# Hydr10n/DirectX-Physically-Based-Raytracer

Hardware: AMD Instinct MI355X
Metric: Mrays/s per GPU + frames/s at 1080p, Cornell Box 4spp/8bounce (higher is better)
Workload: dtype f32

## Files before the change

directx-physically-based-raytracer_amd/csrc/pt_api.hip:

```cpp
#include "pt_internal.hpp"

#include <cmath>
#include <cstdio>
#include <cstring>

using namespace pt;

static thread_local std::string g_createError;
namespace pt { std::string& create_error() { return g_createError; } }

int pt::fail(Context* c, int status, const std::string& msg)
{
    if (c) c->lastError = msg; else g_createError = msg;
    return status;
}
int pt::fail_hip(Context* c, hipError_t e, const char* what)
{
    return fail(c, e == hipErrorOutOfMemory ? PT_ERROR_OUT_OF_MEMORY : PT_ERROR_HIP, std::string(what) + ": " + hipGetErrorString(e));
}

static int poll_tlas_header(Context& c, bool wait);

extern "C" {

// ... 88 lines not shown

int pt_set_round_chains(PtContext* ctx, uint32_t chains)
{
    if (!ctx) return PT_ERROR_INVALID_ARGUMENT;
    API_ARG(&ctx->c, chains <= Context::kMaxChains, "at most 4 chains");
    ctx->c.chains = chains;
    ctx->c.graphKey.clear(); ctx->c.chainGraphKey.clear();
    return PT_OK;
}

int pt_sync(PtContext* ctx)
{
    if (!ctx) return PT_ERROR_INVALID_ARGUMENT;
    API_HIP(&ctx->c, hipSetDevice(ctx->c.device));
    API_HIP(&ctx->c, hipStreamSynchronize(ctx->c.stream));
    return poll_tlas_header(ctx->c, true);
}

int pt_heap_resize(PtContext* ctx, uint32_t descriptor_count)
{
    if (!ctx) return PT_ERROR_INVALID_ARGUMENT;
    ctx->c.heapHost.resize(descriptor_count, HeapEntry{ nullptr, 0, 0, 0 });
    ctx->c.heapDirty = true;
    return PT_OK;
}

int pt_heap_set_buffer(PtContext* ctx, uint32_t descriptor, const void* device_ptr, uint64_t bytes, uint32_t stride)
{
    if (!ctx) return PT_ERROR_INVALID_ARGUMENT;
    Context& c = ctx->c;
    API_ARG(&c, descriptor < c.heapHost.size(), "descriptor index beyond pt_heap_resize");
    API_ARG(&c, stride == 0 || stride == 2 || stride == 4 || stride == 8, "buffer stride must be 0 (raw), 2 / 4 (typed index buffer) or 8 (structured half4 motion vectors)");
    c.heapHost[descriptor] = HeapEntry{ device_ptr, bytes, stride, kKindBuffer };
    c.heapDirty = true;
    return PT_OK;
}

int pt_heap_set_texture(PtContext* ctx, uint32_t descriptor, const void* device_ptr, uint32_t width, uint32_t height, uint32_t format, uint32_t is_cube)
{
    if (!ctx) return PT_ERROR_INVALID_ARGUMENT;
    Context& c = ctx->c;
    API_ARG(&c, descriptor < c.heapHost.size(), "descriptor index beyond pt_heap_resize");
    API_ARG(&c, device_ptr && width && height, "texture pointer / size is null");
    API_ARG(&c, format <= PT_FORMAT_R32G32B32A32_FLOAT, "unsupported texture format");
    API_ARG(&c, !is_cube || width == height, "cube faces must be square");
    c.heapHost[descriptor] = HeapEntry{ device_ptr, (uint64_t)width | ((uint64_t)height << 32), format, is_cube ? kKindTextureCube : kKindTexture2D };
    c.heapDirty = true;
    return PT_OK;
}

static int upload_heap(Context& c)
{
    if (!c.srgbLutDev) {
        float lut[256];
        for (int i = 0; i < 256; i++) { double v = i / 255.0; lut[i] = (float)(v <= 0.04045 ? v / 12.92 : pow((v + 0.055) / 1.055, 2.4)); }
        DeviceBuffer<float> dev;
        API_HIP(&c, dev.reserve(256));
        API_HIP(&c, hipMemcpy(dev.data(), lut, sizeof lut, hipMemcpyHostToDevice));
        c.srgbLutDev = std::move(dev);
    }
    if (!c.heapDirty) return PT_OK;
    uint32_t n = (uint32_t)c.heapHost.size();
    c.heapHasTextures = false;
    for (const HeapEntry& e : c.heapHost) if (e.kind != kKindBuffer) c.heapHasTextures = true;
    API_HIP(&c, c.heapDev.reserve(n));
    if (n) API_HIP(&c, hipMemcpyAsync(c.heapDev.data(), c.heapHost.data(), sizeof(HeapEntry) * n, hipMemcpyHostToDevice, c.stream));
    API_HIP(&c, hipStreamSynchronize(c.stream));
    c.heapDirty = false; c.validated = false;
    return PT_OK;
}

static int check_geometries(Context& c, const PtGeometryDesc* geometries, uint32_t geometry_count)
{
    API_ARG(&c, geometries || geometry_count == 0, "geometries is NULL");
    for (uint32_t g = 0; g < geometry_count; g++) {
        API_ARG(&c, geometries[g].IndexStride == 2 || geometries[g].IndexStride == 4, "Triangle index format must be either uint16 or uint32");
        API_ARG(&c, geometries[g].IndexCount % 3 == 0, "Triangle index count must be divisible by 3");
        API_ARG(&c, geometries[g].IndexCount == 0 || (geometries[g].VertexBuffer && geometries[g].IndexBuffer), "geometry buffer is NULL");
        API_ARG(&c, geometries[g].VertexStride >= 12, "vertex stride must cover a float3 position");
    }
    return PT_OK;
}

static int check_depth(Context& c, uint32_t tlasDepth)
{
    if (2u * (tlasDepth + c.maxBlasDepth) + 4u > (uint32_t)kStackSize)
        return fail(&c, PT_ERROR_INVALID_ARGUMENT, "acceleration structure too deep for the traversal stack (top level " + std::to_string(tlasDepth)
                    + " + bottom level " + std::to_string(c.maxBlasDepth) + " levels)");
    return PT_OK;
}

static int poll_tlas_header(Context& c, bool wait)
{
    if (!c.tlasHeaderPending) return PT_OK;
    if (wait) API_HIP(&c, hipEventSynchronize(c.tlasHeaderEvent.get()));
    else if (hipEventQuery(c.tlasHeaderEvent.get()) != hipSuccess) { (void)hipGetLastError(); return PT_OK; }
    c.tlasHeaderPending = false;
    if (c.tlasHeaderHost.data()->error) { drop_tlas(c); return fail(&c, PT_ERROR_INVALID_ARGUMENT, "top-level build failed: tree deeper than the builder's level limit"); }
    int s = check_depth(c, c.tlasHeaderHost.data()->depth);
    if (s != PT_OK) drop_tlas(c);
    return s;
}

int pt_build_bottom_level(PtContext* ctx, const PtGeometryDesc* geometries, uint32_t geometry_count, uint32_t build_flags, uint64_t* out_blas_id)
{
    if (!ctx) return PT_ERROR_INVALID_ARGUMENT;
    Context& c = ctx->c;
    API_ARG(&c, out_blas_id, "out_blas_id is NULL");
    int s = check_geometries(c, geometries, geometry_count);
    if (s != PT_OK) return s;
    API_HIP(&c, hipSetDevice(c.device));
    Blas b;
    const bool updatable = (build_flags & PT_BUILD_FLAG_ALLOW_UPDATE) != 0;
    if (!updatable) std::swap(b.tree, c.buildScratch);
    hipError_t e = build_blas_device(geometries, geometry_count, updatable, c.stream, b);
    if (!updatable) std::swap(b.tree, c.buildScratch);
    if (e != hipSuccess) return fail_hip(&c, e, "bottom-level build");
    if (b.buildError || 2u * b.depth + 4u > (uint32_t)kStackSize) return fail(&c, PT_ERROR_INVALID_ARGUMENT, "bottom-level build failed: tree too deep for the traversal stack");
    b.geometryCount = geometry_count;
    uint64_t id = c.nextBlasId++;
    c.maxBlasDepth = std::max(c.maxBlasDepth, b.depth);
    c.blas[id] = std::move(b);
    *out_blas_id = id;
    return PT_OK;
}

int pt_update_bottom_level(PtContext* ctx, uint64_t blas_id, const PtGeometryDesc* geometries, uint32_t geometry_count, uint32_t build_flags)
{
    if (!ctx) return PT_ERROR_INVALID_ARGUMENT;
    Context& c = ctx->c;
    auto it = c.blas.find(blas_id);
    API_ARG(&c, it != c.blas.end(), "unknown bottom-level id");
    API_ARG(&c, c.viewers.empty(), "other contexts view this context's scene (pt_share_scene): destroy or re-point them before updating a bottom level");
    int s = check_geometries(c, geometries, geometry_count);
    if (s != PT_OK) return s;
    API_HIP(&c, hipSetDevice(c.device));
    Blas& b = it->second;
    uint32_t ntris = 0;
    for (uint32_t g = 0; g < geometry_count; g++) ntris += geometries[g].IndexCount / 3;
    if (b.updatable && ntris == b.triCount && geometry_count == b.geometryCount) {
        hipError_t e = refit_blas_device(geometries, geometry_count, c.stream, b);
        if (e != hipSuccess) return fail_hip(&c, e, "bottom-level update");
        drop_tlas(c);
        return PT_OK;
    }
    API_HIP(&c, hipStreamSynchronize(c.stream));
    Blas nb;
    const bool updatable = (build_flags & PT_BUILD_FLAG_ALLOW_UPDATE) != 0 || b.updatable;
    if (!updatable) std::swap(nb.tree, c.buildScratch);
    hipError_t e = build_blas_device(geometries, geometry_count, updatable, c.stream, nb);
    if (!updatable) std::swap(nb.tree, c.buildScratch);
    if (e != hipSuccess) return fail_hip(&c, e, "bottom-level update");
    if (nb.buildError || 2u * nb.depth + 4u > (uint32_t)kStackSize) return fail(&c, PT_ERROR_INVALID_ARGUMENT, "bottom-level update failed: tree too deep for the traversal stack");
    nb.geometryCount = geometry_count;
    c.maxBlasDepth = std::max(c.maxBlasDepth, nb.depth);
    b = std::move(nb);
    drop_tlas(c);
    return PT_OK;
}

int pt_skin_mesh(PtContext* ctx, const void* skeletal_vertices, const float* skeletal_transforms, void* vertices, void* motion_vectors, uint32_t vertex_count)
{
    if (!ctx) return PT_ERROR_INVALID_ARGUMENT;
    Context& c = ctx->c;
    API_ARG(&c, vertex_count == 0 || (skeletal_vertices && skeletal_transforms && vertices && motion_vectors), "a skinning buffer is NULL");
    API_HIP(&c, hipSetDevice(c.device));
    API_HIP(&c, launch_skin(c.stream, skeletal_vertices, skeletal_transforms, vertices, motion_vectors, vertex_count));
    return PT_OK;
}

int pt_release_bottom_level(PtContext* ctx, uint64_t blas_id)
{
    if (!ctx) return PT_ERROR_INVALID_ARGUMENT;
    Context& c = ctx->c;
    auto it = c.blas.find(blas_id);
    API_ARG(&c, it != c.blas.end(), "unknown bottom-level id");
    API_ARG(&c, c.viewers.empty(), "other contexts view this context's scene (pt_share_scene)");
    hipStreamSynchronize(c.stream);
    for (uint64_t id : c.tlasBlasIds) if (id == blas_id) { drop_tlas(c); break; }
    c.blas.erase(it);
    c.maxBlasDepth = 0;
    for (auto& kv : c.blas) c.maxBlasDepth = std::max(c.maxBlasDepth, kv.second.depth);
    return PT_OK;
}

namespace {
struct TopLevelPlan {
    struct Piece { uint64_t id; Blas* b; uint32_t nodeBase, triBase; bool referenced; };
    std::vector<Piece> pieces;
    std::vector<uint64_t> pieceIds;
    std::map<uint64_t, uint32_t> pieceOf;
    std::vector<BlasEntry> table;
    uint32_t tlasNodeExact = 0, tlasNodeCap = 0, blobNodes = 0, blobTris = 0;
    uint64_t tris = 0, objectEnd = 0, bindingHash = 1469598103934665603ull, lightHash = 1469598103934665603ull;
    size_t srcBytes = 0, nodeAt = 0, triAt = 0, idxAt = 0, instAt = 0, leafAt = 0, enterAt = 0, total = 0;
    size_t node_at(const Piece& p) const { return nodeAt + sizeof(WideNode) * (size_t)p.nodeBase; }
    size_t tri_at(const Piece& p) const { return triAt + sizeof(TriPacket) * (size_t)p.triBase; }
    size_t idx_at(const Piece& p) const { return idxAt + 16 * (size_t)p.triBase; }
    bool in_place(const Piece& p) const { return p.b->blobNodeAt == node_at(p) && p.b->blobTriAt == tri_at(p) && p.b->blobIdxAt == idx_at(p); }
};
}

static int plan_top_level(Context& c, const PtInstanceDesc* descs, uint32_t count, TopLevelPlan& P)
{
    P.tlasNodeExact = wide_node_capacity(count);
    P.tlasNodeCap = P.tlasNodeExact;
    if (count >= 64u) { P.tlasNodeCap = 128u; while (P.tlasNodeCap < P.tlasNodeExact) P.tlasNodeCap <<= 1; }
    if (c.blobDev && c.tlasNodeReserve >= P.tlasNodeExact && c.tlasNodeReserve <= 2u * P.tlasNodeCap) P.tlasNodeCap = c.tlasNodeReserve;
    P.blobNodes = P.tlasNodeCap;
    P.lightHash ^= count;
    P.srcBytes = sizeof(InstanceSource) * (size_t)count;
    std::vector<uint8_t>& up = c.tlasUploadHost;
    up.resize(P.srcBytes);
    for (uint32_t i = 0; i < count; i++) {
        auto it = c.blas.find(descs[i].AccelerationStructure);
        API_ARG(&c, it != c.blas.end(), "instance refers to an unknown bottom-level id");
        Blas& b = it->second;
        auto pb = P.pieceOf.find(descs[i].AccelerationStructure);
        if (pb == P.pieceOf.end()) {
            P.pieces.push_back(TopLevelPlan::Piece{ descs[i].AccelerationStructure, &b, P.blobNodes, P.blobTris, true });
            P.table.push_back(BlasEntry{ nullptr, nullptr, b.rootBounds.data(), b.triCount, b.nodeCount, P.blobNodes, P.blobTris, nullptr, descs[i].InstanceID & 0xFFFFFFu, b.geometryCount });
            P.blobNodes += b.nodeCount; P.blobTris += b.triCount;
            P.pieceIds.push_back(descs[i].AccelerationStructure);
            pb = P.pieceOf.emplace(descs[i].AccelerationStructure, (uint32_t)P.table.size() - 1).first;
        }
        InstanceSource src;
        memcpy(src.transform, descs[i].Transform, sizeof(float) * 12);
        src.instanceID = descs[i].InstanceID & 0xFFFFFFu; src.mask = descs[i].InstanceMask & 0xFFu; src.blasSlot = pb->second; src._pad = 0;
        memcpy(up.data() + sizeof(InstanceSource) * (size_t)i, &src, sizeof src);
        P.tris += b.triCount;
        P.objectEnd = std::max<uint64_t>(P.objectEnd, (uint64_t)src.instanceID + b.geometryCount);
        P.bindingHash = (P.bindingHash ^ src.instanceID) * 1099511628211ull; P.bindingHash = (P.bindingHash ^ descs[i].AccelerationStructure) * 1099511628211ull;
        P.lightHash = (P.lightHash ^ src.instanceID) * 1099511628211ull; P.lightHash = (P.lightHash ^ src.mask) * 1099511628211ull;
        P.lightHash = (P.lightHash ^ descs[i].AccelerationStructure) * 1099511628211ull;
    }
    for (auto& kv : c.blas)
        if (kv.second.inBlob && !P.pieceOf.count(kv.first)) {
// ... 51 lines not shown
        Blas& b = *p.b;
        uint8_t* dn = blob + P.node_at(p); uint8_t* dt = blob + P.tri_at(p); uint8_t* di = blob + P.idx_at(p);
        const uint64_t n16 = sizeof(WideNode) * (uint64_t)b.nodeCount / 16, t16 = sizeof(TriPacket) * (uint64_t)b.triCount / 16, i16 = b.triCount;
        const void *sn, *st_, *si;
        if (b.updatable) {
            jobs.push_back(BlobCopy{ b.nodes.data(), dn, n16 });
            if (b.triCount) { jobs.push_back(BlobCopy{ b.tris.data(), dt, t16 }); jobs.push_back(BlobCopy{ b.idx.data(), di, i16 }); }
            sn = b.nodes.data(); st_ = b.tris.data(); si = b.idx.data();
        } else {
            if (b.inBlob) {
                if (newBlob) {
                    preJobs.push_back(BlobCopy{ oldBlob + b.blobNodeAt, dn, n16 });
                    if (b.triCount) { preJobs.push_back(BlobCopy{ oldBlob + b.blobTriAt, dt, t16 }); preJobs.push_back(BlobCopy{ oldBlob + b.blobIdxAt, di, i16 }); }
                }
            } else {
                preJobs.push_back(BlobCopy{ b.nodes.data(), dn, n16 });
                if (b.triCount) { preJobs.push_back(BlobCopy{ b.tris.data(), dt, t16 }); preJobs.push_back(BlobCopy{ b.idx.data(), di, i16 }); }
                adopting.push_back(&b);
            }
            sn = dn; st_ = dt; si = di;
        }
        if (p.referenced) { BlasEntry& row = P.table[P.pieceOf[p.id]]; row.nodes = (const WideNode*)sn; row.tris = (const TriPacket*)st_; row.idx = (const uint4*)si; }
    }
    const size_t tableOff = (P.srcBytes + 15) / 16 * 16, tableBytes = sizeof(BlasEntry) * P.table.size();
    hipError_t e = build_tlas_prepare(c.tlas, count);
    if (e != hipSuccess) return fail_hip(&c, e, "top-level build");
    jobs.push_back(BlobCopy{ c.tlas.nodes.data(), blob + P.nodeAt, sizeof(WideNode) * (size_t)P.tlasNodeExact / 16 });
    const size_t preOff = (tableOff + tableBytes + 15) / 16 * 16, preBytes = sizeof(BlobCopy) * preJobs.size();
    const size_t jobsOff = (preOff + preBytes + 15) / 16 * 16, jobsBytes = sizeof(BlobCopy) * jobs.size();
    std::vector<uint8_t>& up = c.tlasUploadHost;
    up.resize(jobsOff + jobsBytes);
    if (tableBytes) memcpy(up.data() + tableOff, P.table.data(), tableBytes);
    if (preBytes) memcpy(up.data() + preOff, preJobs.data(), preBytes);
    memcpy(up.data() + jobsOff, jobs.data(), jobsBytes);
    if (up.size() > c.tlasUploadDev.capacity()) {
        if (!growth) API_HIP(&c, hipStreamSynchronize(c.stream));
        API_HIP(&c, c.tlasUploadDev.reserve(up.size() * 2));
    }
    {
        Context::UploadStage& sg = c.tlasStage[c.tlasStageNext];
        c.tlasStageNext ^= 1u;
        if (sg.event) API_HIP(&c, hipEventSynchronize(sg.event.get()));
        else API_HIP(&c, create_event(sg.event, hipEventDisableTiming));
        if (up.size() > sg.host.capacity()) API_HIP(&c, sg.host.reserve(up.size() * 2));
        memcpy(sg.host.data(), up.data(), up.size());
        API_HIP(&c, hipMemcpyAsync(c.tlasUploadDev.data(), sg.host.data(), up.size(), hipMemcpyHostToDevice, c.stream));
        API_HIP(&c, hipEventRecord(sg.event.get(), c.stream));
    }
    const uint8_t* upDev = c.tlasUploadDev.data();
    const InstanceSource* dSrc = (const InstanceSource*)upDev;
    const BlasEntry* dTable = (const BlasEntry*)(upDev + tableOff);
    const BlobCopy* dPre = (const BlobCopy*)(upDev + preOff);
    const BlobCopy* dJobs = (const BlobCopy*)(upDev + jobsOff);

    if (!preJobs.empty()) e = launch_blob_assembly(nullptr, c.tlas, nullptr, 0, nullptr, nullptr, dPre, (uint32_t)preJobs.size(), nullptr, c.stream);
    if (e == hipSuccess) e = launch_instance_records(dSrc, dTable, count, c.tlas.instances.data(), c.tlas.blasBounds.data(), c.tlas.tree.bounds.data(), c.stream);
    if (e == hipSuccess) e = build_tlas_device(c.tlas.instances.data(), c.tlas.blasBounds.data(), count, c.stream, c.tlas);
    if (e == hipSuccess) e = launch_blob_assembly(c.tlas.instances.data(), c.tlas, dTable, count, (InstanceT*)(blob + P.instAt), (InstanceT*)(blob + P.leafAt),
                                                 dJobs, (uint32_t)jobs.size(), (f4v*)(blob + P.enterAt), c.stream);
    if (e == hipSuccess) e = hipMemcpyAsync(c.tlasHeaderHost.data(), c.tlas.tree.header.data(), sizeof(WideHeader), hipMemcpyDeviceToHost, c.stream);
    if (e == hipSuccess) e = hipEventRecord(c.tlasHeaderEvent.get(), c.stream);
    if (!adopting.empty() || (newBlob && oldBlob)) {
        const hipError_t es = hipStreamSynchronize(c.stream);
        if (e == hipSuccess) e = es;
    }
    if (e != hipSuccess) {
        if (newCopy) (void)hipStreamSynchronize(c.stream);
        return fail_hip(&c, e, "top-level build");
    }

    if (newBlob) c.blobDev = std::move(newCopy);
    for (Blas* b : adopting) { b->nodes.reset(); b->tris.reset(); b->idx.reset(); b->inBlob = true; }
    for (const auto& p : P.pieces) if (p.b->inBlob) { p.b->blobNodeAt = P.node_at(p); p.b->blobTriAt = P.tri_at(p); p.b->blobIdxAt = P.idx_at(p); }
    c.tlasHeaderPending = true;
    c.tlasNodeReserve = P.tlasNodeCap;
    SceneRefs& r = c.scene;
    r.instances = c.tlas.instances.data(); r.instanceCount = count; r.triangleCount = P.tris;
    r.blob.base = (const f4v*)c.blobDev.data();
    r.blob.nodeOff16 = (uint32_t)(P.nodeAt / 16); r.blob.triOff16 = (uint32_t)(P.triAt / 16); r.blob.idxOff16 = (uint32_t)(P.idxAt / 16);
    r.blob.instOff16 = (uint32_t)(P.instAt / 16); r.blob.leafInstOff16 = (uint32_t)(P.leafAt / 16); r.blob.enterOff16 = (uint32_t)(P.enterAt / 16);
    r.blob.instCount = count; r.blob.nodeCount = P.blobNodes; r.blob.triCount = P.blobTris; r.blob.bytes = (uint32_t)P.total;
    r.blasTable = dTable; r.blasTableCount = (uint32_t)P.table.size(); r.instSource = dSrc; r.blasTableMaxTris = 0;
    for (const BlasEntry& te : P.table) r.blasTableMaxTris = std::max(r.blasTableMaxTris, te.triCount);
    c.tlasBlasIds = P.pieceIds;
    if (P.objectEnd != c.tlasObjectEnd || count != c.tlasValidatedCount || P.bindingHash != c.tlasBindingHash) c.validated = false;
    c.tlasObjectEnd = P.objectEnd; c.tlasValidatedCount = count; c.tlasBindingHash = P.bindingHash;
    if (P.lightHash != c.tlasLightHash) c.lightListValid = false;
    c.tlasLightHash = P.lightHash;
    c.normalsShared = c.validated && c.sharedVerdict;
    c.haveTlas = true;
    return PT_OK;
}

int pt_share_scene(PtContext* ctx, PtContext* source)
{
    if (!ctx || !source || ctx == source) return PT_ERROR_INVALID_ARGUMENT;
    Context& c = ctx->c; Context& s = source->c;
    API_ARG(&c, c.device == s.device, "both contexts must live on the same device");
    API_ARG(&c, c.viewers.empty(), "other contexts view this context's scene");
    API_ARG(&c, !s.sceneOwner, "the source views another context's scene itself: share from the owner");
    API_HIP(&c, hipSetDevice(c.device));
    API_HIP(&c, hipStreamSynchronize(s.stream));
    API_HIP(&c, hipStreamSynchronize(c.stream));
    int st = poll_tlas_header(s, true);
    if (st != PT_OK) return fail(&c, st, s.lastError);
    if (!s.haveTlas) return fail(&c, PT_ERROR_NOT_READY, "the source context has no top-level acceleration structure");
    if (c.sceneOwner) detach_from_owner(c);
    else { API_HIP(&c, materialise_adopted(c)); c.tlas = Tlas(); c.blobDev.reset(); }
    drop_tlas(c);
    c.scene = s.scene;
    c.tlasObjectEnd = s.tlasObjectEnd; c.maxBlasDepth = s.maxBlasDepth;
    c.heapHost = s.heapHost; c.heapDirty = true;
    c.objects = s.objects; c.objectCount = s.objectCount; c.instanceData = s.instanceData; c.instanceDataCount = s.instanceDataCount;
    c.sceneOwner = &s; s.viewers.push_back(&c);
    c.tlasHeaderPending = false; c.validated = false;
    c.haveTlas = true;
    return PT_OK;
}

int pt_get_accel_stats(PtContext* ctx, PtAccelStats* out)
{
    if (!ctx || !out) return PT_ERROR_INVALID_ARGUMENT;
    Context& c = ctx->c;
    API_HIP(&c, hipSetDevice(c.device));
    API_HIP(&c, hipStreamSynchronize(c.stream));
    int st = poll_tlas_header(c, true);
    if (st != PT_OK) return st;
    memset(out, 0, sizeof *out);
    out->InstanceCount = c.scene.instanceCount;
    out->BottomLevelCount = (uint32_t)c.blas.size();
    out->TriangleCount = c.scene.triangleCount;
    out->NodeSizeBytes = sizeof(WideNode); out->TriangleSizeBytes = sizeof(TriPacket);
    uint64_t nb = (uint64_t)wide_node_capacity(c.scene.instanceCount) * sizeof(WideNode), tb = 0;
    for (auto& kv : c.blas) { nb += (uint64_t)kv.second.nodeCount * sizeof(WideNode); tb += (uint64_t)kv.second.triCount * sizeof(TriPacket); out->MaxBottomLevelDepth = std::max(out->MaxBottomLevelDepth, kv.second.depth); }
    out->BlobBytes = c.sceneOwner ? 0 : c.scene.blob.bytes;
    out->SharedScene = c.sceneOwner ? 1u : 0u;
    out->NormalRecords = c.normalsShared ? 1u : 0u;
    out->RoundObjectsInLds = round_objects_in_lds(c, c.objectCount, (bool)c.shadeGeomDev);
    out->RoundRecordsInLds = round_records_in_lds(c, c.objectCount, (bool)c.shadeGeomDev);
    if (c.tlasHeaderHost && !c.tlasHeaderPending) out->TopLevelDepth = c.tlasHeaderHost.data()->depth;
    out->NodeBytes = nb; out->TriangleBytes = tb;
    for (auto& kv : c.blas) if (!kv.second.inBlob) out->OwnedBottomLevelBytes += (uint64_t)kv.second.nodeCount * sizeof(WideNode) + (uint64_t)kv.second.triCount * (sizeof(TriPacket) + 16);
    return PT_OK;
}

int pt_set_camera(PtContext* ctx, const PtCamera* camera)
{
    if (!ctx) return PT_ERROR_INVALID_ARGUMENT;
    API_ARG(&ctx->c, camera, "camera is NULL");
    ctx->c.camera = *camera; ctx->c.haveCamera = true;
    return PT_OK;
}
int pt_set_scene_data(PtContext* ctx, const PtSceneData* scene_data)
{
    if (!ctx) return PT_ERROR_INVALID_ARGUMENT;
    API_ARG(&ctx->c, scene_data, "scene_data is NULL");
    ctx->c.sceneData = *scene_data; ctx->c.haveSceneData = true;
    return PT_OK;
}
int pt_set_object_data(PtContext* ctx, const PtObjectData* device_objects, uint32_t count)
{
    if (!ctx) return PT_ERROR_INVALID_ARGUMENT;
    API_ARG(&ctx->c, device_objects || count == 0, "device_objects is NULL");
    ctx->c.objects = device_objects; ctx->c.objectCount = count;
    return PT_OK;
}
int pt_invalidate_object_data(PtContext* ctx)
{
    if (!ctx) return PT_ERROR_INVALID_ARGUMENT;
    ctx->c.validated = false; ctx->c.normalsShared = false; ctx->c.sharedVerdict = false;
    ctx->c.objectDataGen++;
    return PT_OK;
}
int pt_set_instance_data(PtContext* ctx, const PtInstanceData* device_instances, uint32_t count)
{
    if (!ctx) return PT_ERROR_INVALID_ARGUMENT;
    ctx->c.instanceData = device_instances; ctx->c.instanceDataCount = count;
    return PT_OK;
}

int pt_set_sharding(PtContext* ctx, const PtSharding* s)
{
    if (!ctx) return PT_ERROR_INVALID_ARGUMENT;
    API_ARG(&ctx->c, s && s->RankCount >= 1 && s->RankIndex < s->RankCount && s->BandHeight >= 1, "invalid sharding");
    ctx->c.sharding = *s;
    return PT_OK;
}

int pt_local_rows(const PtSharding* s, uint32_t frame_height, uint32_t* out_rows)
{
    if (!s || !out_rows || s->RankCount == 0 || s->BandHeight == 0 || s->RankIndex >= s->RankCount) return PT_ERROR_INVALID_ARGUMENT;
    uint32_t rows = 0;
    for (uint32_t b = s->RankIndex; (uint64_t)b * s->BandHeight < frame_height; b += s->RankCount) {
        uint32_t y0 = b * s->BandHeight;
        rows += (frame_height - y0 < s->BandHeight) ? frame_height - y0 : s->BandHeight;
    }
    *out_rows = rows;
    return PT_OK;
}

int pt_deinterleave_bands(PtContext* ctx, void* dst_full, const void* gathered, const uint64_t* rank_offsets_host, uint32_t rank_count,
                          uint32_t band_height, uint32_t width, uint32_t height, uint32_t pixel_bytes)
{
    if (!ctx) return PT_ERROR_INVALID_ARGUMENT;
    Context& c = ctx->c;
    API_ARG(&c, dst_full && gathered && rank_offsets_host && rank_count >= 1 && band_height >= 1, "invalid de-interleave arguments");
    API_ARG(&c, pixel_bytes % 4 == 0, "pixel size must be a multiple of 4 bytes");
    API_HIP(&c, hipSetDevice(c.device));
    API_ARG(&c, rank_count <= 64, "at most 64 ranks");
    hipError_t e = launch_deinterleave(c.stream, dst_full, gathered, rank_offsets_host, rank_count, band_height, width, height, pixel_bytes);
    if (e != hipSuccess) return fail_hip(&c, e, "de-interleave");
    return PT_OK;
}

}

static int validate_scene(Context& c)
{
    if (c.validated && c.validatedObjects == c.objects && c.validatedObjectCount == c.objectCount) return PT_OK;
    const uint32_t heapCount = (uint32_t)c.heapHost.size();
    if (c.tlasObjectEnd > c.objectCount)
        return fail(&c, PT_ERROR_INVALID_ARGUMENT, "InstanceID + geometry count of an instance reaches ObjectData[" + std::to_string(c.tlasObjectEnd - 1)
                    + "] but only " + std::to_string(c.objectCount) + " objects are bound (pt_set_object_data)");
    if (c.instanceData && c.instanceDataCount < c.scene.instanceCount)
        return fail(&c, PT_ERROR_INVALID_ARGUMENT, "InstanceData holds fewer records than the top level has instances");
    uint32_t sharedMismatch = 0;
    if (c.objectCount) {
        API_HIP(&c, c.validateDev.reserve(8));
        if (c.objectCount > c.shadeGeomDev.capacity()) {
            API_HIP(&c, hipStreamSynchronize(c.stream));
            c.shadeGeomDev.reset(); c.shadeTexDev.reset();
            API_HIP(&c, c.shadeTexDev.reserve(kTextureSlots * (size_t)c.objectCount));
            API_HIP(&c, c.shadeGeomDev.reserve(c.objectCount));
        }
        API_HIP(&c, hipMemsetAsync(c.validateDev.data(), 0, sizeof(uint32_t) * 8, c.stream));
        API_HIP(&c, launch_validate_objects(c.stream, c.objects, c.objectCount, c.heapDev.data(), heapCount, c.validateDev.data(), c.shadeGeomDev.data(), c.shadeTexDev.data()));
        if (c.scene.blasTable && c.scene.instSource)
            API_HIP(&c, launch_check_shared_geometry(c.stream, c.scene.instSource, c.scene.blasTable, c.scene.blob.instCount, c.shadeGeomDev.data(), c.validateDev.data()));
        uint32_t r[8] = { 0, 0, 0, 0, 0, 0, 0, 0 };
        API_HIP(&c, hipMemcpyAsync(r, c.validateDev.data(), sizeof r, hipMemcpyDeviceToHost, c.stream));
        API_HIP(&c, hipStreamSynchronize(c.stream));
        sharedMismatch = r[4];
        if (r[0]) {
            static const char* what[] = { "", "MeshDescriptors.Vertices", "MeshDescriptors.Indices", "MeshDescriptors.MotionVectors", "TextureMapInfo.Descriptor" };
            return fail(&c, PT_ERROR_INVALID_ARGUMENT, std::string("ObjectData[") + std::to_string(r[1]) + "]." + what[r[0] < 5 ? r[0] : 0] + " = " + std::to_string(r[2])
                        + (r[3] ? " is not the kind of descriptor that member needs" : " is beyond the descriptor heap (" + std::to_string(heapCount) + " descriptors)"));
        }
    }
    c.validated = true; c.validatedObjects = c.objects; c.validatedObjectCount = c.objectCount;
    c.sharedVerdict = c.objectCount != 0 && c.scene.blasTable != nullptr && sharedMismatch == 0;
    c.normalsShared = c.sharedVerdict;
    return PT_OK;
}

int pt::make_views(Context& c, uint32_t width, uint32_t height, SceneView& sv, FrameView& fv, bool needFrameInputs)
{
    int s = poll_tlas_header(c, true);
    if (s != PT_OK) return s;
    if (!c.haveTlas) return fail(&c, PT_ERROR_NOT_READY, "no top-level acceleration structure: call pt_build_top_level first");
    if (needFrameInputs && (!c.haveCamera || !c.haveSceneData)) return fail(&c, PT_ERROR_NOT_READY, "camera / scene data not set");
    if (!c.objects && c.scene.instanceCount) return fail(&c, PT_ERROR_NOT_READY, "object data not set");
    s = upload_heap(c);
    if (s != PT_OK) return s;
    s = validate_scene(c);
    if (s != PT_OK) return s;
    if (needFrameInputs && c.sceneData.EnvironmentLightTextureDescriptor != ~0u) {
        const uint32_t d = c.sceneData.EnvironmentLightTextureDescriptor;
        API_ARG(&c, d < c.heapHost.size(), "SceneData.EnvironmentLightTextureDescriptor is beyond the descriptor heap");
        API_ARG(&c, c.heapHost[d].kind == (c.sceneData.IsEnvironmentLightTextureCubeMap ? kKindTextureCube : kKindTexture2D),
                "SceneData.EnvironmentLightTextureDescriptor is not the kind of texture IsEnvironmentLightTextureCubeMap says");
    }
    sv.accel.instances = c.scene.instances; sv.accel.instanceCount = c.scene.instanceCount;
    sv.objects = c.objects; sv.objectCount = c.objectCount; sv.shadeGeom = c.shadeGeomDev.data(); sv.shadeTex = c.shadeTexDev.data();
    sv.instanceData = c.instanceData;
    sv.heap = c.heapDev.data(); sv.heapCount = (uint32_t)c.heapHost.size();
    sv.srgbLut = c.srgbLutDev.data();
    fv.width = width; fv.height = height;
    fv.rankIndex = c.sharding.RankIndex; fv.rankCount = c.sharding.RankCount; fv.bandHeight = c.sharding.BandHeight;
    pt_local_rows(&c.sharding, height, &fv.localRows);
    return PT_OK;
}

int pt::check_raytrace_args(Context& c, const PtTextures* tx)
{
    API_ARG(&c, c.settings.Denoiser <= PT_DENOISER_NRD_RELAX, "unknown Denoiser value");
    API_ARG(&c, !c.settings.IsDIEnabled || (tx->Diffuse && tx->Specular), "IsDIEnabled reads the direct lighting from Textures.Diffuse / Textures.Specular (pt_di_render): not bound");
    API_ARG(&c, !(c.settings.Denoiser >= PT_DENOISER_NRD_REBLUR) || (tx->Diffuse && tx->Specular), "NRD modes write Textures.Diffuse / Textures.Specular: not bound");
    API_ARG(&c, c.settings.SamplesPerPixel < 65536 && c.settings.Bounces < 32768, "SamplesPerPixel / Bounces out of range");
    API_ARG(&c, tx->Position && tx->FlatNormal && tx->GeometricNormal && tx->BaseColorMetalness && tx->NormalRoughness && tx->IOR
                 && tx->Transmission && tx->Radiance, "a G-buffer texture the path tracer reads is not bound (Raytracing::Textures)");
    return PT_OK;
}

extern "C" {

int pt_gbuffer_render(PtContext* ctx, const PtGBufferConstants* constants, const PtTextures* textures)
{
    if (!ctx) return PT_ERROR_INVALID_ARGUMENT;
    Context& c = ctx->c;
    API_ARG(&c, constants && textures, "constants / textures is NULL");
    API_HIP(&c, hipSetDevice(c.device));
    SceneView sv; FrameView fv; memset(&sv, 0, sizeof sv); memset(&fv, 0, sizeof fv);
    int s = make_views(c, constants->RenderSize[0], constants->RenderSize[1], sv, fv);
    if (s != PT_OK) return s;
    API_HIP(&c, launch_gbuffer(c, sv, fv, constants->Flags, *textures));
    return PT_OK;
}

int pt_raytrace_set_constants(PtContext* ctx, const PtGraphicsSettings* settings)
{
    if (!ctx) return PT_ERROR_INVALID_ARGUMENT;
    API_ARG(&ctx->c, settings, "settings is NULL");
    ctx->c.settings = *settings; ctx->c.haveSettings = true;
    return PT_OK;
}

int pt_raytrace_render(PtContext* ctx, const PtTextures* tx)
{
    if (!ctx) return PT_ERROR_INVALID_ARGUMENT;
    Context& c = ctx->c;
    API_ARG(&c, tx, "textures is NULL");
    if (!c.haveSettings) return fail(&c, PT_ERROR_NOT_READY, "call pt_raytrace_set_constants first");
    int s = check_raytrace_args(c, tx);
    if (s != PT_OK) return s;
    API_HIP(&c, hipSetDevice(c.device));
    SceneView sv; FrameView fv; memset(&sv, 0, sizeof sv); memset(&fv, 0, sizeof fv);
    s = make_views(c, c.settings.RenderSize[0], c.settings.RenderSize[1], sv, fv);
    if (s != PT_OK) return s;
    if (c.settings.Bounces == 0) return PT_OK;
    API_HIP(&c, launch_raytrace(c, sv, fv, *tx, false));
    return PT_OK;
}

int pt_trace_visibility(PtContext* ctx, const PtRayDesc* device_rays, uint32_t count, float* device_visibility)
// ... 168 lines not shown
```

directx-physically-based-raytracer_amd/csrc/pt_internal.hpp:

```cpp
#pragma once
#include <hip/hip_runtime.h>

#include <algorithm>
#include <map>
#include <string>
#include <type_traits>
#include <vector>

#include "../../include/ptamd.h"
#include "pt_memory.hpp"
#include "pt_trace2.hpp"
#include "pt_sharc.hpp"

namespace pt {

struct WideHeader { uint32_t nodeCount, itemCount, depth, error; };

struct TreeBuffers {
    DeviceBuffer<float4> boxLo, boxHi; DeviceBuffer<uint32_t> bounds;
    DeviceBuffer<uint64_t> keys, keysSorted; DeviceBuffer<uint32_t> index, indexSorted;
    DeviceBuffer<uint8_t> sortTemp; size_t sortTempBytes = 0;
    DeviceBuffer<uint64_t> leafKeys; DeviceBuffer<float4> leafLo, leafHi;
    DeviceBuffer<int2> children; DeviceBuffer<int> parentInternal, parentLeaf;
    DeviceBuffer<float4> nodeLo, nodeHi; DeviceBuffer<uint32_t> arrival;
    DeviceBuffer<int> binaryRootOf, slotRefs; DeviceBuffer<uint32_t> leafDst, slotOfPrim;
    DeviceBuffer<WideHeader> header; DeviceBuffer<uint8_t> collapseState;
    DeviceBuffer<uint8_t> dp;
};

inline uint32_t wide_node_capacity(uint32_t nleaves) { return nleaves + 1u; }

struct Blas {
    DeviceBuffer<WideNode> nodes;
    DeviceBuffer<TriPacket> tris;
    DeviceBuffer<uint4> idx;
    DeviceBuffer<float> rootBounds;
    uint32_t triCount = 0, leafCount = 0, nodeCount = 0, depth = 0, geometryCount = 0;
    bool buildError = false, updatable = false;
    bool inBlob = false; uint64_t blobNodeAt = 0, blobTriAt = 0, blobIdxAt = 0;
    TreeBuffers tree;
};

struct Tlas {
    DeviceBuffer<WideNode> nodes;
    DeviceBuffer<float> rootBounds;
    DeviceBuffer<InstanceRecord> instances;
    DeviceBuffer<const float*> blasBounds;
    TreeBuffers tree;
};

struct InstanceSource { float transform[12]; uint32_t instanceID, mask, blasSlot, _pad; };
struct BlasEntry { const WideNode* nodes; const TriPacket* tris; const float* rootBounds; uint32_t triCount, nodeCount, nodeBase, triBase; const uint4* idx;
                   uint32_t objectBase, geometryCount; };
struct BlobCopy { const void* src; void* dst; uint64_t n16; };

struct SceneRefs {
    const InstanceRecord* instances = nullptr; uint32_t instanceCount = 0;
    uint64_t triangleCount = 0;
    BlobView blob{};
    const BlasEntry* blasTable = nullptr; uint32_t blasTableCount = 0, blasTableMaxTris = 0;
    const InstanceSource* instSource = nullptr;
};

struct alignas(16) ShadeGeom { const uint8_t* vb; uint32_t stride, nOff, tOff, uvOff[2], _pad; };
static_assert(sizeof(ShadeGeom) == 32, "layout");

struct SceneView {
    AccelView accel;
    const PtObjectData* objects;
    const ShadeGeom* shadeGeom;
    const HeapEntry* shadeTex;
    const PtInstanceData* instanceData;
    const HeapEntry* heap;
    const float* srgbLut;
    uint32_t objectCount, heapCount;
};

struct FrameView {
    uint32_t width, height;
    uint32_t localRows;
    uint32_t rankIndex, rankCount, bandHeight;
};

struct PathQueue {
    float4* s0;
    float4* s1;
    float4* s2;
    float4* r0;
    float4* r1;
    uint4*  hit;
};

constexpr uint32_t kSubQueueShiftFused = 5, kSubQueueShiftStream = 7, kSubQueuesMax = 1u << kSubQueueShiftStream;

struct FrameConstants { PtCamera cam; PtSceneData sd; PtGraphicsSettings gs; };
struct RoundArgs;

struct DeviceCounters {
    unsigned long long primaryRays, secondaryRays, nodesVisited, trianglesTested;
    unsigned int mismatchCount, stackOverflows;
    float mismatchRay[16];
    unsigned int maxNodesPerRay, _pad2;
};

struct Context {
    int device = 0;
    hipStream_t stream = nullptr;
    std::string lastError;

    std::vector<HeapEntry> heapHost;
    DeviceBuffer<HeapEntry> heapDev; bool heapDirty = true;
    DeviceBuffer<float> srgbLutDev;
    bool heapHasTextures = false;

    std::map<uint64_t, Blas> blas; uint64_t nextBlasId = 1;
    TreeBuffers buildScratch;
    Tlas tlas; bool haveTlas = false;
    DeviceBuffer<uint8_t> blobDev;
    SceneRefs scene;
    Context* sceneOwner = nullptr;
    std::vector<Context*> viewers;
    uint32_t framesInFlight = 1;
    std::vector<uint64_t> tlasBlasIds;
    std::vector<uint8_t> tlasUploadHost; DeviceBuffer<uint8_t> tlasUploadDev;
    struct UploadStage { PinnedBuffer<uint8_t> host; Event event; };
    UploadStage tlasStage[2]; uint32_t tlasStageNext = 0;
    PinnedBuffer<WideHeader> tlasHeaderHost; Event tlasHeaderEvent; bool tlasHeaderPending = false;
    uint32_t maxBlasDepth = 0, tlasNodeReserve = 0;
    uint32_t tlasValidatedCount = ~0u, persistentGrid = 0;
    uint64_t tlasBindingHash = 0;
    uint64_t tlasObjectEnd = 0;
    DeviceBuffer<ShadeGeom> shadeGeomDev;
    DeviceBuffer<HeapEntry> shadeTexDev;
    DeviceBuffer<uint4> shadeRecA; DeviceBuffer<uint32_t> shadeRecB;
    bool normalsShared = false;
    bool sharedVerdict = false;
    bool validated = false; DeviceBuffer<uint32_t> validateDev;
    const void* validatedObjects = nullptr; uint32_t validatedObjectCount = 0;

    PtCamera camera{}; PtSceneData sceneData{}; PtGraphicsSettings settings{};
    bool haveCamera = false, haveSceneData = false, haveSettings = false;
    const PtObjectData* objects = nullptr; uint32_t objectCount = 0;
    const PtInstanceData* instanceData = nullptr; uint32_t instanceDataCount = 0;
    PtSharding sharding{0, 1, 16, 0};

    DeviceBuffer<uint4> queueArrays[2][6];
    PathQueue queue[2]{};
    DeviceBuffer<uint4> primaryRecords;
    DeviceBuffer<float2> pixelAux;
    DeviceBuffer<FrameConstants> frameConstants;
    GraphExec graphExec; std::string graphKey; bool disableGraphs = false;
    static constexpr uint32_t kMaxChains = 4;
    uint32_t chains = 0;
    Stream chainStream[kMaxChains - 1]; Event chainFork, chainJoin[kMaxChains - 1];
    GraphExec chainGraph[kMaxChains]; std::string chainGraphKey;
    DeviceBuffer<uint32_t> queueCounts;
    DeviceBuffer<RoundArgs> roundArgs; std::string roundArgsKey;
    DeviceBuffer<DeviceCounters> counters;
    uint64_t lastIterations = 0;
    uint32_t debugFlags = 0;

    void* comm = nullptr; bool commOwned = false; uint32_t commRank = 0, commWorld = 1;

    bool timing = false;
    std::vector<Event> evExtend, evShade, evRound;
    uint32_t nExtend = 0, nShade = 0, nRound = 0;

    PtDISettings diSettings{}; bool haveDISettings = false;
    uint64_t tlasLightHash = 0;
    uint32_t objectDataGen = 0;
    DeviceBuffer<uint4> lightList; uint32_t lightCount = 0;
    DeviceBuffer<uint32_t> lightInstStart;
    uint64_t lightListKey = 0; bool lightListValid = false;
    DeviceBuffer<PtTriangleLight> lightRecords; DeviceBuffer<float> lightCdf, lightBlockSums; uint32_t lightRecordCount = 0;
    PtDIResamplingSettings diReuse{}; bool diReuseOn = false;
    DeviceBuffer<PtDIReservoir> diResA, diResB;
    DeviceBuffer<int8_t> diOffsets;
    bool diHistoryValid = false; uint32_t diHistorySize[2] = {0, 0}; uint64_t diHistoryLightKey = 0; uint32_t diResCount = 0;
    PtDIVisibilitySettings diVisibility{}; bool diVisibilityOn = false;
    PtDIPairwiseSettings diPairwise{};
    PtDILightSamplingSettings diSampling{};
    DeviceBuffer<PtDIPresampledLight> diTiles, diCells;
    uint32_t diTileCount = 0, diCellCount = 0;
    uint32_t diReGIRLayout = 0;
    DeviceBuffer<float> diOnion;

    PtPostProcessSettings post{}; bool havePost = false;
    DeviceBuffer<ushort4> postLevels;
    uint32_t postDims[9][2] = {};
    size_t postOffset[9] = {};

    PtSHARCSettings sharcSettings{}; bool haveSharcSettings = false;
    uint32_t sharcCapacity = 0, sharcParity = 0;
    DeviceBuffer<unsigned long long> sharcKeys;
    DeviceBuffer<uint4> sharcVoxels[2];
    DeviceBuffer<SharcView> sharcView;
    DeviceBuffer<float> sharcRough[2];
    DeviceBuffer<PtSHARCPathScatter> sharcLogScatter;
    DeviceBuffer<PtSHARCPathVertex> sharcLog; uint32_t sharcLogPaths = 0, sharcLogBounces = 0;
};

std::string& create_error();
int fail(Context* c, int status, const std::string& msg);
int fail_hip(Context* c, hipError_t e, const char* what);
#define API_HIP(ctx, expr) do { hipError_t e_ = (expr); if (e_ != hipSuccess) return pt::fail_hip(ctx, e_, #expr); } while (0)
#define API_ARG(ctx, cond, msg) do { if (!(cond)) return pt::fail(ctx, PT_ERROR_INVALID_ARGUMENT, msg); } while (0)
int make_views(Context& c, uint32_t width, uint32_t height, SceneView& sv, FrameView& fv, bool needFrameInputs = true);
int check_raytrace_args(Context& c, const PtTextures* tx);

template <typename T>
int download_counted(Context& c, const T* src, uint32_t count, uint32_t row, T* host_dst, uint32_t capacity, uint32_t* out_count, uint32_t* out_row = nullptr)
{
    API_HIP(&c, hipSetDevice(c.device));
    API_HIP(&c, hipStreamSynchronize(c.stream));
    *out_count = count;
    if (out_row) *out_row = row;
    const size_t n = std::min((size_t)capacity, (size_t)count * row);
    if (n) API_HIP(&c, hipMemcpy(host_dst, src, sizeof(T) * n, hipMemcpyDeviceToHost));
    return PT_OK;
}

template <typename F> void with_flags(F&& f) { f(); }
template <typename F, typename... Rest> void with_flags(F&& f, bool first, Rest... rest)
{
    if (first) with_flags([&](auto... bs) { f(std::true_type{}, bs...); }, rest...);
    else with_flags([&](auto... bs) { f(std::false_type{}, bs...); }, rest...);
}

hipError_t build_blas_device(const PtGeometryDesc* geoms, uint32_t ngeoms, bool allowUpdate, hipStream_t stream, Blas& out);
hipError_t refit_blas_device(const PtGeometryDesc* geoms, uint32_t ngeoms, hipStream_t stream, Blas& b);
hipError_t build_tlas_prepare(Tlas& out, uint32_t n);
hipError_t build_tlas_device(const InstanceRecord* dInstances, const float* const* dBlasBounds, uint32_t n, hipStream_t stream, Tlas& out);
hipError_t launch_instance_records(const InstanceSource* src, const BlasEntry* table, uint32_t n, InstanceRecord* rec, const float** bounds, uint32_t* sceneBounds, hipStream_t stream);
hipError_t launch_blob_assembly(const InstanceRecord* inst, const Tlas& tlas, const BlasEntry* table, uint32_t n, InstanceT* outInst,
                                InstanceT* outLeafInst, const BlobCopy* jobs, uint32_t njobs, f4v* outEnter, hipStream_t stream);
__host__ __device__ void invert_3x4(const float m[12], float out[12]);

hipError_t launch_skin(hipStream_t stream, const void* skeletal, const float* transforms, void* vertices, void* motion, uint32_t count);

struct FramePlan {
    uint32_t rounds, segCap, grid, sqShift;
    bool streaming, fused, first;
    bool flat, lds;
    uint32_t ldsFixed, roundLds, extend2Lds;
    uint32_t objectsInLds, recordsInLds;
    bool recordsUsable;
    bool writeT, stats, di, textured, sharc;
    float2* aux;
    uint32_t nsq() const { return 1u << sqShift; }
    uint32_t cstride() const { return 3u * nsq(); }
};

hipError_t launch_shade(Context& c, const FramePlan& p, const SceneView& sv, const FrameView& fv, const PtTextures& tx, uint32_t round, uint32_t grid, hipStream_t stream,
                        uint32_t sqBase, uint32_t sqCount);
hipError_t launch_extend_stream(Context& c, const FramePlan& p, const AlphaContext& ac, uint32_t round, hipStream_t stream, uint32_t sqBase, uint32_t sqCount);

hipError_t launch_gbuffer(Context& c, const SceneView& sv, const FrameView& fv, uint32_t flags, const PtTextures& tx);
hipError_t launch_raytrace(Context& c, const SceneView& sv, const FrameView& fv, const PtTextures& tx, bool sharcQuery);
hipError_t launch_visibility(Context& c, const SceneView& sv, const void* rays, uint32_t count, void* out);
hipError_t launch_bsdf_evaluate(hipStream_t stream, const float* q, uint32_t count, float* r);
hipError_t launch_bsdf_sample(hipStream_t stream, const float* q, uint32_t count, float* r);
hipError_t launch_debug_trace(Context& c, const SceneView& sv, const float* ray8, uint32_t* devLog, uint32_t logCap);
hipError_t launch_debug_closest(Context& c, const SceneView& sv, const void* rays, uint32_t count, void* hits);
uint32_t round_objects_in_lds(const Context& c, uint32_t objectCount, bool haveShadeGeom);
uint32_t round_records_in_lds(const Context& c, uint32_t objectCount, bool haveShadeGeom);
inline bool normal_records_usable(const Context& c) { return c.normalsShared && c.scene.blasTable && c.scene.blasTableCount <= 65535u  && c.shadeRecB && c.scene.blob.triCount && c.scene.blob.triCount <= c.shadeRecB.capacity(); }
hipError_t launch_check_shared_geometry(hipStream_t stream, const InstanceSource* src, const BlasEntry* table, uint32_t n, const ShadeGeom* shadeGeom, uint32_t* out);
hipError_t launch_validate_objects(hipStream_t stream, const PtObjectData* objects, uint32_t count, const HeapEntry* heap, uint32_t heapCount, uint32_t* out, ShadeGeom* shadeGeom, HeapEntry* shadeTex);
hipError_t launch_deinterleave(hipStream_t stream, void* dst, const void* src, const uint64_t* rankOffsetsHost, uint32_t rankCount,
                               uint32_t bandHeight, uint32_t width, uint32_t height, uint32_t pixelBytes);

}

struct PtContext { pt::Context c; };
```

directx-physically-based-raytracer_amd/csrc/pt_kernels.hip:

```cpp
#include "pt_internal.hpp"

#include <cstring>

#include "pt_shade.hpp"

namespace pt {

template <bool STATS, bool TEXTURED, int MODE>
__global__ __launch_bounds__(256) void k_gbuffer(SceneView sv, FrameView fv, PtCamera cam, PtSceneData sd, uint32_t flags, PtTextures tx,
                                                 BlobView bv, DeviceCounters* counters)
{
    const uint32_t wv = threadIdx.x >> 6, ln = threadIdx.x & 63u;
    const uint32_t x = blockIdx.x * 16 + (wv & 1u) * 8u + (ln & 7u), ly = blockIdx.y * 16 + (wv >> 1) * 8u + (ln >> 3);
    const bool valid = x < fv.width && ly < fv.localRows;
    if (MODE == 0 && !valid) return;
    const uint32_t y = global_row(fv, valid ? ly : 0u);
    const size_t pi = (size_t)ly * fv.width + x;

    float4 Position = make_float4(INFINITY, INFINITY, INFINITY, INFINITY);
    float LinearDepth = INFINITY, NormalizedDepth = cam.IsNormalizedDepthReversed ? 0.0f : 1.0f;
    float u, v;
    const RayDesc ray = generate_pinhole_ray(cam, valid ? x : 0u, y, fv.width, fv.height, u, v);
    TraceStats st; st.nodes = 0; st.tris = 0; st.overflow = 0;
    Hit hit;
// ... 204 lines not shown
        if (b.inst != h.inst || (h.inst != ~0u && (b.slot != h.slot || b.u != h.u || b.v != h.v))) {
            if (atomicAdd(&counters->mismatchCount, 1u) == 0u) {
                float* m = counters->mismatchRay;
                m[0] = o.x; m[1] = o.y; m[2] = o.z; m[3] = o.w; m[4] = d.x; m[5] = d.y; m[6] = d.z; m[7] = d.w;
                m[8] = __uint_as_float(b.inst); m[9] = __uint_as_float(b.slot); m[10] = b.t; m[11] = 0.0f;
                m[12] = __uint_as_float(h.inst); m[13] = __uint_as_float(h.slot); m[14] = h.t; m[15] = 0.0f;
            }
        }
        q.hit[i] = make_uint4(h.inst, h.slot, __float_as_uint(h.u), __float_as_uint(h.v));
    }
    if (st.overflow) atomicAdd(&counters->stackOverflows, st.overflow);
}

constexpr int kStackLds2 = 8;
constexpr uint32_t kStackLds2Bytes = (uint32_t)kStackLds2 * 256u * 8u;
constexpr uint32_t kExtendLdsFixed = kStackLds2Bytes + (uint32_t)kCandidates * 256u * 4u + 4u * kPhasedWaveLds;
constexpr uint32_t kBlobLdsMax = 40u * 1024u;

template <bool STATS, bool LDS, bool WRITE_T = false, bool FLAT = false>
__global__ __launch_bounds__(256) void k_extend2(BlobView bv, AlphaContext ac, PathQueue q, uint32_t segCap, const uint32_t* count, DeviceCounters* counters, uint32_t sqShift)
{
    extern __shared__ __attribute__((aligned(16))) unsigned char smem[];
    constexpr uint32_t kFixed = FLAT ? kFlatLdsFixed : kExtendLdsFixed;
    const uint32_t nsq = 1u << sqShift, sq = blockIdx.x & (nsq - 1u), bq = blockIdx.x >> sqShift, nbq = gridDim.x >> sqShift;
    const uint32_t n = count[sq];
    if (bq == 0 && threadIdx.x == 0) atomicAdd(&counters->secondaryRays, (unsigned long long)n);
    if (bq * 256u >= n) return;
    PT_LDS_AS void* ldsStack = (PT_LDS_AS void*)smem;
    BlobReader<LDS> blob;
    if constexpr (LDS) {
        f4v* dst = (f4v*)(smem + kFixed);
        const uint32_t n16 = bv.bytes / 16u;
        for (uint32_t i = threadIdx.x; i < n16; i += 256u) dst[i] = bv.base[i];
        __syncthreads();
        blob.p = (const PT_LDS_AS f4v*)(smem + kFixed);
    } else {
        blob.p = bv.base;
    }
    TraceStats st; st.nodes = 0; st.tris = 0; st.overflow = 0;
    if constexpr (FLAT) {
        unsigned char* ldsWave = smem + (uint32_t)kStackLdsFlat * 256u * 8u + (threadIdx.x >> 6) * kFlatWaveLds;
        for (uint32_t base = bq * 256u; base < n; base += nbq * 256u) {
            const uint32_t local = base + threadIdx.x;
            const bool valid = local < n;
            const uint32_t i = sq * segCap + (valid ? local : base);
            float4 o = q.r0[i], d = q.r1[i];
            if (!valid) { o.w = 1.0f; d.w = 0.0f; }
            const Hit h = trace_closest_flat<STATS, LDS>(blob, bv, ac, V3(o.x, o.y, o.z), V3(d.x, d.y, d.z), o.w, d.w, ldsStack, ldsWave, &st);
            if (valid) {
                q.hit[i] = make_uint4(h.inst, h.slot, __float_as_uint(h.u), __float_as_uint(h.v));
                if (WRITE_T) q.r1[i].w = h.t;
            }
        }
    } else {
        uint32_t* ldsCand = (uint32_t*)(smem + kStackLds2Bytes);
        unsigned char* ldsWave = smem + kStackLds2Bytes + (uint32_t)kCandidates * 256u * 4u + (threadIdx.x >> 6) * kPhasedWaveLds;
        for (uint32_t base = bq * 256u; base < n; base += nbq * 256u) {
            const uint32_t local = base + threadIdx.x;
            const bool valid = local < n;
            const uint32_t i = sq * segCap + (valid ? local : base);
            float4 o = q.r0[i], d = q.r1[i];
            if (!valid) { o.w = 1.0f; d.w = 0.0f; }
            const Hit h = trace_closest_v2<STATS, LDS, kStackLds2>(blob, bv, ac, V3(o.x, o.y, o.z), V3(d.x, d.y, d.z), o.w, d.w, ldsStack, ldsCand, ldsWave, &st);
            if (valid) {
                q.hit[i] = make_uint4(h.inst, h.slot, __float_as_uint(h.u), __float_as_uint(h.v));
                if (WRITE_T) q.r1[i].w = h.t;
            }
        }
    }
    if (STATS) { atomicAdd(&counters->nodesVisited, (unsigned long long)st.nodes); atomicAdd(&counters->trianglesTested, (unsigned long long)st.tris); }
    if (st.overflow) atomicAdd(&counters->stackOverflows, st.overflow);
}

struct RoundArgs {
    SceneView sv; FrameView fv; PtTextures tx; BlobView bv; PathQueue qin, qout;
    const FrameConstants* fc; float2* aux; const uint32_t* countIn; uint32_t* countOut; DeviceCounters* counters; uint32_t segCap;
    uint32_t objectsInLds;
    const uint4* recA; const uint32_t* recB;
    uint32_t recordsInLds, sqShift;
    const uint4* primary;
    const SharcView* sharc; const float* roughIn; float* roughOut;
};

template <bool TEXTURED, bool LDS, bool FLAT, bool DI, bool SHARC = false>
__global__ __launch_bounds__(256) __attribute__((amdgpu_waves_per_eu(4, 4))) void k_round(const RoundArgs* __restrict__ A, uint32_t sqBase, uint32_t sqCount)
{
    const SceneView& sv = A->sv; const FrameView& fv = A->fv; const PtTextures& tx = A->tx; const BlobView& bv = A->bv;
    const PathQueue& qin = A->qin; const PathQueue& qout = A->qout;
    const FrameConstants* __restrict__ fc = A->fc; float2* aux = A->aux; const uint32_t segCap = A->segCap;
    const uint32_t* countIn = A->countIn; uint32_t* countOut = A->countOut; DeviceCounters* counters = A->counters;
    const uint4* __restrict__ primary = A->primary;
    extern __shared__ __attribute__((aligned(16))) unsigned char smem[];
    __shared__ uint32_t lds[32];
    uint32_t emits = 0;
    constexpr uint32_t kFixed = FLAT ? kFlatLdsFixed : kExtendLdsFixed;
    const PtCamera& cam = fc->cam; const PtSceneData& sd = fc->sd; const PtGraphicsSettings& gs = fc->gs;
    const uint32_t sqShift = A->sqShift;
    const uint32_t nsq = 1u << sqShift, bq = blockIdx.x / sqCount, sq = sqBase + (blockIdx.x - bq * sqCount), nbq = gridDim.x / sqCount;
    const uint32_t nT = countIn[sq], nF = countIn[nsq + sq];
    const uint32_t seg = sq * segCap;
    if (bq == 0 && threadIdx.x == 0) atomicAdd(&counters->secondaryRays, (unsigned long long)nT);

#ifdef PT_ROUND_PROF
    RoundProf profData; RoundProf* prof = &profData;
    for (int k = 0; k < 16; k++) profData.acc[k] = 0;
    profData.last = __builtin_readcyclecounter();
#else
    RoundProf* prof = nullptr;
#endif
    if (bq * 256u < nT) {
        PT_LDS_AS void* ldsStack = (PT_LDS_AS void*)smem;
        BlobReader<LDS> blob;
        ShadeTables tables;
        tables.recA = A->recA; tables.recB = A->recB;
        if constexpr (LDS) {
            f4v* dst = (f4v*)(smem + kFixed);
            const uint32_t n16 = bv.bytes / 16u;
            for (uint32_t k = threadIdx.x; k < n16; k += 256u) dst[k] = bv.base[k];
            const uint32_t nobj = A->objectsInLds;
            for (uint32_t k = threadIdx.x; k < nobj * kObjLds16; k += 256u) {
                const uint32_t o = k / kObjLds16, part = k - o * kObjLds16;
                dst[n16 + k] = part < 2u ? ((const f4v*)&sv.shadeGeom[o])[part] : ((const f4v*)&sv.objects[o].Material)[part - 2u];
            }
            const uint32_t nrec = A->recordsInLds, recBase = n16 + nobj * kObjLds16;
            for (uint32_t k = threadIdx.x; k < nrec; k += 256u) {
                const uint4 a = A->recA[k];
                dst[recBase + k] = (f4v){ __uint_as_float(a.x), __uint_as_float(a.y), __uint_as_float(a.z), __uint_as_float(a.w) };
                ((uint32_t*)(dst + recBase + nrec))[k] = A->recB[k];
            }
            __syncthreads();
            blob.p = (const PT_LDS_AS f4v*)(smem + kFixed);
            if (nobj) tables.objects = (ObjectTableLds)(smem + kFixed) + n16;
            if (nrec) { tables.recALds = (const PT_LDS_AS f4v*)(smem + kFixed) + recBase; tables.recBLds = (const PT_LDS_AS uint32_t*)((const PT_LDS_AS f4v*)(smem + kFixed) + recBase + nrec); }
        } else {
            blob.p = bv.base;
        }
        const AlphaContext ac = alpha_context(sv);
        TraceStats st; st.nodes = 0; st.tris = 0; st.overflow = 0;
        for (uint32_t base = bq * 256u; base < nT; base += nbq * 256u) {
            const uint32_t local = base + threadIdx.x;
            const bool valid = local < nT;
            const uint32_t i = seg + (valid ? local : base);
            float4 o = qin.r0[i], d = qin.r1[i];
            PathRegs p = load_path(qin, i);
            float pr = 0.0f;
            if constexpr (SHARC) pr = A->roughIn[i];
            if (!valid) { o.w = 1.0f; d.w = 0.0f; }
            PT_PROF_MARK(prof, 0);
            Hit h;
            if constexpr (FLAT) {
                unsigned char* ldsWave = smem + (uint32_t)kStackLdsFlat * 256u * 8u + (threadIdx.x >> 6) * kFlatWaveLds;
                h = trace_closest_flat<false, LDS>(blob, bv, ac, V3(o.x, o.y, o.z), V3(d.x, d.y, d.z), o.w, d.w, ldsStack, ldsWave, &st, prof);
            } else {
                uint32_t* ldsCand = (uint32_t*)(smem + kStackLds2Bytes);
                unsigned char* ldsWave = smem + kStackLds2Bytes + (uint32_t)kCandidates * 256u * 4u + (threadIdx.x >> 6) * kPhasedWaveLds;
                h = trace_closest_v2<false, LDS, kStackLds2>(blob, bv, ac, V3(o.x, o.y, o.z), V3(d.x, d.y, d.z), o.w, d.w, ldsStack, ldsCand, ldsWave, &st);
            }
            bool toTraced = false, toFresh = false;
            v3 newO = V3(0, 0, 0), newD = V3(0, 0, 1);
            if (valid) {
                shade_traced<TEXTURED, DI, SHARC>(sv, GeometryFromBlob<LDS>{ blob, bv, tables }, sd, gs, tx, aux, p, make_uint4(h.inst, h.slot, __float_as_uint(h.u), __float_as_uint(h.v)), h.t,
                                       V3(d.x, d.y, d.z), toTraced, toFresh, newO, newD, prof, A->sharc, &pr);
            }
            PT_PROF_MARK(prof, 6);
            emit_tile<SHARC>(qout, seg, segCap, &countOut[sq], &countOut[nsq + sq], lds + ((emits++ & 1u) << 4), toTraced, toFresh, p, newO, newD, A->roughOut, pr);
            PT_PROF_MARK(prof, 7);
#ifdef PT_ROUND_PROF
            prof->acc[11] += 1u;
#endif
        }
        if (st.overflow) atomicAdd(&counters->stackOverflows, st.overflow);
    }
    for (uint32_t tile = bq; tile * 256u < nF; tile += nbq) {
        const uint32_t local = tile * 256u + threadIdx.x;
        bool toTraced = false, toFresh = false;
        PathRegs p; v3 newO = V3(0, 0, 0), newD = V3(0, 0, 1);
        float pr = 0.0f;
        if (local < nF) {
            p = load_path(qin, seg + (segCap - 1u - local));
            PT_PROF_WAIT(); PT_PROF_MARK(prof, 12);
            shade_fresh<DI, SHARC>(fv, cam, gs, tx, aux, primary, p, toTraced, toFresh, newO, newD, prof, &pr);
        }
        PT_PROF_MARK(prof, 14);
        emit_tile<SHARC>(qout, seg, segCap, &countOut[sq], &countOut[nsq + sq], lds + ((emits++ & 1u) << 4), toTraced, toFresh, p, newO, newD, A->roughOut, pr);
        PT_PROF_MARK(prof, 15);
    }
#ifdef PT_ROUND_PROF
    PT_PROF_MARK(prof, 8);
    if ((threadIdx.x & 63u) == 0u) for (int k = 0; k < 16; k++) atomicAdd((unsigned int*)&counters->mismatchRay[k], (k < 9 || k >= 12) ? (prof->acc[k] >> 6) : prof->acc[k]);
#endif
}

template <bool STATS>
__global__ __launch_bounds__(256) void k_extend(BlobView bv, AlphaContext ac, PathQueue q, uint32_t segCap, const uint32_t* count, DeviceCounters* counters, uint32_t sqShift)
{
    const uint32_t nsq = 1u << sqShift, sq = blockIdx.x & (nsq - 1u), bq = blockIdx.x >> sqShift, nbq = gridDim.x >> sqShift;
    const uint32_t n = count[sq];
    if (bq == 0 && threadIdx.x == 0) atomicAdd(&counters->secondaryRays, (unsigned long long)n);
    __shared__ uint2 ldsStack[kLdsStackDepth * 256];
    uint2 spill[kStackSize - kLdsStackDepth];
    GroupStack<kLdsStackDepth> stack; stack.init((PT_LDS_AS void*)ldsStack, spill);
    BlobReader<false> blob; blob.p = bv.base;
    TraceStats st; st.nodes = 0; st.tris = 0; st.overflow = 0;
    for (uint32_t local = bq * 256u + threadIdx.x; local < n; local += nbq * 256u) {
        const uint32_t i = sq * segCap + local;
        const float4 o = q.r0[i], d = q.r1[i];
        const Hit h = trace_single<STATS, false, false>(blob, bv, ac, V3(o.x, o.y, o.z), V3(d.x, d.y, d.z), o.w, d.w, stack, &st, nullptr);
        q.hit[i] = make_uint4(h.inst, h.slot, __float_as_uint(h.u), __float_as_uint(h.v));
    }
    if (STATS) { atomicAdd(&counters->nodesVisited, (unsigned long long)st.nodes); atomicAdd(&counters->trianglesTested, (unsigned long long)st.tris); }
    if (st.overflow) atomicAdd(&counters->stackOverflows, st.overflow);
}

static uint32_t persistent_grid(Context& c);

__global__ __launch_bounds__(256) void k_visibility(BlobView bv, AlphaContext ac, const float4* __restrict__ rays, uint32_t count, float4* __restrict__ out,
                                                    DeviceCounters* counters)
{
    __shared__ uint2 ldsStack[kLdsStackDepth * 256];
    uint2 spill[kStackSize - kLdsStackDepth];
    GroupStack<kLdsStackDepth> stack; stack.init((PT_LDS_AS void*)ldsStack, spill);
    BlobReader<false> blob; blob.p = bv.base;
    TraceStats st; st.nodes = 0; st.tris = 0; st.overflow = 0;
    for (uint32_t i = blockIdx.x * blockDim.x + threadIdx.x; i < count; i += gridDim.x * blockDim.x) {
        const float4 o = rays[2 * (size_t)i], d = rays[2 * (size_t)i + 1];
        v3 vis;
        const Hit h = trace_single<false, false, true>(blob, bv, ac, V3(o.x, o.y, o.z), V3(d.x, d.y, d.z), o.w, d.w, stack, &st, &vis);
        out[i] = make_float4(vis.x, vis.y, vis.z, h.inst == ~0u ? 1.0f : 0.0f);
    }
    if (st.overflow) atomicAdd(&counters->stackOverflows, st.overflow);
}

__global__ __launch_bounds__(256) void k_debug_trace(BlobView bv, AlphaContext ac, float4 o, float4 d, uint32_t* log, uint32_t logCap)
{
    __shared__ uint2 ldsStack[kLdsStackDepth * 256];
    uint2 spill[kStackSize - kLdsStackDepth];
    GroupStack<kLdsStackDepth> stack; stack.init((PT_LDS_AS void*)ldsStack, spill);
    BlobReader<false> blob; blob.p = bv.base;
    TraceStats st; st.nodes = 0; st.tris = 0; st.overflow = 0;
    const float a = 0.02f * (float)threadIdx.x, ca = cosf(a), sa = sinf(a);
    const v3 dd = V3(d.x * ca - d.z * sa, d.y, d.x * sa + d.z * ca);
    trace_single<false, false, false, GroupStack<kLdsStackDepth>, true>(blob, bv, ac, V3(o.x, o.y, o.z), dd, o.w, d.w, stack, &st, nullptr, log, threadIdx.x == 0 ? logCap : 0u);
}

hipError_t launch_debug_trace(Context& c, const SceneView& sv, const float* ray8, uint32_t* devLog, uint32_t logCap)
{
    k_debug_trace<<<1, 256, 0, c.stream>>>(c.scene.blob, alpha_context(sv), make_float4(ray8[0], ray8[1], ray8[2], ray8[3]), make_float4(ray8[4], ray8[5], ray8[6], ray8[7]), devLog, logCap);
    return hipGetLastError();
}

template <bool BRUTE>
__global__ __launch_bounds__(256) void k_debug_closest(AccelView av, BlobView bv, AlphaContext ac, const float4* __restrict__ rays, uint32_t count, uint4* __restrict__ out,
                                                       DeviceCounters* counters)
{
    __shared__ uint2 ldsStack[kLdsStackDepth * 256];
    uint2 spill[kStackSize - kLdsStackDepth];
    GroupStack<kLdsStackDepth> stack; stack.init((PT_LDS_AS void*)ldsStack, spill);
    BlobReader<false> blob; blob.p = bv.base;
    TraceStats st; st.nodes = 0; st.tris = 0; st.overflow = 0;
    for (uint32_t i = blockIdx.x * blockDim.x + threadIdx.x; i < count; i += gridDim.x * blockDim.x) {
        const float4 o = rays[2 * (size_t)i], d = rays[2 * (size_t)i + 1];
        const Hit h = BRUTE ? trace_brute_force(av, ac, V3(o.x, o.y, o.z), V3(d.x, d.y, d.z), o.w, d.w)
                            : trace_single<false, false, false>(blob, bv, ac, V3(o.x, o.y, o.z), V3(d.x, d.y, d.z), o.w, d.w, stack, &st, nullptr);
        out[2 * (size_t)i] = make_uint4(__float_as_uint(h.t), __float_as_uint(h.u), __float_as_uint(h.v), h.inst);
        out[2 * (size_t)i + 1] = make_uint4(h.geom, h.prim, h.slot, 0u);
    }
    if (st.overflow) atomicAdd(&counters->stackOverflows, st.overflow);
}

__global__ void k_validate_objects(const PtObjectData* __restrict__ objects, uint32_t count, const HeapEntry* __restrict__ heap, uint32_t heapCount, uint32_t* out,
                                   ShadeGeom* __restrict__ shadeGeom, HeapEntry* __restrict__ shadeTex)
{
    const uint32_t i = blockIdx.x * blockDim.x + threadIdx.x;
    if (i >= count) return;
    const PtObjectData* od = &objects[i];
    uint32_t err = 0, desc = 0, kind = 0;
    const uint32_t md[3] = { od->MeshDescriptors.Vertices, od->MeshDescriptors.Indices, od->MeshDescriptors.MotionVectors };
    for (uint32_t k = 0; k < 3 && !err; k++) {
        if (md[k] == ~0u) continue;
        if (md[k] >= heapCount) { err = k + 1; desc = md[k]; }
        else if (heap[md[k]].kind != kKindBuffer) { err = k + 1; desc = md[k]; kind = 1; }
    }
    for (uint32_t k = 0; k < 7 && !err; k++) {
        const uint32_t d = od->TextureMapInfoArray[k].Descriptor;
        if (d == ~0u) continue;
        if (d >= heapCount) { err = 4; desc = d; }
        else if (heap[d].kind != kKindTexture2D) { err = 4; desc = d; kind = 1; }
    }
    for (uint32_t k = 0; k < kTextureSlots; k++) {
        HeapEntry e; e.ptr = nullptr; e.bytes = 0; e.stride = 0; e.kind = 0;
        const uint32_t d = od->TextureMapInfoArray[k].Descriptor;
        if (!err && d != ~0u) { e = heap[d]; e.kind = od->TextureMapInfoArray[k].TextureCoordinateIndex & 1u; }
        shadeTex[(size_t)i * kTextureSlots + k] = e;
    }
    if (err && atomicCAS(&out[0], 0u, err) == 0u) { out[1] = i; out[2] = desc; out[3] = kind; }
    ShadeGeom sg; sg.vb = nullptr; sg.stride = 0; sg.nOff = ~0u; sg.tOff = ~0u; sg.uvOff[0] = sg.uvOff[1] = ~0u; sg._pad = 0;
    if (!err && md[0] != ~0u && md[1] != ~0u) {
        sg.vb = (const uint8_t*)heap[md[0]].ptr; sg.stride = od->VertexDesc.Stride;
        sg.nOff = od->VertexDesc.AttributeOffsets.Normal; sg.tOff = od->VertexDesc.AttributeOffsets.Tangent;
        sg.uvOff[0] = od->VertexDesc.AttributeOffsets.TextureCoordinates[0]; sg.uvOff[1] = od->VertexDesc.AttributeOffsets.TextureCoordinates[1];
    }
    shadeGeom[i] = sg;
}

hipError_t launch_validate_objects(hipStream_t stream, const PtObjectData* objects, uint32_t count, const HeapEntry* heap, uint32_t heapCount, uint32_t* out, ShadeGeom* shadeGeom, HeapEntry* shadeTex)
{
    if (count) k_validate_objects<<<(count + 255) / 256, 256, 0, stream>>>(objects, count, heap, heapCount, out, shadeGeom, shadeTex);
    return hipGetLastError();
}

__global__ __launch_bounds__(256) void k_capture_normals(const BlasEntry* __restrict__ table, const ShadeGeom* __restrict__ shadeGeom, uint4* __restrict__ recA, uint32_t* __restrict__ recB)
{
    const BlasEntry e = table[blockIdx.y];
    for (uint32_t k = blockIdx.x * 256u + threadIdx.x; k < e.triCount; k += gridDim.x * 256u) {
        const uint32_t geom = __float_as_uint(e.tris[k].a.w);
        const ShadeGeom sg = shadeGeom[e.objectBase + geom];
        uint32_t n[9] = { 0, 0, 0, 0, 0, 0, 0, 0, 0 }, has = 0;
        if (sg.vb && sg.nOff != ~0u) {
            const uint4 ix = e.idx[k];
            const uint32_t vi[3] = { ix.x, ix.y, ix.z };
            has = 1u;
            #pragma unroll
            for (int v = 0; v < 3; v++) {
                const PT_GLOBAL_AS uint16_t* q = gptr<uint16_t>(sg.vb + (size_t)sg.stride * vi[v] + sg.nOff);
                n[3 * v] = q[0]; n[3 * v + 1] = q[1]; n[3 * v + 2] = q[2];
            }
        }
        recA[e.triBase + k] = make_uint4(n[0] | (n[1] << 16), n[2] | (n[3] << 16), n[4] | (n[5] << 16), n[6] | (n[7] << 16));
        recB[e.triBase + k] = n[8] | (has << 16);
    }
}

__global__ void k_check_shared_geometry(const InstanceSource* __restrict__ src, const BlasEntry* __restrict__ table, uint32_t n, const ShadeGeom* __restrict__ shadeGeom, uint32_t* out)
{
    const uint32_t i = blockIdx.x * blockDim.x + threadIdx.x;
    if (i >= n) return;
    const uint32_t id = src[i].instanceID, base = table[src[i].blasSlot].objectBase, ng = table[src[i].blasSlot].geometryCount;
    if (id == base) return;
    for (uint32_t g = 0; g < ng; g++) {
        const ShadeGeom a = shadeGeom[id + g], b = shadeGeom[base + g];
        if (a.vb != b.vb || a.stride != b.stride || a.nOff != b.nOff) { out[4] = 1u; return; }
    }
}

hipError_t launch_check_shared_geometry(hipStream_t stream, const InstanceSource* src, const BlasEntry* table, uint32_t n, const ShadeGeom* shadeGeom, uint32_t* out)
{
    if (n) k_check_shared_geometry<<<(n + 255) / 256, 256, 0, stream>>>(src, table, n, shadeGeom, out);
    return hipGetLastError();
}

__global__ __launch_bounds__(256) void k_bsdf_evaluate(const float* __restrict__ q, uint32_t count, float* __restrict__ r)
{
    const uint32_t i = blockIdx.x * blockDim.x + threadIdx.x;
    if (i >= count) return;
    const float* a = q + 20 * (size_t)i;
    BSDFSample b;
    const bool front = a[7] != 0.0f;
    b.Initialize(V3(a), a[3], a[4], a[5], a[6], front);
    const SurfaceVectors sv = surface_vectors(front, V3(a + 8), V3(a + 11));
    const v3 V = V3(a + 14), L = V3(a + 17);
    float w[3]; b.ComputeLobeWeights(sv, V, 0, w);
    float pdf; v3 dif, spc;
    b.EvaluateAll(sv, L, V, w, pdf, dif, spc);
    float* o = r + 8 * (size_t)i;
    o[0] = dif.x; o[1] = dif.y; o[2] = dif.z; o[3] = spc.x; o[4] = spc.y; o[5] = spc.z; o[6] = pdf; o[7] = 0.0f;
}

__global__ __launch_bounds__(256) void k_bsdf_sample(const float* __restrict__ q, uint32_t count, float* __restrict__ r)
{
    const uint32_t i = blockIdx.x * blockDim.x + threadIdx.x;
    if (i >= count) return;
    const float* a = q + 24 * (size_t)i;
    BSDFSample b;
    const bool front = a[7] != 0.0f;
    b.Initialize(V3(a), a[3], a[4], a[5], a[6], front);
    const SurfaceVectors sv = surface_vectors(front, V3(a + 8), V3(a + 11));
    const v3 V = V3(a + 14);
    const float rnd[4] = { a[17], a[18], a[19], a[20] };
    const uint32_t ext = __float_as_uint(a[21]);
    float w[3]; b.ComputeLobeWeights(sv, V, ext, w);
    v3 L = V3(0.0f, 0.0f, 0.0f); int lobe = 0;
    const bool ok = b.Sample(sv, V, w, rnd, L, lobe);
    float pdf = 0.0f; v3 f = V3(0.0f, 0.0f, 0.0f);
    if (ok) b.EvaluateLobe(sv, L, V, w, lobe, ext, pdf, f);
    float* o = r + 12 * (size_t)i;
    o[0] = L.x; o[1] = L.y; o[2] = L.z; o[3] = pdf; o[4] = f.x; o[5] = f.y; o[6] = f.z; o[7] = w[0]; o[8] = w[1]; o[9] = w[2];
    o[10] = __uint_as_float((uint32_t)lobe); o[11] = __uint_as_float(ok ? 1u : 0u);
}

hipError_t launch_visibility(Context& c, const SceneView& sv, const void* rays, uint32_t count, void* out)
{
    if (!count) return hipSuccess;
    k_visibility<<<persistent_grid(c), 256, 0, c.stream>>>(c.scene.blob, alpha_context(sv), (const float4*)rays, count, (float4*)out, c.counters.data());
    return hipGetLastError();
}

hipError_t launch_debug_closest(Context& c, const SceneView& sv, const void* rays, uint32_t count, void* hits)
{
    if (!count) return hipSuccess;
    if (c.debugFlags & PT_DEBUG_BRUTE_FORCE)
        k_debug_closest<true><<<persistent_grid(c), 256, 0, c.stream>>>(sv.accel, c.scene.blob, alpha_context(sv), (const float4*)rays, count, (uint4*)hits, c.counters.data());
    else
        k_debug_closest<false><<<persistent_grid(c), 256, 0, c.stream>>>(sv.accel, c.scene.blob, alpha_context(sv), (const float4*)rays, count, (uint4*)hits, c.counters.data());
    return hipGetLastError();
}

hipError_t launch_bsdf_evaluate(hipStream_t stream, const float* q, uint32_t count, float* r)
{
    if (!count) return hipSuccess;
    k_bsdf_evaluate<<<(count + 255) / 256, 256, 0, stream>>>(q, count, r);
    return hipGetLastError();
}

hipError_t launch_bsdf_sample(hipStream_t stream, const float* q, uint32_t count, float* r)
{
    if (!count) return hipSuccess;
    k_bsdf_sample<<<(count + 255) / 256, 256, 0, stream>>>(q, count, r);
    return hipGetLastError();
}


struct RankOffsets { uint64_t v[64]; };

__global__ void k_deinterleave(uint8_t* dst, const uint8_t* src, RankOffsets rankOffsets, uint32_t rankCount, uint32_t bandHeight,
                               uint32_t width, uint32_t height, uint32_t pixelBytes)
{
    const uint64_t rowBytes = (uint64_t)width * pixelBytes, chunks = rowBytes / 4;
    const uint64_t total = chunks * height;
    for (uint64_t t = (uint64_t)blockIdx.x * blockDim.x + threadIdx.x; t < total; t += (uint64_t)gridDim.x * blockDim.x) {
        const uint32_t y = (uint32_t)(t / chunks); const uint64_t cx = t % chunks;
        const uint32_t band = y / bandHeight, rank = band % rankCount, localRow = (band / rankCount) * bandHeight + (y - band * bandHeight);
        ((uint32_t*)(dst + (uint64_t)y * rowBytes))[cx] = ((const uint32_t*)(src + rankOffsets.v[rank] + (uint64_t)localRow * rowBytes))[cx];
    }
}

static uint32_t persistent_grid(Context& c)
{
    if (!c.persistentGrid) {
        hipDeviceProp_t p;
        const uint32_t g = hipGetDeviceProperties(&p, c.device) == hipSuccess ? (uint32_t)p.multiProcessorCount * 8u : 1024u;
        c.persistentGrid = (g + kSubQueuesMax - 1) / kSubQueuesMax * kSubQueuesMax;
    }
    return c.persistentGrid;
}

static bool gbuffer_flat(const Context& c)
{
    return c.scene.blob.base && c.scene.blob.instCount <= kFlatInstances &&
           !(c.debugFlags & (PT_DEBUG_TRAVERSAL_V1 | PT_DEBUG_TRAVERSAL_PHASED | PT_DEBUG_BRUTE_FORCE));
}

hipError_t launch_gbuffer(Context& c, const SceneView& sv, const FrameView& fv, uint32_t flags, const PtTextures& tx)
{
    if (fv.localRows == 0 || fv.width == 0) return hipSuccess;
    dim3 grid((fv.width + 15) / 16, (fv.localRows + 15) / 16);
    const int mode = !gbuffer_flat(c) ? 0 : (c.scene.blob.bytes <= kBlobLdsMax ? 1 : 2);
    const uint32_t smem = mode == 0 ? 0u : kFlatLdsFixed + (mode == 1 ? c.scene.blob.bytes : 0u);
    with_flags([&](auto S, auto T) {
        auto launch = [&](auto M) { k_gbuffer<S(), T(), M()><<<grid, 256, smem, c.stream>>>(sv, fv, c.camera, c.sceneData, flags, tx, c.scene.blob, c.counters.data()); };
        if (mode == 0) launch(std::integral_constant<int, 0>{}); else if (mode == 1) launch(std::integral_constant<int, 1>{}); else launch(std::integral_constant<int, 2>{});
    }, (c.debugFlags & PT_DEBUG_TRAVERSAL_STATS) != 0, c.heapHasTextures);
    return hipGetLastError();
}

static hipError_t ensure_queues(Context& c, uint32_t capacity, uint32_t iterations)
{
    hipError_t e = hipSuccess;
    for (auto& arrays : c.queueArrays) for (auto& a : arrays) if (e == hipSuccess) e = a.reserve(capacity);
    for (int k = 0; k < 2; k++) {
        DeviceBuffer<uint4>* a = c.queueArrays[k];
        c.queue[k] = PathQueue{ (float4*)a[0].data(), (float4*)a[1].data(), (float4*)a[2].data(), (float4*)a[3].data(), (float4*)a[4].data(), a[5].data() };
    }
    if (e != hipSuccess) return e;
    if ((e = c.primaryRecords.reserve(3 * (size_t)capacity)) != hipSuccess) return e;
    return c.queueCounts.reserve(iterations);
}

static void timing_begin(Context& c, std::vector<Event>& ev, uint32_t k)
{
    if (!c.timing) return;
    while (ev.size() < 2 * (size_t)(k + 1)) { hipEvent_t e; hipEventCreate(&e); ev.emplace_back(e); }
    hipEventRecord(ev[2 * k].get(), c.stream);
}
static void timing_end(Context& c, std::vector<Event>& ev, uint32_t k) { if (c.timing) hipEventRecord(ev[2 * k + 1].get(), c.stream); }

static uint32_t lds_bytes_of_records(uint32_t n) { return (n * 20u + 15u) / 16u * 16u; }
static uint32_t round_lds_bytes(bool flat, uint32_t blobBytes, uint32_t objects, uint32_t records)
{
    return (flat ? kFlatLdsFixed : kExtendLdsFixed) + blobBytes + objects * kObjLds16 * 16u + lds_bytes_of_records(records);
}
static bool round_lds_fits(uint32_t bytes) { return (bytes + 128u + 511u) / 512u * 512u <= 160u * 1024u / 4u; }
static bool lockstep_flat(const Context& c) { return c.scene.blob.instCount <= kFlatInstances && !(c.debugFlags & PT_DEBUG_TRAVERSAL_PHASED); }

uint32_t round_objects_in_lds(const Context& c, uint32_t objectCount, bool haveShadeGeom)
{
    if (c.scene.blob.bytes > kBlobLdsMax || !objectCount || !haveShadeGeom) return 0u;
    return round_lds_fits(round_lds_bytes(lockstep_flat(c), c.scene.blob.bytes, objectCount, 0u)) ? objectCount : 0u;
}
uint32_t round_records_in_lds(const Context& c, uint32_t objectCount, bool haveShadeGeom)
{
    const uint32_t nobj = round_objects_in_lds(c, objectCount, haveShadeGeom);
    if (!nobj || !normal_records_usable(c)) return 0u;
    return round_lds_fits(round_lds_bytes(lockstep_flat(c), c.scene.blob.bytes, nobj, c.scene.blob.triCount)) ? c.scene.blob.triCount : 0u;
}

static void plan_frame(FramePlan& p, Context& c, const SceneView& sv, const FrameView& fv, bool sharcQuery)
{
    std::memset(&p, 0, sizeof p);
    const PtGraphicsSettings& gs = c.settings;
    const uint32_t tiles = (fv.width * fv.localRows + 255u) / 256u;
    p.rounds = gs.SamplesPerPixel * (gs.Bounces + 1u);
    p.lds = c.scene.blob.bytes <= kBlobLdsMax;
    p.sqShift = p.lds ? kSubQueueShiftFused : kSubQueueShiftStream;
    p.segCap = (tiles + p.nsq() - 1) / p.nsq() * 256u;
    p.grid = std::min(persistent_grid(c), (tiles + p.nsq() - 1) / p.nsq() * p.nsq());
    const uint32_t lockStepFlags = PT_DEBUG_LOCKSTEP | PT_DEBUG_TRAVERSAL_PHASED | PT_DEBUG_BRUTE_FORCE | PT_DEBUG_TRAVERSAL_V1 | PT_DEBUG_UNFUSED_ROUNDS;
    const uint32_t pairOnlyFlags = PT_DEBUG_TRAVERSAL_STATS | PT_DEBUG_BRUTE_FORCE | PT_DEBUG_TRAVERSAL_V1 | PT_DEBUG_UNFUSED_ROUNDS;
    p.streaming = !p.lds && !(c.debugFlags & lockStepFlags);
    p.fused = !p.streaming && !(c.debugFlags & pairOnlyFlags);
    p.first = p.streaming || p.fused;
    p.flat = lockstep_flat(c);
    p.ldsFixed = p.flat ? kFlatLdsFixed : kExtendLdsFixed;
    p.recordsUsable = normal_records_usable(c);
    p.objectsInLds = round_objects_in_lds(c, sv.objectCount, sv.shadeGeom != nullptr);
    p.recordsInLds = round_records_in_lds(c, sv.objectCount, sv.shadeGeom != nullptr);
    p.extend2Lds = round_lds_bytes(p.flat, p.lds ? c.scene.blob.bytes : 0u, 0u, 0u);
    p.roundLds = round_lds_bytes(p.flat, p.lds ? c.scene.blob.bytes : 0u, p.objectsInLds, p.recordsInLds);
    p.aux = gs.Denoiser != PT_DENOISER_NONE ? c.pixelAux.data() : nullptr;
    p.sharc = sharcQuery;
    p.writeT = p.aux != nullptr || p.sharc;
    p.stats = (c.debugFlags & PT_DEBUG_TRAVERSAL_STATS) != 0;
    p.di = gs.IsDIEnabled != 0u;
    p.textured = c.heapHasTextures;
}

constexpr uint32_t kStreamingChains = 3;
static uint32_t frame_chains(const Context& c, const FramePlan& p, bool ownStreams)
{
    if (!p.first) return 1u;
    const uint32_t choice = (p.streaming && c.framesInFlight <= 1) ? kStreamingChains : 1u;
    const uint32_t want = c.chains ? c.chains : (ownStreams ? choice : 1u);
    return std::max(1u, std::min({ want, Context::kMaxChains, p.nsq() }));
}

static hipError_t enqueue_preamble(Context& c, const FramePlan& p, const SceneView& sv, const FrameView& fv, const PtTextures& tx)
{
    if (p.recordsUsable)
        k_capture_normals<<<dim3(std::min((c.scene.blasTableMaxTris + 255u) / 256u, 64u), c.scene.blasTableCount), 256, 0, c.stream>>>(c.scene.blasTable, sv.shadeGeom, c.shadeRecA.data(), c.shadeRecB.data());
    if (p.first)
        with_flags([&](auto S, auto D) {
            k_pt_first<D(), S()><<<p.grid, 256, 0, c.stream>>>(fv, c.frameConstants.data(), tx, c.queue[1], p.aux, p.segCap, &c.queueCounts.data()[p.cstride()], c.primaryRecords.data(), p.sqShift, c.sharcRough[1].data());
        }, p.sharc, p.di);
    else k_pt_init<<<p.grid, 256, 0, c.stream>>>(fv, c.frameConstants.data(), tx, c.queue[0], p.aux, p.segCap, &c.queueCounts.data()[p.nsq()], c.primaryRecords.data(), p.sqShift);
    return hipGetLastError();
}

static hipError_t enqueue_chain(Context& c, const FramePlan& p, const SceneView& sv, const FrameView& fv, const PtTextures& tx, uint32_t g, uint32_t chains, hipStream_t s)
{
    const uint32_t nsq = p.nsq(), perSq = std::max(1u, p.grid / nsq);
    const uint32_t sqBase = (uint32_t)((uint64_t)nsq * g / chains), sqCount = (uint32_t)((uint64_t)nsq * (g + 1) / chains) - sqBase;
    if (p.streaming) {
        const AlphaContext ac = alpha_context(sv);
        for (uint32_t r = 0; r <= p.rounds; r++) {
            if (r > 0) {
                timing_begin(c, c.evShade, c.nShade);
                launch_shade(c, p, sv, fv, tx, r, perSq * sqCount, s, sqBase, sqCount);
                timing_end(c, c.evShade, c.nShade); c.nShade++;
            }
            if (r == p.rounds) break;
            timing_begin(c, c.evExtend, c.nExtend);
            launch_extend_stream(c, p, ac, r, s, sqBase, sqCount);
            timing_end(c, c.evExtend, c.nExtend); c.nExtend++;
        }
        return hipGetLastError();
    }
    for (uint32_t r = 1; r <= p.rounds; r++) {
        timing_begin(c, c.evRound, c.nRound);
        with_flags([&](auto T, auto L, auto F, auto D, auto S) {
            k_round<T(), L(), F(), D(), S()><<<perSq * sqCount, 256, p.roundLds, s>>>(c.roundArgs.data() + r, sqBase, sqCount);
        }, p.textured, p.lds, p.flat, p.di, p.sharc);
        timing_end(c, c.evRound, c.nRound); c.nRound++;
    }
    return hipGetLastError();
}

static hipError_t enqueue_validation_rounds(Context& c, const FramePlan& p, const SceneView& sv, const FrameView& fv, const PtTextures& tx)
{
    const AlphaContext ac = alpha_context(sv);
    for (uint32_t r = 0; r <= p.rounds; r++) {
        PathQueue& qout = c.queue[(r + 1) & 1];
        uint32_t* cout = &c.queueCounts.data()[(r + 1) * p.cstride()];
        timing_begin(c, c.evShade, c.nShade);
        launch_shade(c, p, sv, fv, tx, r, p.grid, c.stream, 0u, p.nsq());
        timing_end(c, c.evShade, c.nShade); c.nShade++;
        if (r == p.rounds) break;
        timing_begin(c, c.evExtend, c.nExtend);
        if (c.debugFlags & PT_DEBUG_BRUTE_FORCE) k_extend_brute<<<p.grid, 256, 0, c.stream>>>(sv.accel, c.scene.blob, ac, qout, p.segCap, cout, c.counters.data(), p.sqShift);
        else if (c.debugFlags & PT_DEBUG_TRAVERSAL_V1)
            with_flags([&](auto S) { k_extend<S()><<<p.grid, 256, 0, c.stream>>>(c.scene.blob, ac, qout, p.segCap, cout, c.counters.data(), p.sqShift); }, p.stats);
        else
            with_flags([&](auto S, auto L, auto W, auto F) {
                k_extend2<S(), L(), W(), F()><<<p.grid, 256, p.extend2Lds, c.stream>>>(c.scene.blob, ac, qout, p.segCap, cout, c.counters.data(), p.sqShift);
            }, p.stats, p.lds, p.writeT, p.flat);
        timing_end(c, c.evExtend, c.nExtend); c.nExtend++;
    }
    return hipGetLastError();
}

static hipError_t enqueue_frame(Context& c, const FramePlan& p, const SceneView& sv, const FrameView& fv, const PtTextures& tx, uint32_t chains)
{
    hipError_t e = enqueue_preamble(c, p, sv, fv, tx);
    if (e != hipSuccess) return e;
    if (!p.first) return enqueue_validation_rounds(c, p, sv, fv, tx);
    for (uint32_t g = 0; g < chains && e == hipSuccess; g++) e = enqueue_chain(c, p, sv, fv, tx, g, chains, c.stream);
    return e;
}

template <typename T> static void key_add(std::string& k, const T& v) { k.append((const char*)&v, sizeof v); }

hipError_t launch_raytrace(Context& c, const SceneView& sv, const FrameView& fv, const PtTextures& tx, bool sharcQuery)
{
    const PtGraphicsSettings& gs = c.settings;
    const uint32_t npix = fv.width * fv.localRows;
    c.lastIterations = 0;
    if (c.normalsShared && c.scene.blasTable && c.scene.blob.triCount > c.shadeRecB.capacity()) {
        hipError_t ea = hipStreamSynchronize(c.stream);
        if (ea != hipSuccess) return ea;
        c.shadeRecA.reset(); c.shadeRecB.reset();
        if ((ea = c.shadeRecA.reserve(c.scene.blob.triCount)) != hipSuccess) return ea;
        if ((ea = c.shadeRecB.reserve(c.scene.blob.triCount)) != hipSuccess) return ea;
    }
    if (npix == 0 || gs.SamplesPerPixel == 0) return hipSuccess;
    hipError_t e;
    if (gs.Denoiser != PT_DENOISER_NONE && (e = c.pixelAux.reserve(npix)) != hipSuccess) return e;
    FramePlan plan; plan_frame(plan, c, sv, fv, sharcQuery);
    const FramePlan& p = plan;
    const uint32_t rounds = p.rounds, nsq = p.nsq(), cstride = p.cstride();
    if ((e = ensure_queues(c, p.segCap * nsq, (rounds + 2) * cstride)) != hipSuccess) return e;
    if ((e = c.frameConstants.reserve(1)) != hipSuccess) return e;
    if (p.sharc) for (auto& a : c.sharcRough) if ((e = a.reserve((size_t)p.segCap * nsq)) != hipSuccess) return e;
    FrameConstants fc; fc.cam = c.camera; fc.sd = c.sceneData; fc.gs = c.settings;
    k_set_constants<<<1, 256, 0, c.stream>>>(fc, c.frameConstants.data(), c.queueCounts.data(), (rounds + 2u) * cstride);
    c.lastIterations = rounds + 1;

    std::string key;
    key_add(key, sv); key_add(key, fv); key_add(key, tx); key_add(key, plan);
    key_add(key, c.queue[0]); key_add(key, c.queue[1]); key_add(key, c.queueCounts.data()); key_add(key, c.scene.blob);
    key_add(key, c.frameConstants.data()); key_add(key, c.primaryRecords.data()); key_add(key, c.stream); key_add(key, c.pixelAux.data()); key_add(key, gs.Denoiser); key_add(key, c.debugFlags);
    key_add(key, c.framesInFlight); key_add(key, c.chains);
    key_add(key, c.sharcView.data()); key_add(key, c.sharcRough[0].data()); key_add(key, c.sharcRough[1].data());
    key_add(key, c.shadeRecA.data()); key_add(key, c.scene.blasTable); key_add(key, c.scene.blasTableCount); key_add(key, c.scene.blasTableMaxTris);
    if (key != c.roundArgsKey || !c.roundArgs.data()) {
        if ((e = c.roundArgs.reserve(rounds + 1)) != hipSuccess) return e;
        std::vector<RoundArgs> host(rounds + 1);
        for (uint32_t r = 0; r <= rounds; r++) {
            RoundArgs& a = host[r];
            std::memset(&a, 0, sizeof a);
            a.sv = sv; a.fv = fv; a.tx = tx; a.bv = c.scene.blob; a.qin = c.queue[r & 1]; a.qout = c.queue[(r + 1) & 1];
            a.fc = c.frameConstants.data(); a.aux = p.aux; a.countIn = &c.queueCounts.data()[r * cstride]; a.countOut = &c.queueCounts.data()[(r + 1) * cstride]; a.sqShift = p.sqShift;
            a.counters = c.counters.data(); a.segCap = p.segCap; a.primary = c.primaryRecords.data(); a.objectsInLds = p.objectsInLds;
            if (p.recordsUsable) { a.recA = c.shadeRecA.data(); a.recB = c.shadeRecB.data(); a.recordsInLds = p.recordsInLds; }
            if (p.sharc) { a.sharc = c.sharcView.data(); a.roughIn = c.sharcRough[r & 1].data(); a.roughOut = c.sharcRough[(r + 1) & 1].data(); }
        }
        if ((e = hipMemcpyAsync(c.roundArgs.data(), host.data(), sizeof(RoundArgs) * (rounds + 1), hipMemcpyHostToDevice, c.stream)) != hipSuccess) return e;
        if ((e = hipStreamSynchronize(c.stream)) != hipSuccess) return e;
        c.roundArgsKey = key;
    }

    const bool graphable = c.stream != nullptr && !c.timing && !c.disableGraphs &&
                           (c.debugFlags & ~(PT_DEBUG_UNFUSED_ROUNDS | PT_DEBUG_TRAVERSAL_PHASED | PT_DEBUG_LOCKSTEP | PT_DEBUG_GATHER_LOCAL_ONLY | PT_DEBUG_GATHER_SELF_EXCHANGE | PT_DEBUG_SHARC_LOG_PATHS | PT_DEBUG_SHARC_SKIP_UPDATE)) == 0;
    auto capture = [&](hipStream_t s, GraphExec& exec, auto&& body) -> hipError_t {
        if (exec) { hipStreamSynchronize(c.stream); exec.reset(); }
        hipGraph_t graph = nullptr;
        hipError_t ce = hipStreamBeginCapture(s, hipStreamCaptureModeRelaxed);
        if (ce == hipSuccess) {
            const hipError_t e2 = body();
            ce = hipStreamEndCapture(s, &graph);
            if (ce == hipSuccess) ce = e2;
        }
        hipGraphExec_t ge = nullptr;
        if (ce == hipSuccess) ce = hipGraphInstantiate(&ge, graph, nullptr, nullptr, 0);
        if (graph) hipGraphDestroy(graph);
        if (ce == hipSuccess) exec.reset(ge); else (void)hipGetLastError();
        return ce;
    };
    const uint32_t chains = frame_chains(c, p, graphable);
    if (graphable && chains > 1) {
        if (!c.chainFork && (e = create_event(c.chainFork, hipEventDisableTiming)) != hipSuccess) return e;
        for (uint32_t g = 1; g < chains; g++) {
            if (!c.chainStream[g - 1] && (e = create_stream(c.chainStream[g - 1], hipStreamNonBlocking)) != hipSuccess) return e;
            if (!c.chainJoin[g - 1] && (e = create_event(c.chainJoin[g - 1], hipEventDisableTiming)) != hipSuccess) return e;
        }
        if (key != c.chainGraphKey) {
            c.chainGraphKey.clear();
            for (uint32_t g = 0; g < chains; g++) {
                hipStream_t s = g == 0 ? c.stream : c.chainStream[g - 1].get();
                if (capture(s, c.chainGraph[g], [&] { return enqueue_chain(c, p, sv, fv, tx, g, chains, s); }) != hipSuccess) { c.disableGraphs = true; break; }
            }
            if (!c.disableGraphs) c.chainGraphKey = key;
        }
        if (!c.disableGraphs) {
            if ((e = enqueue_preamble(c, p, sv, fv, tx)) != hipSuccess) return e;
            if ((e = hipEventRecord(c.chainFork.get(), c.stream)) != hipSuccess) return e;
            for (uint32_t g = 1; g < chains; g++) {
                hipStream_t s = c.chainStream[g - 1].get();
                if ((e = hipStreamWaitEvent(s, c.chainFork.get(), 0)) != hipSuccess) return e;
                if ((e = hipGraphLaunch(c.chainGraph[g].get(), s)) != hipSuccess) return e;
                if ((e = hipEventRecord(c.chainJoin[g - 1].get(), s)) != hipSuccess) return e;
            }
            if ((e = hipGraphLaunch(c.chainGraph[0].get(), c.stream)) != hipSuccess) return e;
            for (uint32_t g = 1; g < chains; g++) if ((e = hipStreamWaitEvent(c.stream, c.chainJoin[g - 1].get(), 0)) != hipSuccess) return e;
            return hipSuccess;
        }
    } else if (graphable) {
        if (key != c.graphKey || !c.graphExec) {
            c.graphKey.clear();
            if (capture(c.stream, c.graphExec, [&] { return enqueue_frame(c, p, sv, fv, tx, 1u); }) != hipSuccess) c.disableGraphs = true;
            else c.graphKey = key;
        }
        if (c.graphExec) return hipGraphLaunch(c.graphExec.get(), c.stream);
    }
    return enqueue_frame(c, p, sv, fv, tx, frame_chains(c, p, false));
}

hipError_t launch_deinterleave(hipStream_t stream, void* dst, const void* src, const uint64_t* rankOffsetsHost, uint32_t rankCount,
                               uint32_t bandHeight, uint32_t width, uint32_t height, uint32_t pixelBytes)
{
    RankOffsets ro;
    for (uint32_t r = 0; r < 64; r++) ro.v[r] = r < rankCount ? rankOffsetsHost[r] : 0;
    k_deinterleave<<<1024, 256, 0, stream>>>((uint8_t*)dst, (const uint8_t*)src, ro, rankCount, bandHeight, width, height, pixelBytes);
    return hipGetLastError();
}

}
```

directx-physically-based-raytracer_amd/csrc/pt_math.hpp:

```cpp
#pragma once
#include <hip/hip_runtime.h>
#include <stdint.h>

namespace pt {

struct v3 { float x, y, z; };

#define PT_DEV __device__ __forceinline__

PT_DEV v3 V3(float x, float y, float z) { v3 r; r.x = x; r.y = y; r.z = z; return r; }
PT_DEV v3 V3(const float* p) { return V3(p[0], p[1], p[2]); }
PT_DEV v3 operator+(v3 a, v3 b) { return V3(a.x + b.x, a.y + b.y, a.z + b.z); }
PT_DEV v3 operator-(v3 a, v3 b) { return V3(a.x - b.x, a.y - b.y, a.z - b.z); }
PT_DEV v3 operator*(v3 a, v3 b) { return V3(a.x * b.x, a.y * b.y, a.z * b.z); }
PT_DEV v3 operator*(v3 a, float s) { return V3(a.x * s, a.y * s, a.z * s); }
PT_DEV v3 operator-(v3 a) { return V3(-a.x, -a.y, -a.z); }
PT_DEV v3 vabs(v3 a) { return V3(fabsf(a.x), fabsf(a.y), fabsf(a.z)); }
PT_DEV float mad(float a, float b, float c) { return __builtin_fmaf(a, b, c); }
PT_DEV float sop3(float a0, float b0, float a1, float b1, float a2, float b2) { return mad(a2, b2, mad(a1, b1, a0 * b0)); }
PT_DEV float sop3t(float a0, float b0, float a1, float b1, float a2, float b2, float t) { return mad(a2, b2, mad(a1, b1, mad(a0, b0, t))); }
PT_DEV float dot(v3 a, v3 b) { return sop3(a.x, b.x, a.y, b.y, a.z, b.z); }
PT_DEV v3 cross(v3 a, v3 b) { return V3(mad(a.y, b.z, -(a.z * b.y)), mad(a.z, b.x, -(a.x * b.z)), mad(a.x, b.y, -(a.y * b.x))); }
PT_DEV v3 madd(v3 a, float s, v3 b) { return V3(mad(a.x, s, b.x), mad(a.y, s, b.y), mad(a.z, s, b.z)); }
PT_DEV v3 madd(v3 a, v3 s, v3 b) { return V3(mad(a.x, s.x, b.x), mad(a.y, s.y, b.y), mad(a.z, s.z, b.z)); }
// ... 184 lines not shown
    float bd = mad(c2, Y3, mad(c1, Y1, c0));
    float bias = bn * ml_positive_rcp(bd);
    float s0 = mad(3.32707f, X1, 0.0365463f);
    float s1 = mad(-9.04756f, X1, 9.0632f);
    float sn = mad(s1, Y1, s0);
    float d0 = mad(-1.36772f, X3, mad(3.59685f, X2, 1.0f));
    float d1 = mad(9.22949f, X3, mad(-16.3174f, X2, 9.04401f));
    float d2 = mad(-20.2123f, X3, mad(19.7886f, X2, 5.56589f));
    float sd = mad(d2, Y3, mad(d1, Y1, d0));
    float scale = sn * ml_positive_rcp(sd);
    return V3(saturate(mad(F0.x, scale, bias)), saturate(mad(F0.y, scale, bias)), saturate(mad(F0.z, scale, bias)));
}
PT_DEV v3 ml_vndf_get_ray(float u0, float u1, float roughness, v3 Vl)
{
    float m = roughness * roughness;
    v3 Vh = normalize(V3(m * Vl.x, m * Vl.y, Vl.z));
    float s, c; sincos_2pi(u0, s, c);
    float z = mad(1.0f - u1, 1.0f + Vh.z, -Vh.z);
    float sinT = ml_sqrt01(mad(-z, z, 1.0f));
    v3 h = V3(mad(sinT, c, Vh.x), mad(sinT, s, Vh.y), z + Vh.z);
    return normalize(V3(m * h.x, m * h.y, fmaxf(h.z, 0.0f)));
}
PT_DEV float ml_vndf_pdf(v3 Vl, float NoH, float roughness)
{
    float m = roughness * roughness;
    float D = ml_distribution_ggx(roughness, NoH);
    float ax = m * Vl.x, ay = m * Vl.y;
    float len2 = mad(ay, ay, ax * ax);
    float t = sqrtf(mad(Vl.z, Vl.z, len2));
    if (Vl.z >= 0.0f) return D / (2.0f * (Vl.z + t));
    return D * (t - Vl.z) / (2.0f * len2);
}
PT_DEV float ml_from_srgb1(float x)
{
    x = saturate(x);
    return x >= 0.04045f ? powf(x * (1.0f / 1.055f) + (0.055f / 1.055f), 2.4f) : x * (1.0f / 12.92f);
}

struct SurfaceVectors {
    v3 FrontGeometricNormal, ShadingNormal;
    basis3 ShadingBasis;
};
PT_DEV SurfaceVectors surface_vectors(bool isFront, v3 geometricNormal, v3 shadingNormal)
{
    SurfaceVectors sv;
    sv.FrontGeometricNormal = isFront ? geometricNormal : -geometricNormal;
    sv.ShadingNormal = shadingNormal;
    sv.ShadingBasis = ml_get_basis(shadingNormal);
    return sv;
}

constexpr float kMinRoughness = 2e-3f;
enum : int { LOBE_DIFFUSE = 0, LOBE_SPECULAR = 1, LOBE_TRANSMISSION = 2 };
constexpr uint32_t kExtLambertianOnly = 0x1u;

struct BSDFSample {
    v3 BaseColor; float Metallic; v3 Albedo; float Roughness, IORi, IORo; v3 F0; float Transmission;

    PT_DEV void Initialize(v3 baseColor, float metallic, float roughness, float IOR, float transmission, bool isFrontFace)
    {
        BaseColor = baseColor;
        Metallic = metallic;
        Albedo = baseColor * (1.0f - metallic);
        Roughness = fmaxf(kMinRoughness, roughness);
        IORi = 1.0f; IORo = IOR;
        if (!isFrontFace) { IORi = IOR; IORo = 1.0f; }
        float r = (IORi - IORo) / (IORi + IORo);
        float r2 = r * r;
        F0 = V3(mad(metallic, baseColor.x - r2, r2), mad(metallic, baseColor.y - r2, r2), mad(metallic, baseColor.z - r2, r2));
        Transmission = transmission;
    }

    PT_DEV float EstimateDiffuseProbability(float NoV) const
    {
        v3 Fenv = ml_env_term_rtg(F0, NoV, Roughness);
        float diffuse = ml_luminance(Albedo * V3(1.0f - Fenv.x, 1.0f - Fenv.y, 1.0f - Fenv.z));
        float specular = ml_luminance(Fenv);
        float sum = diffuse + specular;
        float p = sum > 0.0f ? diffuse / sum : 1.0f;
        if (0.0f < p && p < 1.0f) return clampf(p, 0.05f, 0.95f);
        return p;
    }

    PT_DEV void ComputeLobeWeights(const SurfaceVectors& sv, v3 V, uint32_t ext, float w[3]) const
    {
        if (ext & kExtLambertianOnly) { w[0] = 1.0f; w[1] = 0.0f; w[2] = 0.0f; return; }
        float NoV = fabsf(dot(sv.ShadingNormal, V));
        float tw = Transmission * (1.0f - Metallic);
        float rw = 1.0f - tw;
        float dw = EstimateDiffuseProbability(NoV);
        float sw = 1.0f - dw;
        w[LOBE_DIFFUSE] = dw * rw;
        w[LOBE_SPECULAR] = sw * rw;
        w[LOBE_TRANSMISSION] = tw;
    }

    PT_DEV static v3 reflect(v3 i, v3 n) { float d = dot(n, i); return madd(n, -(2.0f * d), i); }
    PT_DEV static v3 refract(v3 i, v3 n, float eta)
    {
        float d = dot(n, i);
        float k = mad(-(eta * eta), mad(-d, d, 1.0f), 1.0f);
        if (k < 0.0f) return V3(0.0f, 0.0f, 0.0f);
        float s = mad(eta, d, sqrtf(k));
        return madd(n, -s, i * eta);
    }

    PT_DEV bool Sample(const SurfaceVectors& sv, v3 V, const float w[3], const float rnd[4], v3& L, int& lobe) const
    {
        lobe = 0;
        {
            float weight = w[2];
            if (rnd[0] < weight) lobe = 2;
            else { weight += w[1]; if (rnd[0] < weight) lobe = 1; }
        }
        if (lobe == LOBE_DIFFUSE) {
            L = rotate_vector_inv(sv.ShadingBasis, ml_cosine_get_ray(rnd[1], rnd[2]));
            return dot(sv.FrontGeometricNormal, L) > 0.0f;
        }
        v3 Vlocal = rotate_vector(sv.ShadingBasis, V);
        v3 H = rotate_vector_inv(sv.ShadingBasis, ml_vndf_get_ray(rnd[1], rnd[2], Roughness, Vlocal));
        if (lobe == LOBE_SPECULAR) {
            L = reflect(-V, H);
            return dot(sv.FrontGeometricNormal, L) > 0.0f;
        }
        float VoH = fabsf(dot(V, H)), eta = IORi / IORo;
        if (eta * eta * (1.0f - VoH * VoH) > 1.0f || rnd[3] < ml_fresnel_dielectric(eta, VoH)) {
            L = reflect(-V, H);
        } else {
            L = refract(-V, H, eta);
            if (!finite3(L)) L = -V;
        }
        return true;
    }

    PT_DEV v3 ComputeHalfVector(const SurfaceVectors& sv, v3 L, v3 V, bool isTransmissive) const
    {
        v3 N = sv.FrontGeometricNormal, H;
        if (isTransmissive && dot(N, L) < 0.0f) {
            H = normalize(L * IORo + V * IORi);
            if (dot(N, H) < 0.0f) H = -H;
        } else {
            H = normalize(L + V);
        }
        return H;
    }

    PT_DEV void EvaluateAll(const SurfaceVectors& sv, v3 L, v3 V, const float w[3], float& pdf, v3& diffuse, v3& specular, uint32_t ext = 0) const
    {
        const float tw = w[LOBE_TRANSMISSION];
        pdf = 0.0f; diffuse = V3(0.0f, 0.0f, 0.0f); specular = V3(0.0f, 0.0f, 0.0f);
        if (tw > 0.0f) { float p; v3 f; EvaluateLobe(sv, L, V, w, LOBE_TRANSMISSION, 0, p, f); pdf = p; specular = f; }
        if (tw < 1.0f && dot(sv.FrontGeometricNormal, L) > 0.0f) {
            float pd, ps; v3 fd, fs;
            EvaluateLobe(sv, L, V, w, LOBE_DIFFUSE, ext, pd, fd);
            if (ext & kExtLambertianOnly) { ps = 0.0f; fs = V3(0.0f, 0.0f, 0.0f); }
            else EvaluateLobe(sv, L, V, w, LOBE_SPECULAR, 0, ps, fs);
            pdf += pd + ps;
            diffuse = fd;
            specular = specular + fs;
        }
    }

    PT_DEV void EvaluateLobe(const SurfaceVectors& sv, v3 L, v3 V, const float w[3], int lobe, uint32_t ext,
                             float& pdf, v3& f) const
    {
        const float tw = w[LOBE_TRANSMISSION];
        const v3 H = ComputeHalfVector(sv, L, V, tw > 0.0f);
        const v3 N = sv.ShadingNormal;
        const float lw = w[lobe];
        const float NoL = fabsf(dot(N, L));
        if (lobe == LOBE_TRANSMISSION) {
            pdf = NoL * lw;
            f = (BaseColor * NoL) * tw;
            return;
        }
        const float rw = 1.0f - tw;
        pdf = 0.0f; f = V3(0.0f, 0.0f, 0.0f);
        if (!(dot(sv.FrontGeometricNormal, L) > 0.0f)) return;
        const float NoV = fabsf(dot(N, V)), VoH = fabsf(dot(V, H));
        if (lobe == LOBE_DIFFUSE) {
            pdf = ml_cosine_pdf(NoL) * lw;
            float dterm = (ext & kExtLambertianOnly) ? (1.0f / kPi) : ml_diffuse_burley(Roughness, NoL, NoV, VoH);
            f = ((Albedo * NoL) * dterm) * rw;
            return;
        }
        const float NoH = fabsf(dot(N, H));
        v3 Vlocal = rotate_vector(sv.ShadingBasis, V);
        pdf = ml_vndf_pdf(Vlocal, NoH, Roughness) * lw;
        float D = ml_distribution_ggx(Roughness, NoH);
        float G = ml_geometry_term_mod(Roughness, NoL, NoV);
        v3 F = ml_fresnel_schlick(F0, VoH);
        float k = NoL * D * G;
        f = (F * k) * rw;
    }
};

PT_DEV void safe_triangle_spawn_point(v3 v0, v3 v1, v3 v2, float bx, float by, const float* M, const float* W,
                                      v3& objPosition, v3& wldPosition, v3& wldNormal, float& wldOffsetOut)
{
    v3 e1 = v1 - v0, e2 = v2 - v0;
    v3 op = V3(v0.x + __builtin_fmaf(bx, e1.x, by * e2.x), v0.y + __builtin_fmaf(bx, e1.y, by * e2.y),
               v0.z + __builtin_fmaf(bx, e1.z, by * e2.z));
    v3 on = cross(e1, e2);
    v3 wp;
    wp.x = M[3]  + __builtin_fmaf(M[0], op.x, __builtin_fmaf(M[1], op.y, M[2]  * op.z));
    wp.y = M[7]  + __builtin_fmaf(M[4], op.x, __builtin_fmaf(M[5], op.y, M[6]  * op.z));
    wp.z = M[11] + __builtin_fmaf(M[8], op.x, __builtin_fmaf(M[9], op.y, M[10] * op.z));
    v3 wn = V3(W[0] * on.x + W[4] * on.y + W[8]  * on.z,
               W[1] * on.x + W[5] * on.y + W[9]  * on.z,
               W[2] * on.x + W[6] * on.y + W[10] * on.z);
    float wldScale = 1.0f / sqrtf(dot(wn, wn));
    wn = wn * wldScale;

    const float c0 = 5.9604644775390625E-8f;
    const float c1 = 1.788139769587360206060111522674560546875E-7f;
    const float c2 = 1.19209317972490680404007434844970703125E-7f;
    v3 ae1 = vabs(e1), ae2 = vabs(e2);
    v3 ext3 = (ae1 + ae2) + vabs(ae1 - ae2);
    float extent = fmaxf(fmaxf(ext3.x, ext3.y), ext3.z);
    v3 av0 = vabs(v0);
    float ce = c1 * extent;
    v3 objErr = V3(__builtin_fmaf(c0, av0.x, ce), __builtin_fmaf(c0, av0.y, ce), __builtin_fmaf(c0, av0.z, ce));
    v3 aop = vabs(op);
    v3 mo = V3(fabsf(M[0]) * aop.x + fabsf(M[1]) * aop.y + fabsf(M[2])  * aop.z,
               fabsf(M[4]) * aop.x + fabsf(M[5]) * aop.y + fabsf(M[6])  * aop.z,
               fabsf(M[8]) * aop.x + fabsf(M[9]) * aop.y + fabsf(M[10]) * aop.z);
    v3 wldErr = V3(__builtin_fmaf(c1, mo.x, c2 * fabsf(M[3])), __builtin_fmaf(c1, mo.y, c2 * fabsf(M[7])),
                   __builtin_fmaf(c1, mo.z, c2 * fabsf(M[11])));
    v3 awp = vabs(wp);
    v3 wo = V3(fabsf(W[0]) * awp.x + fabsf(W[1]) * awp.y + fabsf(W[2])  * awp.z + fabsf(W[3]),
               fabsf(W[4]) * awp.x + fabsf(W[5]) * awp.y + fabsf(W[6])  * awp.z + fabsf(W[7]),
               fabsf(W[8]) * awp.x + fabsf(W[9]) * awp.y + fabsf(W[10]) * awp.z + fabsf(W[11]));
    objErr = V3(__builtin_fmaf(c2, wo.x, objErr.x), __builtin_fmaf(c2, wo.y, objErr.y), __builtin_fmaf(c2, wo.z, objErr.z));
    float wldOffset = dot(wldErr, vabs(wn));
    float objOffset = dot(objErr, vabs(on));
    wldOffset = __builtin_fmaf(wldScale, objOffset, wldOffset);
    objPosition = op; wldPosition = wp; wldNormal = wn; wldOffsetOut = wldOffset;
}

PT_DEV v3 safe_world_ray_origin(v3 position, v3 flatNormal, float offset, v3 dir)
{
    float s = ml_sign(dot(dir, flatNormal));
    v3 n = flatNormal * s;
    return V3(__builtin_fmaf(offset, n.x, position.x), __builtin_fmaf(offset, n.y, position.y), __builtin_fmaf(offset, n.z, position.z));
}

}
```

directx-physically-based-raytracer_amd/csrc/pt_shade.hpp:

```cpp
#pragma once
#include "pt_internal.hpp"
#include "pt_sharc.hpp"

namespace pt {


constexpr int kLdsStackDepth = 12;

struct RayDesc { v3 o, d; float tmin, tmax; };

PT_DEV RayDesc generate_pinhole_ray(const PtCamera& cam, uint32_t px, uint32_t py, uint32_t W, uint32_t H, float& u, float& v)
{
    u = ((float)px + 0.5f + cam.Jitter[0]) / (float)W;
    v = ((float)py + 0.5f + cam.Jitter[1]) / (float)H;
    float nx = u * 2.0f + -1.0f, ny = v * -2.0f + 1.0f;
    v3 R = V3(cam.RightDirection), U = V3(cam.UpDirection), F = V3(cam.ForwardDirection);
    v3 d = V3(mad(ny, U.x, mad(nx, R.x, F.x)), mad(ny, U.y, mad(nx, R.y, F.y)), mad(ny, U.z, mad(nx, R.z, F.z)));
    RayDesc r;
    r.o = V3(cam.Position);
    r.d = normalize(d);
    float invCos = 1.0f / dot(normalize(F), r.d);
    r.tmin = cam.NearDepth * invCos;
    r.tmax = cam.FarDepth * invCos;
    return r;
// ... 172 lines not shown

PT_DEV uint32_t block_reserve(bool alive, uint32_t* counter, uint32_t* lds)
{
    const uint32_t lane = threadIdx.x & 63, wave = threadIdx.x >> 6;
    const unsigned long long m = wave_ballot(alive);
    const uint32_t prefix = (uint32_t)__popcll(m & ((1ull << lane) - 1ull));
    if (lane == 0) lds[wave] = (uint32_t)__popcll(m);
    __syncthreads();
    if (threadIdx.x == 0) {
        const uint32_t total = lds[0] + lds[1] + lds[2] + lds[3];
        lds[4] = total ? atomicAdd(counter, total) : 0u;
    }
    __syncthreads();
    uint32_t base = lds[4];
    for (uint32_t w = 0; w < wave; w++) base += lds[w];
    __syncthreads();
    return base + prefix;
}

PT_DEV void block_reserve2(bool a, bool b, uint32_t* counterA, uint32_t* counterB, uint32_t* lds, uint32_t& slotA, uint32_t& slotB)
{
    const uint32_t lane = threadIdx.x & 63, wave = threadIdx.x >> 6;
    const unsigned long long lt = (1ull << lane) - 1ull;
    const unsigned long long ma = wave_ballot(a), mb = wave_ballot(b);
    if (lane == 0) { lds[wave] = (uint32_t)__popcll(ma); lds[4 + wave] = (uint32_t)__popcll(mb); }
    __syncthreads();
    if (threadIdx.x == 0) {
        const uint32_t total = lds[0] + lds[1] + lds[2] + lds[3];
        lds[8] = total ? atomicAdd(counterA, total) : 0u;
    }
    if (threadIdx.x == 64) {
        const uint32_t total = lds[4] + lds[5] + lds[6] + lds[7];
        lds[9] = total ? atomicAdd(counterB, total) : 0u;
    }
    __syncthreads();
    uint32_t baseA = lds[8], baseB = lds[9];
    for (uint32_t w = 0; w < wave; w++) { baseA += lds[w]; baseB += lds[4 + w]; }
    slotA = baseA + (uint32_t)__popcll(ma & lt);
    slotB = baseB + (uint32_t)__popcll(mb & lt);
}

struct PathRegs { v3 thr, srad, rsum; uint32_t pixel, rng, sample, bounce; };

PT_DEV PathRegs load_path(const PathQueue& q, uint32_t i)
{
    const float4 a = q.s0[i], b = q.s1[i], c = q.s2[i];
    PathRegs p;
    p.thr = V3(a.x, a.y, a.z); p.pixel = __float_as_uint(a.w);
    p.srad = V3(b.x, b.y, b.z); p.rng = __float_as_uint(b.w);
    p.rsum = V3(c.x, c.y, c.z);
    const uint32_t cnt = __float_as_uint(c.w);
    p.sample = cnt >> 16; p.bounce = cnt & 0xFFFFu;
    return p;
}
PT_DEV void store_path(const PathQueue& q, uint32_t i, const PathRegs& p)
{
    q.s0[i] = make_float4(p.thr.x, p.thr.y, p.thr.z, __uint_as_float(p.pixel));
    q.s1[i] = make_float4(p.srad.x, p.srad.y, p.srad.z, __uint_as_float(p.rng));
    q.s2[i] = make_float4(p.rsum.x, p.rsum.y, p.rsum.z, __uint_as_float((p.sample << 16) | p.bounce));
}

PT_DEV bool scatter_step(const PtGraphicsSettings& gs, uint32_t bounce, uint32_t& rng, v3& thr, const SurfaceHit& h, const BSDFSample& bs, v3 rayDir, v3& L, int& lobe,
                         float* rndOut = nullptr)
{
    const SurfaceVectors svec = surface_vectors(h.IsFrontFace, h.GeometricNormal, h.ShadingNormal);
    const v3 V = -rayDir;
    float w[3]; bs.ComputeLobeWeights(svec, V, gs.ExtFlags, w);
    float rnd[4];
    rnd[0] = rng_float(rng); rnd[1] = rng_float(rng); rnd[2] = rng_float(rng); rnd[3] = rng_float(rng);
    if (rndOut) { rndOut[0] = rnd[0]; rndOut[1] = rnd[1]; rndOut[2] = rnd[2]; rndOut[3] = rnd[3]; }
    if (!bs.Sample(svec, V, w, rnd, L, lobe)) return false;
    float pdf; v3 f;
    bs.EvaluateLobe(svec, L, V, w, lobe, gs.ExtFlags, pdf, f);
    if (pdf == 0.0f || (f.x == 0.0f && f.y == 0.0f && f.z == 0.0f)) return false;
    { const float ipdf = 1.0f / pdf; thr = thr * V3(f.x * ipdf, f.y * ipdf, f.z * ipdf); }
    if (gs.IsRussianRouletteEnabled && bounce > 3) {
        const float prob = fmaxf(thr.x, fmaxf(thr.y, thr.z));
        if (rng_float(rng) >= prob) return false;
        { const float iprob = 1.0f / prob; thr = V3(thr.x * iprob, thr.y * iprob, thr.z * iprob); }
    }
    return true;
}

template <bool SHARC = false>
PT_DEV bool scatter(const PtGraphicsSettings& gs, PathRegs& p, const SurfaceHit& h, const BSDFSample& bs, v3 emission, v3 rayDir, v3& newO, v3& newD, int& lobe,
                    float* previousRoughness = nullptr)
{
    p.srad = madd(p.thr, emission, p.srad);
    const SurfaceVectors svec = surface_vectors(h.IsFrontFace, h.GeometricNormal, h.ShadingNormal);
    const v3 V = -rayDir;
    float w[3]; bs.ComputeLobeWeights(svec, V, gs.ExtFlags, w);
    float rnd[4];
    rnd[0] = rng_float(p.rng); rnd[1] = rng_float(p.rng); rnd[2] = rng_float(p.rng); rnd[3] = rng_float(p.rng);
    v3 L;
    if (!bs.Sample(svec, V, w, rnd, L, lobe)) return false;
    float pdf; v3 f;
    bs.EvaluateLobe(svec, L, V, w, lobe, gs.ExtFlags, pdf, f);
    if (pdf == 0.0f || (f.x == 0.0f && f.y == 0.0f && f.z == 0.0f)) return false;
    { const float ipdf = 1.0f / pdf; p.thr = p.thr * V3(f.x * ipdf, f.y * ipdf, f.z * ipdf); }
    if (gs.IsRussianRouletteEnabled && p.bounce > 3) {
        const float prob = fmaxf(p.thr.x, fmaxf(p.thr.y, p.thr.z));
        if (rng_float(p.rng) >= prob) return false;
        { const float iprob = 1.0f / prob; p.thr = V3(p.thr.x * iprob, p.thr.y * iprob, p.thr.z * iprob); }
    }
    if (ml_luminance(p.thr) <= gs.ThroughputThreshold) return false;
    if constexpr (SHARC) *previousRoughness += lobe == LOBE_DIFFUSE ? 1.0f : bs.Roughness;
    if (!(p.bounce < gs.Bounces)) return false;
    newO = safe_world_ray_origin(h.Position, h.FlatNormal, h.PositionOffset, L);
    newD = L;
    p.bounce++;
    return true;
}

PT_DEV void load_direct(const PtTextures& tx, uint32_t pixel, v3& directDiffuse, v3& directSpecular)
{
    const ushort4 d = ((const ushort4*)tx.Diffuse)[pixel], s = ((const ushort4*)tx.Specular)[pixel];
    directDiffuse = V3(f16_to_f32(d.x), f16_to_f32(d.y), f16_to_f32(d.z));
    directSpecular = V3(f16_to_f32(s.x), f16_to_f32(s.y), f16_to_f32(s.z));
}
PT_DEV bool direct_valid(const PtTextures& tx, uint32_t pixel)
{
    v3 dd, ds; load_direct(tx, pixel, dd, ds);
    const v3 di = dd + ds;
    return di.x > 0.0f || di.y > 0.0f || di.z > 0.0f;
}

template <bool DI = false, bool SHARC = false>
PT_DEV bool end_sample(const PtGraphicsSettings& gs, const PtTextures& tx, const float2* aux, PathRegs& p)
{
    p.rsum = p.rsum + p.srad;
    p.sample++;
    if (p.sample < gs.SamplesPerPixel) { p.thr = V3(1, 1, 1); p.srad = V3(0, 0, 0); p.bounce = 0; return true; }
    v3 out = V3(0, 0, 0);
    if (finite3(p.rsum)) { const float ns = (float)gs.SamplesPerPixel; out = V3(p.rsum.x / ns, p.rsum.y / ns, p.rsum.z / ns); }
    if (gs.Denoiser == PT_DENOISER_NRD_REBLUR || gs.Denoiser == PT_DENOISER_NRD_RELAX) {
        const ushort4 rad = ((const ushort4*)tx.Radiance)[p.pixel];
        const v3 ind = V3(fmaxf(out.x - f16_to_f32(rad.x), 0.0f), fmaxf(out.y - f16_to_f32(rad.y), 0.0f), fmaxf(out.z - f16_to_f32(rad.z), 0.0f));
        const float2 a = aux[p.pixel];
        const bool isDiffuse = a.y != 0.0f;
        if constexpr (DI) {
            v3 dd, ds; load_direct(tx, p.pixel, dd, ds);
            const v3 id = isDiffuse ? ind : V3(0, 0, 0), is = isDiffuse ? V3(0, 0, 0) : ind;
            const float hd = isDiffuse ? a.x : 0.0f, hs = isDiffuse ? 0.0f : a.x;
            ((ushort4*)tx.Diffuse)[p.pixel] = make_ushort4(f32_to_f16(dd.x + id.x), f32_to_f16(dd.y + id.y), f32_to_f16(dd.z + id.z), f32_to_f16(hd));
            ((ushort4*)tx.Specular)[p.pixel] = make_ushort4(f32_to_f16(ds.x + is.x), f32_to_f16(ds.y + is.y), f32_to_f16(ds.z + is.z), f32_to_f16(hs));
            return false;
        }
        const ushort4 packed = make_ushort4(f32_to_f16(ind.x), f32_to_f16(ind.y), f32_to_f16(ind.z), f32_to_f16(a.x));
        const ushort4 zero = make_ushort4(0, 0, 0, 0);
        if (tx.Diffuse) ((ushort4*)tx.Diffuse)[p.pixel] = isDiffuse ? packed : zero;
        if (tx.Specular) ((ushort4*)tx.Specular)[p.pixel] = isDiffuse ? zero : packed;
        return false;
    }
    if constexpr (DI && !SHARC) { v3 dd, ds; load_direct(tx, p.pixel, dd, ds); out = out + (dd + ds); }
    if (gs.Denoiser == PT_DENOISER_DLSS_RAY_RECONSTRUCTION && tx.SpecularHitDistance) {
        const float2 a = aux[p.pixel];
        if (a.y == 0.0f && isfinite(a.x)) ((uint16_t*)tx.SpecularHitDistance)[p.pixel] = f32_to_f16(a.x);
    }
    ((ushort4*)tx.Radiance)[p.pixel] = make_ushort4(f32_to_f16(out.x), f32_to_f16(out.y), f32_to_f16(out.z), 0);
    if (tx.RadianceF32) ((float4*)tx.RadianceF32)[p.pixel] = make_float4(out.x, out.y, out.z, 0.0f);
    return false;
}

template <bool LDS> struct GeometryFromBlob {
    const BlobReader<LDS>& blob; const BlobView& bv; ShadeTables tables = ShadeTables();
    PT_DEV HitGeometry load(uint32_t inst, uint32_t slot) const { return load_hit_geometry<LDS>(blob, bv, inst, slot); }
};

template <bool TEXTURED, bool DI = false, bool SHARC = false, typename GEOMETRY>
PT_DEV void shade_traced(const SceneView& sv, const GEOMETRY& geometry, const PtSceneData& sd, const PtGraphicsSettings& gs, const PtTextures& tx, float2* aux,
                         PathRegs& p, uint4 hr, float hitT, v3 rayDir, bool& toTraced, bool& toFresh, v3& newO, v3& newD, RoundProf* prof = nullptr,
                         const SharcView* sharc = nullptr, float* previousRoughness = nullptr)
{
    bool goes = false; int lobe = 0;
    if (aux && p.sample == 0 && p.bounce == 1) aux[p.pixel].x = hr.x == ~0u ? INFINITY : hitT;
    if (hr.x == ~0u) {
        p.srad = madd(p.thr, environment_light_color(sv, sd, rayDir), p.srad);
    } else {
        SurfaceHit h;
        reconstruct_hit<TEXTURED>(sv, geometry.load(hr.x, hr.y), hr.x, __uint_as_float(hr.z), __uint_as_float(hr.w), rayDir, h, geometry.tables);
        PT_PROF_MARK(prof, 5);
        bool cached = false;
        if constexpr (SHARC) {
            v3 radiance;
            cached = sharc_query(*sharc, h.Position, dot(h.FlatNormal, rayDir) < 0.0f ? h.FlatNormal : -h.FlatNormal, hitT, *previousRoughness, radiance);
            if (cached) p.srad = madd(p.thr, radiance, p.srad);
        }
        if (!cached) {
            const PtMaterial m = surface_material<TEXTURED>(sv, h, geometry.tables.objects);
            BSDFSample bs;
            bs.Initialize(V3(m.BaseColor), m.Metallic, m.Roughness, m.IOR, m.Transmission, h.IsFrontFace);
            v3 emission = material_emission(m);
            if constexpr (DI) if (p.bounce == 1u && direct_valid(tx, p.pixel)) emission = V3(0, 0, 0);
            goes = scatter<SHARC>(gs, p, h, bs, emission, rayDir, newO, newD, lobe, previousRoughness);
        }
    }
    if (goes) toTraced = true;
    else toFresh = end_sample<DI, SHARC>(gs, tx, aux, p);
}

template <bool DI = false, bool SHARC = false>
PT_DEV void shade_fresh_record(const FrameView& fv, const PtCamera& cam, const PtGraphicsSettings& gs, const PtTextures& tx, float2* aux, uint4 r0, uint4 r1, uint4 r2,
                               PathRegs& p, bool& toTraced, bool& toFresh, v3& newO, v3& newD, float* previousRoughness = nullptr)
{
    const uint32_t pixel = p.pixel;
    const uint32_t px = pixel % fv.width, py = global_row(fv, pixel / fv.width);
    float uu, vv;
    const RayDesc primaryRay = generate_pinhole_ray(cam, px, py, fv.width, fv.height, uu, vv);
    const v3 rayDir = primaryRay.d;
    const float4 pos = make_float4(__uint_as_float(r0.x), __uint_as_float(r0.y), __uint_as_float(r0.z), __uint_as_float(r0.w));
    const short4 nr = make_short4((short)(r1.x & 0xFFFFu), (short)(r1.x >> 16), (short)(r1.y & 0xFFFFu), (short)(r1.y >> 16));
    const short2 fe = make_short2((short)(r1.z & 0xFFFFu), (short)(r1.z >> 16)), ge = make_short2((short)(r1.w & 0xFFFFu), (short)(r1.w >> 16));
    const uchar4 bcm = make_uchar4((unsigned char)(r2.x & 0xFFu), (unsigned char)((r2.x >> 8) & 0xFFu), (unsigned char)((r2.x >> 16) & 0xFFu), (unsigned char)(r2.x >> 24));
    const ushort4 rad = make_ushort4((unsigned short)(r2.y & 0xFFFFu), (unsigned short)(r2.y >> 16), (unsigned short)(r2.z & 0xFFFFu), (unsigned short)(r2.z >> 16));
    SurfaceHit h;
    h.Position = V3(pos.x, pos.y, pos.z); h.PositionOffset = pos.w;
    h.FlatNormal = oct_decode(snorm16_to_f32(fe.x), snorm16_to_f32(fe.y));
    h.GeometricNormal = oct_decode(snorm16_to_f32(ge.x), snorm16_to_f32(ge.y));
    h.ShadingNormal = V3(snorm16_to_f32(nr.x), snorm16_to_f32(nr.y), snorm16_to_f32(nr.z));
    h.IsFrontFace = dot(h.GeometricNormal, rayDir) < 0.0f;
    const v3 emission = V3(f16_to_f32(rad.x), f16_to_f32(rad.y), f16_to_f32(rad.z));
    const float metal = unorm8_to_f32(bcm.w);
    const float ior = f16_to_f32((uint16_t)(r2.w & 0xFFFFu));
    const float tr = metal < 1.0f ? unorm8_to_f32((uint8_t)((r2.w >> 16) & 0xFFu)) : 0.0f;
    BSDFSample bs;
    bs.Initialize(V3(unorm8_to_f32(bcm.x), unorm8_to_f32(bcm.y), unorm8_to_f32(bcm.z)), metal, snorm16_to_f32(nr.w), ior, tr, h.IsFrontFace);
    int lobe = 0;
    const bool first = p.sample == 0;
    if constexpr (SHARC) {
        *previousRoughness = 0.0f;
        if constexpr (DI) { v3 dd, ds; load_direct(tx, p.pixel, dd, ds); p.srad = p.srad + (dd + ds); }
    }
    if (scatter<SHARC>(gs, p, h, bs, emission, rayDir, newO, newD, lobe, previousRoughness)) {
        toTraced = true;
        if (aux && first) aux[p.pixel].y = lobe == LOBE_DIFFUSE ? 1.0f : 0.0f;
    } else toFresh = end_sample<DI, SHARC>(gs, tx, aux, p);
}

template <bool DI = false, bool SHARC = false>
PT_DEV void shade_fresh(const FrameView& fv, const PtCamera& cam, const PtGraphicsSettings& gs, const PtTextures& tx, float2* aux, const uint4* __restrict__ primary,
                        PathRegs& p, bool& toTraced, bool& toFresh, v3& newO, v3& newD, RoundProf* prof = nullptr, float* previousRoughness = nullptr)
{
    const uint32_t pixel = p.pixel;
    const uint4 r0 = primary[3 * (size_t)pixel], r1 = primary[3 * (size_t)pixel + 1], r2 = primary[3 * (size_t)pixel + 2];
    PT_PROF_WAIT(); PT_PROF_MARK(prof, 13);
    shade_fresh_record<DI, SHARC>(fv, cam, gs, tx, aux, r0, r1, r2, p, toTraced, toFresh, newO, newD, previousRoughness);
}

template <bool SHARC = false>
PT_DEV void emit_tile(const PathQueue& qout, uint32_t seg, uint32_t segCap, uint32_t* countTraced, uint32_t* countFresh, uint32_t* lds,
                      bool toTraced, bool toFresh, const PathRegs& p, v3 newO, v3 newD, float* roughnessOut = nullptr, float previousRoughness = 0.0f)
{
    uint32_t st, sf;
    block_reserve2(toTraced, toFresh, countTraced, countFresh, lds, st, sf);
    if (toTraced) {
        store_path(qout, seg + st, p);
        qout.r0[seg + st] = make_float4(newO.x, newO.y, newO.z, 0.0f);
        qout.r1[seg + st] = make_float4(newD.x, newD.y, newD.z, INFINITY);
        if constexpr (SHARC) roughnessOut[seg + st] = previousRoughness;
    }
    if (toFresh) store_path(qout, seg + (segCap - 1u - sf), p);
}

}
```

directx-physically-based-raytracer_amd/csrc/pt_trace.hpp:

```cpp
#pragma once
#include "pt_texture.hpp"

namespace pt {

__device__ __forceinline__ unsigned long long wave_ballot(bool p) { return __builtin_amdgcn_ballot_w64(p); }


struct alignas(16) WideNode {
    float origin[3]; uint32_t expImask;
    uint32_t childBase, triBase, meta[2];
    uint32_t qlox[2], qloy[2];
    uint32_t qloz[2], qhix[2];
    uint32_t qhiy[2], qhiz[2];
};
struct alignas(16) TriPacket { float4 a, b, c; };
static_assert(sizeof(WideNode) == 80 && sizeof(TriPacket) == 48, "layout");

struct alignas(16) InstanceRecord {
    float worldToObject[12];
    float objectToWorld[12];
    const WideNode* nodes;
    const TriPacket* tris;
    uint32_t instanceID;
    uint32_t mask;
// ... 106 lines not shown
        }
    }
    return hits;
}

struct RaySetup { bool c1, c2; float Sx, Sy, Sz; };
PT_DEV float sel_kz(v3 v, const RaySetup& r) { return r.c2 ? v.z : (r.c1 ? v.y : v.x); }
PT_DEV float sel_kx(v3 v, const RaySetup& r) { return r.c2 ? v.x : (r.c1 ? v.z : v.y); }
PT_DEV float sel_ky(v3 v, const RaySetup& r) { return r.c2 ? v.y : (r.c1 ? v.x : v.z); }

PT_DEV RaySetup ray_setup(v3 d)
{
    RaySetup r;
    const float ax = fabsf(d.x), ay = fabsf(d.y), az = fabsf(d.z);
    r.c1 = ay > ax;
    r.c2 = az > (r.c1 ? ay : ax);
    r.Sz = 1.0f / sel_kz(d, r);
    r.Sx = sel_kx(d, r) * r.Sz;
    r.Sy = sel_ky(d, r) * r.Sz;
    return r;
}

__device__ __attribute__((noinline)) void tri_edge_fallback(float Ax, float Ay, float Bx, float By, float Cx, float Cy, float& U, float& V, float& W)
{
    double CxBy = (double)Cx * (double)By, CyBx = (double)Cy * (double)Bx;
    U = (float)(CxBy - CyBx);
    double AxCy = (double)Ax * (double)Cy, AyCx = (double)Ay * (double)Cx;
    V = (float)(AxCy - AyCx);
    double BxAy = (double)Bx * (double)Ay, ByAx = (double)By * (double)Ax;
    W = (float)(BxAy - ByAx);
}

typedef float f2p __attribute__((ext_vector_type(2)));
PT_DEV bool tri_test(const RaySetup& r, v3 o, v3 v0, v3 v1, v3 v2, float& t, float& u, float& v)
{
    const f2p oxy = { o.x, o.y };
    const f2p Axy = (f2p){ v0.x, v0.y } - oxy, Bxy = (f2p){ v1.x, v1.y } - oxy, Cxy = (f2p){ v2.x, v2.y } - oxy;
    const v3 A = V3(Axy.x, Axy.y, v0.z - o.z), B = V3(Bxy.x, Bxy.y, v1.z - o.z), C = V3(Cxy.x, Cxy.y, v2.z - o.z);
    float Akz = sel_kz(A, r), Bkz = sel_kz(B, r), Ckz = sel_kz(C, r);
    const f2p S = { r.Sx, r.Sy };
    const f2p a = (f2p){ sel_kx(A, r), sel_ky(A, r) } - S * Akz;
    const f2p b = (f2p){ sel_kx(B, r), sel_ky(B, r) } - S * Bkz;
    const f2p c = (f2p){ sel_kx(C, r), sel_ky(C, r) } - S * Ckz;
    const f2p pu = c * b.yx, pv = a * c.yx, pw = b * a.yx;
    float U = pu.x - pu.y;
    float V = pv.x - pv.y;
    float W = pw.x - pw.y;
    if (__builtin_expect(U == 0.0f || V == 0.0f || W == 0.0f, 0)) tri_edge_fallback(a.x, a.y, b.x, b.y, c.x, c.y, U, V, W);
    if ((U < 0.0f || V < 0.0f || W < 0.0f) && (U > 0.0f || V > 0.0f || W > 0.0f)) return false;
    float det = U + V + W;
    if (det == 0.0f) return false;
    float Az = r.Sz * Akz, Bz = r.Sz * Bkz, Cz = r.Sz * Ckz;
    float T = U * Az + V * Bz + W * Cz;
    float rcp = 1.0f / det;
    t = T * rcp; u = V * rcp; v = W * rcp;
    return true;
}

PT_DEV bool is_better(const Hit& h, float tmin, float t, uint32_t inst, uint32_t geom, uint32_t prim)
{
    if (!(t > tmin)) return false;
    if (t < h.t) return true;
    if (t == h.t && h.inst != ~0u)
        return inst < h.inst || (inst == h.inst && (geom < h.geom || (geom == h.geom && prim < h.prim)));
    return false;
}

struct AlphaContext {
    const PtObjectData* objects;
    const HeapEntry* heap;
    const float* srgbLut;
    const struct InstanceRecord* instances;
    const HeapEntry* shadeTex = nullptr;
};

__device__ __attribute__((noinline)) bool candidate_is_opaque(const AlphaContext ac, uint32_t inst, uint32_t geom, uint32_t prim, float u, float v)
{
    const PtObjectData* od = &ac.objects[ac.instances[inst].instanceID + geom];
    TexCoords tc;
    get_texture_coordinates(od, ac.heap, prim, u, v, tc);
    return is_opaque(od, ac.heap, ac.srgbLut, tc, ac.shadeTex ? ac.shadeTex + (size_t)(ac.instances[inst].instanceID + geom) * kTextureSlots : nullptr);
}

PT_DEV void commit_candidate(const AlphaContext& ac, uint32_t flags, Hit& h, float tmin, float t, float u, float v,
                             uint32_t inst, uint32_t geom, uint32_t prim, uint32_t slot)
{
    if (!is_better(h, tmin, t, inst, geom, prim)) return;
    if (!(flags & PT_GEOMETRY_FLAG_OPAQUE) && !candidate_is_opaque(ac, inst, geom, prim, u, v)) return;
    h.t = t; h.u = u; h.v = v; h.inst = inst; h.geom = geom; h.prim = prim; h.slot = slot;
}

PT_DEV void transform_ray(const float* W, v3 o, v3 d, v3& ro, v3& rd)
{
    ro = V3(sop3t(W[0], o.x, W[1], o.y, W[2], o.z, W[3]), sop3t(W[4], o.x, W[5], o.y, W[6], o.z, W[7]), sop3t(W[8], o.x, W[9], o.y, W[10], o.z, W[11]));
    rd = V3(sop3(W[0], d.x, W[1], d.y, W[2], d.z), sop3(W[4], d.x, W[5], d.y, W[6], d.z), sop3(W[8], d.x, W[9], d.y, W[10], d.z));
}

PT_DEV Hit trace_brute_force(const AccelView& av, const AlphaContext& ac, v3 o, v3 d, float tmin, float tmax)
{
    Hit h; h.t = tmax; h.u = 0.0f; h.v = 0.0f; h.inst = ~0u; h.geom = 0; h.prim = 0; h.slot = 0;
    for (uint32_t x = 0; x < av.instanceCount; x++) {
        const InstanceRecord* ir = &av.instances[x];
        if (!(ir->mask & 0xFFu)) continue;
        v3 ro, rd;
        transform_ray(ir->worldToObject, o, d, ro, rd);
        const RaySetup rs = ray_setup(rd);
        for (uint32_t i = 0; i < ir->triCount; i++) {
            const TriPacket tp = ir->tris[i];
            float t, u, v;
            if (tri_test(rs, ro, V3(tp.a.x, tp.a.y, tp.a.z), V3(tp.b.x, tp.b.y, tp.b.z), V3(tp.c.x, tp.c.y, tp.c.z), t, u, v))
                commit_candidate(ac, __float_as_uint(tp.c.w), h, tmin, t, u, v, x, __float_as_uint(tp.a.w), __float_as_uint(tp.b.w), i);
        }
    }
    if (h.inst != ~0u && !(h.t < tmax)) h.inst = ~0u;
    return h;
}

}
```

directx-physically-based-raytracer_amd/csrc/pt_trace2.hpp:

```cpp
#pragma once
#include "pt_trace.hpp"

namespace pt {

#ifdef PT_ROUND_PROF
struct RoundProf { uint64_t last; uint32_t acc[16]; };
#define PT_PROF_WAIT() __builtin_amdgcn_s_waitcnt(0)
#define PT_PROF_MARK(P, i) do { if (P) { const uint64_t now_ = __builtin_readcyclecounter(); (P)->acc[i] += (uint32_t)(now_ - (P)->last); (P)->last = now_; } } while (0)
#else
struct RoundProf;
#define PT_PROF_MARK(P, i) do { } while (0)
#define PT_PROF_WAIT() do { } while (0)
#endif

struct alignas(16) InstanceT {
    float worldToObject[12];
    float boxLo[3]; uint32_t nodeBase;
    float boxHi[3]; uint32_t triBase;
    uint32_t mask, triCount, instanceID, instanceIndex;
    float objectToWorld[12];
};
static_assert(sizeof(InstanceT) == 144, "layout");

struct BlobView {
    const f4v* base;
    uint32_t instOff16, nodeOff16, triOff16, leafInstOff16;
    uint32_t idxOff16;
    uint32_t enterOff16;
    uint32_t instCount, nodeCount, triCount;
    uint32_t bytes;
};

constexpr uint32_t kInst16 = 9;
constexpr uint32_t kNode16 = 5;
constexpr uint32_t kTri16 = 3;
constexpr int kCandidates = 8;

template <bool LDS> struct BlobReader;
template <> struct BlobReader<false> {
    const f4v* p;
    PT_DEV f4v ld(uint32_t i) const { return p[i]; }
    PT_DEV uint32_t ld32(uint32_t i) const { return ((const uint32_t*)p)[i]; }
};
template <> struct BlobReader<true> {
    const PT_LDS_AS f4v* p;
    PT_DEV f4v ld(uint32_t i) const { return p[i]; }
    PT_DEV uint32_t ld32(uint32_t i) const { return ((const PT_LDS_AS uint32_t*)p)[i]; }
};

template <bool STATS, bool LDS, typename STACK>
PT_DEV void visit_node(const BlobReader<LDS>& blob, uint32_t nodeBase16, const BoxRay& br, float tmin, float tmax, uint2& G, uint2& T,
                       STACK& stack, TraceStats* stats)
{
    const uint32_t bit = 31u - (uint32_t)__builtin_clz(G.y);
    G.y &= ~(1u << bit);
    if (G.y > 0x00FFFFFFu) stack.push(G);
    const uint32_t slot = (bit - 24u) ^ (br.octinv4 & 7u);
    const uint32_t rel = (uint32_t)__builtin_popcount(G.y & 0xFFu & ~(0xFFFFFFFFu << slot));
    const uint32_t a = nodeBase16 + (G.x + rel) * kNode16;
    const f4v n0 = blob.ld(a), n1 = blob.ld(a + 1), n2 = blob.ld(a + 2), n3 = blob.ld(a + 3), n4 = blob.ld(a + 4);
    if (STATS) stats->nodes++;
    const uint32_t hits = wide_node_hits(n0, n1, n2, n3, n4, br, tmin, tmax);
    G = make_uint2(__float_as_uint(n1.x), (hits & 0xFF000000u) | (__float_as_uint(n0.w) >> 24));
    T = make_uint2(__float_as_uint(n1.y), hits & 0x00FFFFFFu);
}

template <bool STATS, bool LDS, bool CULL, typename STACK>
PT_DEV f4v trace_item(const BlobReader<LDS>& blob, const BlobView& bv, const AlphaContext& ac, const f4v* rays, uint32_t src, uint32_t x,
                      STACK& stack, TraceStats* stats)
{
    const f4v r0 = rays[2 * src], r1 = rays[2 * src + 1];
    const v3 io = V3(r0.x, r0.y, r0.z), id = V3(r1.x, r1.y, r1.z);
    const float itmin = r0.w, ibest = r1.w;
    Hit hi; hi.t = ibest; hi.u = 0.0f; hi.v = 0.0f; hi.inst = 0xFFFFFFFEu; hi.geom = ~0u; hi.prim = ~0u; hi.slot = ~0u;
    const uint32_t ia = bv.instOff16 + x * kInst16;
    const f4v b0 = blob.ld(ia + 3), b1 = blob.ld(ia + 4);
    bool enter = true;
    if (CULL) {
        const v3 iidir = safe_inv(id), iood = io * iidir;
        const float lx = __builtin_fmaf(b0.x, iidir.x, -iood.x), hx = __builtin_fmaf(b1.x, iidir.x, -iood.x);
        const float ly = __builtin_fmaf(b0.y, iidir.y, -iood.y), hy = __builtin_fmaf(b1.y, iidir.y, -iood.y);
        const float lz = __builtin_fmaf(b0.z, iidir.z, -iood.z), hz = __builtin_fmaf(b1.z, iidir.z, -iood.z);
        const float tn = fmaxf(fmaxf(fminf(lx, hx), fminf(ly, hy)), fmaxf(fminf(lz, hz), itmin));
        const float tf = fminf(fminf(fmaxf(lx, hx), fmaxf(ly, hy)), fminf(fmaxf(lz, hz), ibest));
        enter = tn <= tf * 1.0000004f;
    }
    if (enter) {
        const f4v w0 = blob.ld(ia), w1 = blob.ld(ia + 1), w2 = blob.ld(ia + 2);
        const v3 ro = V3(sop3t(w0.x, io.x, w0.y, io.y, w0.z, io.z, w0.w), sop3t(w1.x, io.x, w1.y, io.y, w1.z, io.z, w1.w), sop3t(w2.x, io.x, w2.y, io.y, w2.z, io.z, w2.w));
        const v3 rd = V3(sop3(w0.x, id.x, w0.y, id.y, w0.z, id.z), sop3(w1.x, id.x, w1.y, id.y, w1.z, id.z), sop3(w2.x, id.x, w2.y, id.y, w2.z, id.z));
        const RaySetup rs = ray_setup(rd);
        const BoxRay br = box_ray(ro, rd);
        const uint32_t triBase16 = bv.triOff16 + __float_as_uint(b1.w) * kTri16;
        const uint32_t nodeBase16 = bv.nodeOff16 + __float_as_uint(b0.w) * kNode16;
        const uint32_t ntri = __float_as_uint(blob.ld(ia + 5).y);
        const bool single = blas_single_leaf(ntri);
        uint2 G = root_node_group(single), T = root_tri_group(single, ntri);
        const int floor = stack.sp;
        while (true) {
            if (G.y > 0x00FFFFFFu) visit_node<STATS, LDS>(blob, nodeBase16, br, itmin, hi.t, G, T, stack, stats);
            while (T.y) {
                const uint32_t i = T.x + (uint32_t)__builtin_ctz(T.y);
                T.y &= T.y - 1u;
                const uint32_t ta = triBase16 + i * kTri16;
                const f4v pa = blob.ld(ta), pb = blob.ld(ta + 1), pc = blob.ld(ta + 2);
                if (STATS) stats->tris++;
                float t, u, v;
                if (tri_test(rs, ro, V3(pa.x, pa.y, pa.z), V3(pb.x, pb.y, pb.z), V3(pc.x, pc.y, pc.z), t, u, v))
                    commit_candidate(ac, __float_as_uint(pc.w), hi, itmin, t, u, v, x, __float_as_uint(pa.w), __float_as_uint(pb.w), i);
            }
            if (G.y <= 0x00FFFFFFu) {
                if (stack.sp == floor) break;
                G = stack.pop();
            }
        }
    }
    return (f4v){ hi.t, hi.u, hi.v, __uint_as_float(hi.slot) };
}

PT_DEV void merge_item(Hit& h, float tmin, f4v q, uint32_t x)
{
    const uint32_t slot = __float_as_uint(q.w);
    if (slot != ~0u && q.x > tmin && (q.x < h.t || (q.x == h.t && h.inst != ~0u && x < h.inst))) {
        h.t = q.x; h.u = q.y; h.v = q.z; h.inst = x; h.slot = slot;
    }
}

constexpr uint32_t kPhasedItems = 128;
constexpr uint32_t kPhasedWaveLds = 64u * 32u + kPhasedItems * 16u + kPhasedItems * 4u;

template <bool STATS, bool LDS, int STACK_DEPTH>
PT_DEV Hit trace_closest_v2(const BlobReader<LDS>& blob, const BlobView& bv, const AlphaContext& ac, v3 o, v3 d, float tmin, float tmax,
                            PT_LDS_AS void* ldsStack, uint32_t* ldsCand, unsigned char* ldsWave, TraceStats* stats)
{
    Hit h; h.t = tmax; h.u = 0.0f; h.v = 0.0f; h.inst = ~0u; h.geom = 0; h.prim = 0; h.slot = 0;
    if (bv.instCount == 0) return h;
    uint2 spill[kStackSize - STACK_DEPTH];
    GroupStack<STACK_DEPTH> stack; stack.init(ldsStack, spill);
    uint32_t* cand = ldsCand + threadIdx.x;
    const uint32_t lane = threadIdx.x & 63u;
    const unsigned long long ltMask = (1ull << lane) - 1ull;
    f4v* rays = (f4v*)ldsWave;
    f4v* results = (f4v*)(ldsWave + 64u * 32u);
    uint32_t* items = (uint32_t*)(ldsWave + 64u * 32u + kPhasedItems * 16u);
    rays[2 * lane] = (f4v){ o.x, o.y, o.z, tmin };

    const BoxRay br = box_ray(o, d);
    const bool oneInstance = bv.instCount == 1u;
    uint2 G = root_node_group(oneInstance), T = root_tri_group(oneInstance, 1u);
    bool tlasDone = !(tmin <= tmax);
    while (true) {
        uint32_t nCand = 0;
        while (!tlasDone && nCand < (uint32_t)kCandidates) {
            if (T.y) {
                const uint32_t i = T.x + (uint32_t)__builtin_ctz(T.y);
                T.y &= T.y - 1u;
                const f4v mk = blob.ld(bv.leafInstOff16 + i * kInst16 + 5);
                if ((__float_as_uint(mk.x) & 0xFFu) && __float_as_uint(mk.y) != 0u) { cand[nCand * 256] = __float_as_uint(mk.w); nCand++; }
            } else if (G.y > 0x00FFFFFFu) {
                visit_node<STATS, LDS>(blob, bv.nodeOff16, br, tmin, h.t, G, T, stack, stats);
            } else if (stack.sp > 0) {
                G = stack.pop();
            } else {
                tlasDone = true;
            }
        }
        for (uint32_t k = 0; wave_ballot(nCand > k) != 0ull; ) {
            uint32_t total = 0, k2 = k;
            while (true) {
                const unsigned long long bb = wave_ballot(nCand > k2);
                const uint32_t n = (uint32_t)__builtin_popcountll(bb);
                if (n == 0u || total + n > kPhasedItems) break;
                if (nCand > k2) items[total + (uint32_t)__builtin_popcountll(bb & ltMask)] = lane | (cand[k2 * 256] << 8);
                total += n; k2++;
            }
            rays[2 * lane + 1] = (f4v){ d.x, d.y, d.z, h.t };
            __builtin_amdgcn_wave_barrier();
            for (uint32_t j = lane; j < total; j += 64u) {
                const uint32_t it = items[j];
                results[j] = trace_item<STATS, LDS, true>(blob, bv, ac, rays, it & 0xFFu, it >> 8, stack, stats);
            }
            __builtin_amdgcn_wave_barrier();
            uint32_t off = 0;
            for (uint32_t kk = k; kk < k2; kk++) {
                const unsigned long long bb = wave_ballot(nCand > kk);
                if (nCand > kk) merge_item(h, tmin, results[off + (uint32_t)__builtin_popcountll(bb & ltMask)], cand[kk * 256]);
                off += (uint32_t)__builtin_popcountll(bb);
            }
            __builtin_amdgcn_wave_barrier();
            k = k2;
        }
        if (!wave_ballot(!tlasDone)) break;
    }
    stats->overflow += stack.overflow;
    if (h.inst != ~0u && !(h.t < tmax)) h.inst = ~0u;
    return h;
}

constexpr uint32_t kFlatInstances = 32;
constexpr int kStackLdsFlat = 4;
constexpr uint32_t kFlatItems = 192;
constexpr uint32_t kFlatWaveLds = 64u * 32u + kFlatItems * 16u + kFlatItems * 4u;
constexpr uint32_t kFlatLdsFixed = (uint32_t)kStackLdsFlat * 256u * 8u + 4u * kFlatWaveLds;

template <bool STATS, bool LDS>
PT_DEV Hit trace_closest_flat(const BlobReader<LDS>& blob, const BlobView& bv, const AlphaContext& ac, v3 o, v3 d, float tmin, float tmax,
                              PT_LDS_AS void* ldsStack, unsigned char* ldsWave, TraceStats* stats, RoundProf* prof = nullptr)
{
    Hit h; h.t = tmax; h.u = 0.0f; h.v = 0.0f; h.inst = ~0u; h.geom = 0; h.prim = 0; h.slot = 0;
    uint32_t quads = 0, meshes = 0;
    {
        const v3 idir = safe_inv(d), ood = o * idir;
        for (uint32_t x = 0; x < bv.instCount; x++) {
            const uint32_t ia = bv.instOff16 + x * kInst16;
            const f4v b0 = blob.ld(ia + 3), b1 = blob.ld(ia + 4), mk = blob.ld(ia + 5);
            const uint32_t ntri = __float_as_uint(mk.y);
            if (!(__float_as_uint(mk.x) & 0xFFu) || ntri == 0u) continue;
            const float lx = __builtin_fmaf(b0.x, idir.x, -ood.x), hx = __builtin_fmaf(b1.x, idir.x, -ood.x);
            const float ly = __builtin_fmaf(b0.y, idir.y, -ood.y), hy = __builtin_fmaf(b1.y, idir.y, -ood.y);
            const float lz = __builtin_fmaf(b0.z, idir.z, -ood.z), hz = __builtin_fmaf(b1.z, idir.z, -ood.z);
            const float tn = fmaxf(fmaxf(fminf(lx, hx), fminf(ly, hy)), fmaxf(fminf(lz, hz), tmin));
            const float tf = fminf(fminf(fmaxf(lx, hx), fmaxf(ly, hy)), fminf(fmaxf(lz, hz), tmax));
            const uint32_t bit = (tn <= tf * 1.0000004f) ? (1u << x) : 0u;
            if (blas_single_leaf(ntri)) quads |= bit; else meshes |= bit;
        }
        if (STATS) stats->nodes += (bv.instCount * 2u + 4u) / 5u;
    }
    PT_PROF_MARK(prof, 1);

    const uint32_t lane = threadIdx.x & 63u;
    const unsigned long long ltMask = (1ull << lane) - 1ull;
    f4v* rays = (f4v*)ldsWave;
    f4v* results = (f4v*)(ldsWave + 64u * 32u);
    uint32_t* items = (uint32_t*)(ldsWave + 64u * 32u + kFlatItems * 16u);
    const uint32_t nm = (uint32_t)__builtin_popcount(meshes), nq = (uint32_t)__builtin_popcount(quads);
    if (!wave_ballot((nm | nq) != 0u)) return h;
    rays[2 * lane] = (f4v){ o.x, o.y, o.z, tmin };
    uint2 spill[kStackSize - kStackLdsFlat];
    GroupStack<kStackLdsFlat> stack; stack.init(ldsStack, spill);

    uint32_t km = 0, kq = 0;
    bool firstBatch = true;
    while (true) {
        uint32_t total = 0, km2 = km, kq2 = kq;
        {
            uint32_t mb = meshes, qb = quads;
            while (true) {
                const unsigned long long bb = wave_ballot(nm > km2);
                const uint32_t n = (uint32_t)__builtin_popcountll(bb);
                if (n == 0u || total + n > kFlatItems) break;
                if (nm > km2) {
                    const uint32_t x = (uint32_t)__builtin_ctz(mb); mb &= mb - 1u;
                    items[total + (uint32_t)__builtin_popcountll(bb & ltMask)] = lane | (x << 8);
                }
                total += n; km2++;
            }
            if (!wave_ballot(nm > km2)) {
                while (true) {
                    const unsigned long long bb = wave_ballot(nq > kq2);
                    const uint32_t n = (uint32_t)__builtin_popcountll(bb);
                    if (n == 0u || total + n > kFlatItems) break;
                    if (nq > kq2) {
                        const uint32_t x = (uint32_t)__builtin_ctz(qb); qb &= qb - 1u;
                        items[total + (uint32_t)__builtin_popcountll(bb & ltMask)] = lane | (x << 8);
                    }
                    total += n; kq2++;
                }
            }
        }
        if (total == 0u) break;
        rays[2 * lane + 1] = (f4v){ d.x, d.y, d.z, h.t };
        __builtin_amdgcn_wave_barrier();
        PT_PROF_MARK(prof, 2);
#ifdef PT_ROUND_PROF
        if (prof) { prof->acc[9] += total; prof->acc[10] += (total + 63u) / 64u; }
#endif

        for (uint32_t j = lane; j < total; j += 64u) {
            const uint32_t it = items[j];
            stack.sp = 0;
            results[j] = firstBatch ? trace_item<STATS, LDS, false>(blob, bv, ac, rays, it & 0xFFu, it >> 8, stack, stats)
                                    : trace_item<STATS, LDS, true>(blob, bv, ac, rays, it & 0xFFu, it >> 8, stack, stats);
        }
        __builtin_amdgcn_wave_barrier();
        PT_PROF_MARK(prof, 3);

        {
            uint32_t off = 0;
            for (uint32_t pass = 0; pass < 2u; pass++) {
                const uint32_t ka = pass == 0u ? km : kq, kb = pass == 0u ? km2 : kq2, mine = pass == 0u ? nm : nq;
                for (uint32_t kk = ka; kk < kb; kk++) {
                    const unsigned long long bb = wave_ballot(mine > kk);
                    if (mine > kk) {
                        uint32_t x;
                        if (pass == 0u) { x = (uint32_t)__builtin_ctz(meshes); meshes &= meshes - 1u; }
                        else { x = (uint32_t)__builtin_ctz(quads); quads &= quads - 1u; }
                        merge_item(h, tmin, results[off + (uint32_t)__builtin_popcountll(bb & ltMask)], x);
                    }
                    off += (uint32_t)__builtin_popcountll(bb);
                }
            }
        }
        __builtin_amdgcn_wave_barrier();
        PT_PROF_MARK(prof, 4);
        km = km2; kq = kq2; firstBatch = false;
    }
    stats->overflow += stack.overflow;
    if (h.inst != ~0u && !(h.t < tmax)) h.inst = ~0u;
    return h;
}

template <bool STATS, bool LDS, bool ANYHIT, typename STACK, bool LOG = false>
PT_DEV Hit trace_single(const BlobReader<LDS>& blob, const BlobView& bv, const AlphaContext& ac, v3 o, v3 d, float tmin, float tmax,
                        STACK& stack, TraceStats* stats, v3* vis, uint32_t* log = nullptr, uint32_t logCap = 0)
{
    uint32_t nlog = 0;
    #define PT_LOG(code, a, b) do { if (LOG && 4u * nlog + 4u <= logCap) { log[4 * nlog] = (code); log[4 * nlog + 1] = (a); log[4 * nlog + 2] = (b); log[4 * nlog + 3] = (uint32_t)stack.sp; nlog++; } } while (0)
    Hit h; h.t = tmax; h.u = 0.0f; h.v = 0.0f; h.inst = ~0u; h.geom = 0; h.prim = 0; h.slot = 0;
    if (ANYHIT) *vis = V3(1.0f, 1.0f, 1.0f);
    if (bv.instCount == 0 || !(tmin <= tmax)) return h;
    constexpr uint32_t kMarker = 0xFFFFFFFFu;
    BoxRay br = box_ray(o, d);
    RaySetup rs; rs.c1 = rs.c2 = false; rs.Sx = rs.Sy = rs.Sz = 0.0f;
    v3 ro = o;
    uint32_t nodeBase16 = bv.nodeOff16, triBase16 = 0, curInst = ~0u;
    const bool oneInstance = bv.instCount == 1u;
    uint2 G = root_node_group(oneInstance), T = root_tri_group(oneInstance, 1u);
    stack.sp = 0;
    while (true) {
        if (T.y) {
            const uint32_t i = T.x + (uint32_t)__builtin_ctz(T.y);
            T.y &= T.y - 1u;
            if (curInst == ~0u) {
                const uint32_t ia = bv.enterOff16 + i * kInst16;
                const f4v mk = blob.ld(ia + 3);
                const uint32_t cm = __float_as_uint(mk.z), ntri = cm & 0x00FFFFFFu, x = __float_as_uint(mk.w);
                if ((cm >> 24) && ntri != 0u) {
                    const f4v w0 = blob.ld(ia), w1 = blob.ld(ia + 1), w2 = blob.ld(ia + 2);
                    const f4v n0 = blob.ld(ia + 4), n1 = blob.ld(ia + 5), n2 = blob.ld(ia + 6), n3 = blob.ld(ia + 7), n4 = blob.ld(ia + 8);
                    ro = V3(sop3t(w0.x, o.x, w0.y, o.y, w0.z, o.z, w0.w), sop3t(w1.x, o.x, w1.y, o.y, w1.z, o.z, w1.w), sop3t(w2.x, o.x, w2.y, o.y, w2.z, o.z, w2.w));
                    const v3 rd = V3(sop3(w0.x, d.x, w0.y, d.y, w0.z, d.z), sop3(w1.x, d.x, w1.y, d.y, w1.z, d.z), sop3(w2.x, d.x, w2.y, d.y, w2.z, d.z));
                    rs = ray_setup(rd);
                    br = box_ray(ro, rd);
                    nodeBase16 = bv.nodeOff16 + __float_as_uint(mk.x) * kNode16;
                    triBase16 = bv.triOff16 + __float_as_uint(mk.y) * kTri16;
                    PT_LOG(1u, x, T.y);
                    stack.push(G); stack.push(T); stack.push(make_uint2(kMarker, 0u));
                    curInst = x;
                    if (blas_single_leaf(ntri)) { G = root_node_group(true); T = root_tri_group(true, ntri); }
                    else {
                        if (STATS) stats->nodes++;
                        PT_LOG(3u, 0u, 0x80000000u);
                        const uint32_t hits = wide_node_hits(n0, n1, n2, n3, n4, br, tmin, ANYHIT ? tmax : h.t);
                        G = make_uint2(__float_as_uint(n1.x), (hits & 0xFF000000u) | (__float_as_uint(n0.w) >> 24));
                        T = make_uint2(__float_as_uint(n1.y), hits & 0x00FFFFFFu);
                        PT_LOG(4u, G.y, T.y);
                    }
                }
            } else {
                const uint32_t ta = triBase16 + i * kTri16;
                const f4v pa = blob.ld(ta), pb = blob.ld(ta + 1), pc = blob.ld(ta + 2);
                const bool two = !ANYHIT && T.y != 0u;
                uint32_t i2 = 0;
                f4v qa = pa, qb = pb, qc = pc;
                if (two) {
// ... 55 lines not shown
```

include/ptamd.h:

```cpp
#ifndef PTAMD_H
#define PTAMD_H

#include <stdint.h>

#ifdef __cplusplus
extern "C" {
#endif

#define PTAMD_ABI_VERSION 4

typedef enum PtStatus {
    PT_OK = 0,
    PT_ERROR_INVALID_ARGUMENT = -1,
    PT_ERROR_HIP = -2,
    PT_ERROR_OUT_OF_MEMORY = -3,
    PT_ERROR_NOT_READY = -4,
    PT_ERROR_NO_DEVICE = -5,
    PT_ERROR_RCCL = -6
} PtStatus;

typedef struct PtVertexDesc {
    uint32_t Stride, _pad[3];
    struct { uint32_t Normal, Tangent, TextureCoordinates[2]; } AttributeOffsets;
} PtVertexDesc;
// ... 322 lines not shown
int  pt_bsdf_sample(PtContext* ctx, const PtBsdfSampleQuery* device_queries, uint32_t count, PtBsdfSampleResult* device_results);

enum { PT_TONE_MAP_SATURATE = 1, PT_TONE_MAP_REINHARD = 2, PT_TONE_MAP_ACES_FILMIC = 3 };
enum { PT_COLOR_ROTATION_HDTV_TO_UHDTV = 0, PT_COLOR_ROTATION_DCI_P3_D65_TO_UHDTV = 1,
       PT_COLOR_ROTATION_HDTV_TO_DCI_P3_D65 = 2 };
typedef struct PtPostProcessSettings {
    uint32_t RenderSize[2];
    uint32_t IsBloomEnabled;  float BloomStrength;
    uint32_t IsHDREnabled;
    uint32_t ToneMappingOperator;  float Exposure;
    float    PaperWhiteNits;  uint32_t ColorPrimaryRotation;
    uint32_t _pad[3];
} PtPostProcessSettings;
typedef struct PtPostTextures {
    const void* Radiance;
    void* Color;
    void* BackBuffer;
    void* Display8;
} PtPostTextures;
int pt_post_set_constants(PtContext* ctx, const PtPostProcessSettings* settings);
int pt_post_render(PtContext* ctx, const PtPostTextures* textures);
int pt_post_download_bloom(PtContext* ctx, uint32_t stage, uint16_t* host_rgba16f, uint64_t capacity_texels,
                           uint32_t* out_width, uint32_t* out_height);

typedef struct PtSHARCSettings {
    uint32_t AccumulationFrames;
    uint32_t MaxStaleFrames;
    float    SceneScale;
    uint32_t IsAntiFireflyEnabled;
    uint32_t DownscaleFactor;
    float    RoughnessThreshold;
    uint32_t IsHashGridVisualizationEnabled;
} PtSHARCSettings;
typedef struct PtSHARCEntry { uint64_t Key; uint32_t Voxel[4]; uint32_t _pad[2]; } PtSHARCEntry;
typedef struct PtSHARCQueryResult { uint32_t Valid; float Radiance[3]; } PtSHARCQueryResult;
typedef struct PtSHARCPathVertex {
    float Position[3]; uint32_t Flags;
    float Normal[3];   float Random;
    float Radiance[3]; uint32_t KeyLo;
    float Throughput[3]; uint32_t KeyHi;
} PtSHARCPathVertex;
typedef struct PtSHARCPathScatter {
    PtBsdfSampleQuery Query;
    float Origin[3]; uint32_t Sampled;
    float L[3];      uint32_t Goes;
} PtSHARCPathScatter;
#define PT_SHARC_VERTEX_HIT       0x1u
#define PT_SHARC_VERTEX_MISS      0x2u
#define PT_SHARC_VERTEX_ENDED     0x4u
#define PT_SHARC_VERTEX_RESAMPLED 0x8u
int pt_sharc_configure(PtContext* ctx, uint32_t capacity);
int pt_sharc_set_constants(PtContext* ctx, const PtSHARCSettings* settings);
int pt_raytrace_render_sharc(PtContext* ctx, const PtTextures* textures);
int pt_sharc_reset(PtContext* ctx);
int pt_sharc_download(PtContext* ctx, PtSHARCEntry* host_dst, uint32_t capacity, uint32_t* out_count);
int pt_sharc_debug_keys(PtContext* ctx, const float* positions, const float* normals, uint32_t n, uint64_t* keys, uint32_t* levels, float* voxel_sizes);
int pt_sharc_debug_query(PtContext* ctx, const float* positions, const float* normals, const float* distances, const float* previous_roughness,
                         uint32_t n, PtSHARCQueryResult* results);
int pt_sharc_download_update_paths(PtContext* ctx, PtSHARCPathVertex* host_dst, uint32_t capacity, uint32_t* out_paths, uint32_t* out_bounces);
int pt_sharc_download_update_scatter(PtContext* ctx, PtSHARCPathScatter* host_dst, uint32_t capacity, uint32_t* out_paths, uint32_t* out_bounces);

typedef struct PtCounters {
    uint64_t PrimaryRays;
    uint64_t SecondaryRays;
    uint64_t NodesVisited;
    uint64_t TrianglesTested;
    uint64_t WavefrontIterations;
    uint64_t BvhMismatches;
    uint64_t StackOverflows;
    uint64_t MaxNodesPerRay;
} PtCounters;
int  pt_reset_counters(PtContext* ctx);
int  pt_get_counters(PtContext* ctx, PtCounters* out);
#define PT_DEBUG_TRAVERSAL_STATS 0x1u
#define PT_DEBUG_TRAVERSAL_V1   0x4u
#define PT_DEBUG_TRAVERSAL_PHASED 0x8u
#define PT_DEBUG_UNFUSED_ROUNDS  0x10u
#define PT_DEBUG_LOCKSTEP        0x20u
#define PT_DEBUG_GATHER_LOCAL_ONLY 0x40u
#define PT_DEBUG_BRUTE_FORCE     0x2u
#define PT_DEBUG_GATHER_SELF_EXCHANGE 0x80u
#define PT_DEBUG_SHARC_LOG_PATHS 0x100u
#define PT_DEBUG_SHARC_SKIP_UPDATE 0x200u
int  pt_set_debug_flags(PtContext* ctx, uint32_t flags);
int  pt_debug_read_mismatch(PtContext* ctx, float* out16);

typedef struct PtBlobLayout {
    uint32_t InstanceOffset16, NodeOffset16, TriangleOffset16, LeafInstanceOffset16;
    uint32_t InstanceCount, NodeCount, TriangleCount, Bytes;
} PtBlobLayout;
int  pt_debug_download_blob(PtContext* ctx, void* host_dst, uint64_t capacity_bytes, PtBlobLayout* out_layout);
int  pt_debug_trace_ray(PtContext* ctx, const PtRayDesc* host_ray, uint32_t* host_log, uint32_t log_words);
typedef struct PtClosestHit { float T, U, V; uint32_t Instance, Geometry, Primitive, Slot, _pad; } PtClosestHit;
int  pt_debug_trace_closest(PtContext* ctx, const PtRayDesc* device_rays, uint32_t count, PtClosestHit* device_hits);

int  pt_enable_kernel_timing(PtContext* ctx, int enable);
int  pt_get_kernel_timing(PtContext* ctx, float* extend_ms, float* shade_ms, uint32_t* extend_launches, uint32_t* shade_launches);
int  pt_get_round_timing(PtContext* ctx, float* round_ms, uint32_t* round_launches);

#ifdef __cplusplus
}
#endif
#endif
```

Before: 11960.

## Specialize round kernel for opaque, non-transmissive scenes via template flags

Tracks whether any referenced bottom level has non-opaque geometry and whether any material uses transmission (found during validation). When neither applies, the round kernel is instantiated with alpha testing and transmission lobes compiled out, which shrinks traversal and shading code and register pressure. A new debug flag forces the generic path. Without PT_SPEC_SPLIT both features collapse into one combined generic/specialized choice, which bounds the added instantiations. The risk is a wrong scene classification, which would drop alpha or transmission effects, plus a larger set of kernel variants.

```diff
diff --git a/directx-physically-based-raytracer_amd/csrc/pt_api.hip b/directx-physically-based-raytracer_amd/csrc/pt_api.hip
--- a/directx-physically-based-raytracer_amd/csrc/pt_api.hip
+++ b/directx-physically-based-raytracer_amd/csrc/pt_api.hip
@@ -194,6 +194,12 @@
     return PT_OK;
 }
 
+static bool any_non_opaque(const PtGeometryDesc* geometries, uint32_t geometry_count)
+{
+    for (uint32_t g = 0; g < geometry_count; g++) if (!(geometries[g].Flags & PT_GEOMETRY_FLAG_OPAQUE)) return true;
+    return false;
+}
+
 static int check_depth(Context& c, uint32_t tlasDepth)
 {
     if (2u * (tlasDepth + c.maxBlasDepth) + 4u > (uint32_t)kStackSize)
@@ -230,6 +236,7 @@
     if (e != hipSuccess) return fail_hip(&c, e, "bottom-level build");
     if (b.buildError || 2u * b.depth + 4u > (uint32_t)kStackSize) return fail(&c, PT_ERROR_INVALID_ARGUMENT, "bottom-level build failed: tree too deep for the traversal stack");
     b.geometryCount = geometry_count;
+    b.hasNonOpaque = any_non_opaque(geometries, geometry_count);
     uint64_t id = c.nextBlasId++;
     c.maxBlasDepth = std::max(c.maxBlasDepth, b.depth);
     c.blas[id] = std::move(b);
@@ -253,6 +260,7 @@
     if (b.updatable && ntris == b.triCount && geometry_count == b.geometryCount) {
         hipError_t e = refit_blas_device(geometries, geometry_count, c.stream, b);
         if (e != hipSuccess) return fail_hip(&c, e, "bottom-level update");
+        b.hasNonOpaque = any_non_opaque(geometries, geometry_count);
         drop_tlas(c);
         return PT_OK;
     }
@@ -265,6 +273,7 @@
     if (e != hipSuccess) return fail_hip(&c, e, "bottom-level update");
     if (nb.buildError || 2u * nb.depth + 4u > (uint32_t)kStackSize) return fail(&c, PT_ERROR_INVALID_ARGUMENT, "bottom-level update failed: tree too deep for the traversal stack");
     nb.geometryCount = geometry_count;
+    nb.hasNonOpaque = any_non_opaque(geometries, geometry_count);
     c.maxBlasDepth = std::max(c.maxBlasDepth, nb.depth);
     b = std::move(nb);
     drop_tlas(c);
@@ -482,6 +491,8 @@
     r.blob.instCount = count; r.blob.nodeCount = P.blobNodes; r.blob.triCount = P.blobTris; r.blob.bytes = (uint32_t)P.total;
     r.blasTable = dTable; r.blasTableCount = (uint32_t)P.table.size(); r.instSource = dSrc; r.blasTableMaxTris = 0;
     for (const BlasEntry& te : P.table) r.blasTableMaxTris = std::max(r.blasTableMaxTris, te.triCount);
+    r.hasNonOpaque = false;
+    for (const auto& p : P.pieces) if (p.referenced && p.b->hasNonOpaque) r.hasNonOpaque = true;
     c.tlasBlasIds = P.pieceIds;
     if (P.objectEnd != c.tlasObjectEnd || count != c.tlasValidatedCount || P.bindingHash != c.tlasBindingHash) c.validated = false;
     c.tlasObjectEnd = P.objectEnd; c.tlasValidatedCount = count; c.tlasBindingHash = P.bindingHash;
@@ -514,6 +525,7 @@
     c.objects = s.objects; c.objectCount = s.objectCount; c.instanceData = s.instanceData; c.instanceDataCount = s.instanceDataCount;
     c.sceneOwner = &s; s.viewers.push_back(&c);
     c.tlasHeaderPending = false; c.validated = false;
+    c.hasTransmission = c.gbufferTransmission = true;
     c.haveTlas = true;
     return PT_OK;
 }
@@ -569,7 +581,9 @@
 {
     if (!ctx) return PT_ERROR_INVALID_ARGUMENT;
     ctx->c.validated = false; ctx->c.normalsShared = false; ctx->c.sharedVerdict = false;
+    ctx->c.hasTransmission = true;
     ctx->c.objectDataGen++;
+    for (pt::Context* v : ctx->c.viewers) { v->validated = false; v->hasTransmission = true; }
     return PT_OK;
 }
 int pt_set_instance_data(PtContext* ctx, const PtInstanceData* device_instances, uint32_t count)
@@ -619,12 +633,14 @@
 {
     if (c.validated && c.validatedObjects == c.objects && c.validatedObjectCount == c.objectCount) return PT_OK;
     const uint32_t heapCount = (uint32_t)c.heapHost.size();
+    c.hasTransmission = true;
     if (c.tlasObjectEnd > c.objectCount)
         return fail(&c, PT_ERROR_INVALID_ARGUMENT, "InstanceID + geometry count of an instance reaches ObjectData[" + std::to_string(c.tlasObjectEnd - 1)
                     + "] but only " + std::to_string(c.objectCount) + " objects are bound (pt_set_object_data)");
     if (c.instanceData && c.instanceDataCount < c.scene.instanceCount)
         return fail(&c, PT_ERROR_INVALID_ARGUMENT, "InstanceData holds fewer records than the top level has instances");
     uint32_t sharedMismatch = 0;
+    bool transmission = false;
     if (c.objectCount) {
         API_HIP(&c, c.validateDev.reserve(8));
         if (c.objectCount > c.shadeGeomDev.capacity()) {
@@ -641,6 +657,7 @@
         API_HIP(&c, hipMemcpyAsync(r, c.validateDev.data(), sizeof r, hipMemcpyDeviceToHost, c.stream));
         API_HIP(&c, hipStreamSynchronize(c.stream));
         sharedMismatch = r[4];
+        transmission = r[5] != 0u;
         if (r[0]) {
             static const char* what[] = { "", "MeshDescriptors.Vertices", "MeshDescriptors.Indices", "MeshDescriptors.MotionVectors", "TextureMapInfo.Descriptor" };
             return fail(&c, PT_ERROR_INVALID_ARGUMENT, std::string("ObjectData[") + std::to_string(r[1]) + "]." + what[r[0] < 5 ? r[0] : 0] + " = " + std::to_string(r[2])
@@ -650,6 +667,7 @@
     c.validated = true; c.validatedObjects = c.objects; c.validatedObjectCount = c.objectCount;
     c.sharedVerdict = c.objectCount != 0 && c.scene.blasTable != nullptr && sharedMismatch == 0;
     c.normalsShared = c.sharedVerdict;
+    c.hasTransmission = transmission;
     return PT_OK;
 }
 
diff --git a/directx-physically-based-raytracer_amd/csrc/pt_internal.hpp b/directx-physically-based-raytracer_amd/csrc/pt_internal.hpp
--- a/directx-physically-based-raytracer_amd/csrc/pt_internal.hpp
+++ b/directx-physically-based-raytracer_amd/csrc/pt_internal.hpp
@@ -37,6 +37,7 @@
     DeviceBuffer<float> rootBounds;
     uint32_t triCount = 0, leafCount = 0, nodeCount = 0, depth = 0, geometryCount = 0;
     bool buildError = false, updatable = false;
+    bool hasNonOpaque = true;
     bool inBlob = false; uint64_t blobNodeAt = 0, blobTriAt = 0, blobIdxAt = 0;
     TreeBuffers tree;
 };
@@ -60,6 +61,7 @@
     BlobView blob{};
     const BlasEntry* blasTable = nullptr; uint32_t blasTableCount = 0, blasTableMaxTris = 0;
     const InstanceSource* instSource = nullptr;
+    bool hasNonOpaque = true;
 };
 
 struct alignas(16) ShadeGeom { const uint8_t* vb; uint32_t stride, nOff, tOff, uvOff[2], _pad; };
@@ -137,6 +139,7 @@
     bool sharedVerdict = false;
     bool validated = false; DeviceBuffer<uint32_t> validateDev;
     const void* validatedObjects = nullptr; uint32_t validatedObjectCount = 0;
+    bool hasTransmission = true, gbufferTransmission = true;
 
     PtCamera camera{}; PtSceneData sceneData{}; PtGraphicsSettings settings{};
     bool haveCamera = false, haveSceneData = false, haveSettings = false;
@@ -227,6 +230,22 @@
     else with_flags([&](auto... bs) { f(std::false_type{}, bs...); }, rest...);
 }
 
+#ifdef PT_SPEC_FORCE_ALPHA
+constexpr bool kSpecForceAlpha = true;
+#else
+constexpr bool kSpecForceAlpha = false;
+#endif
+#ifdef PT_SPEC_FORCE_TRANSMISSION
+constexpr bool kSpecForceTransmission = true;
+#else
+constexpr bool kSpecForceTransmission = false;
+#endif
+#ifdef PT_SPEC_SPLIT
+constexpr bool kSpecSplit = true;
+#else
+constexpr bool kSpecSplit = false;
+#endif
+
 hipError_t build_blas_device(const PtGeometryDesc* geoms, uint32_t ngeoms, bool allowUpdate, hipStream_t stream, Blas& out);
 hipError_t refit_blas_device(const PtGeometryDesc* geoms, uint32_t ngeoms, hipStream_t stream, Blas& b);
 hipError_t build_tlas_prepare(Tlas& out, uint32_t n);
@@ -246,6 +265,7 @@
     uint32_t objectsInLds, recordsInLds;
     bool recordsUsable;
     bool writeT, stats, di, textured, sharc;
+    bool alpha, transmission;
     float2* aux;
     uint32_t nsq() const { return 1u << sqShift; }
     uint32_t cstride() const { return 3u * nsq(); }
diff --git a/directx-physically-based-raytracer_amd/csrc/pt_kernels.hip b/directx-physically-based-raytracer_amd/csrc/pt_kernels.hip
--- a/directx-physically-based-raytracer_amd/csrc/pt_kernels.hip
+++ b/directx-physically-based-raytracer_amd/csrc/pt_kernels.hip
@@ -310,7 +310,7 @@
     const SharcView* sharc; const float* roughIn; float* roughOut;
 };
 
-template <bool TEXTURED, bool LDS, bool FLAT, bool DI, bool SHARC = false>
+template <bool TEXTURED, bool LDS, bool FLAT, bool DI, bool SHARC = false, bool ALPHA = true, bool TRANSMISSION = true>
 __global__ __launch_bounds__(256) __attribute__((amdgpu_waves_per_eu(4, 4))) void k_round(const RoundArgs* __restrict__ A, uint32_t sqBase, uint32_t sqCount)
 {
     const SceneView& sv = A->sv; const FrameView& fv = A->fv; const PtTextures& tx = A->tx; const BlobView& bv = A->bv;
@@ -378,16 +378,16 @@
             Hit h;
             if constexpr (FLAT) {
                 unsigned char* ldsWave = smem + (uint32_t)kStackLdsFlat * 256u * 8u + (threadIdx.x >> 6) * kFlatWaveLds;
-                h = trace_closest_flat<false, LDS>(blob, bv, ac, V3(o.x, o.y, o.z), V3(d.x, d.y, d.z), o.w, d.w, ldsStack, ldsWave, &st, prof);
+                h = trace_closest_flat<false, LDS, ALPHA>(blob, bv, ac, V3(o.x, o.y, o.z), V3(d.x, d.y, d.z), o.w, d.w, ldsStack, ldsWave, &st, prof);
             } else {
                 uint32_t* ldsCand = (uint32_t*)(smem + kStackLds2Bytes);
                 unsigned char* ldsWave = smem + kStackLds2Bytes + (uint32_t)kCandidates * 256u * 4u + (threadIdx.x >> 6) * kPhasedWaveLds;
-                h = trace_closest_v2<false, LDS, kStackLds2>(blob, bv, ac, V3(o.x, o.y, o.z), V3(d.x, d.y, d.z), o.w, d.w, ldsStack, ldsCand, ldsWave, &st);
+                h = trace_closest_v2<false, LDS, kStackLds2, ALPHA>(blob, bv, ac, V3(o.x, o.y, o.z), V3(d.x, d.y, d.z), o.w, d.w, ldsStack, ldsCand, ldsWave, &st);
             }
             bool toTraced = false, toFresh = false;
             v3 newO = V3(0, 0, 0), newD = V3(0, 0, 1);
             if (valid) {
-                shade_traced<TEXTURED, DI, SHARC>(sv, GeometryFromBlob<LDS>{ blob, bv, tables }, sd, gs, tx, aux, p, make_uint4(h.inst, h.slot, __float_as_uint(h.u), __float_as_uint(h.v)), h.t,
+                shade_traced<TEXTURED, DI, SHARC, TRANSMISSION>(sv, GeometryFromBlob<LDS>{ blob, bv, tables }, sd, gs, tx, aux, p, make_uint4(h.inst, h.slot, __float_as_uint(h.u), __float_as_uint(h.v)), h.t,
                                        V3(d.x, d.y, d.z), toTraced, toFresh, newO, newD, prof, A->sharc, &pr);
             }
             PT_PROF_MARK(prof, 6);
@@ -407,7 +407,7 @@
         if (local < nF) {
             p = load_path(qin, seg + (segCap - 1u - local));
             PT_PROF_WAIT(); PT_PROF_MARK(prof, 12);
-            shade_fresh<DI, SHARC>(fv, cam, gs, tx, aux, primary, p, toTraced, toFresh, newO, newD, prof, &pr);
+            shade_fresh<DI, SHARC, TRANSMISSION>(fv, cam, gs, tx, aux, primary, p, toTraced, toFresh, newO, newD, prof, &pr);
         }
         PT_PROF_MARK(prof, 14);
         emit_tile<SHARC>(qout, seg, segCap, &countOut[sq], &countOut[nsq + sq], lds + ((emits++ & 1u) << 4), toTraced, toFresh, p, newO, newD, A->roughOut, pr);
@@ -522,6 +522,15 @@
         shadeTex[(size_t)i * kTextureSlots + k] = e;
     }
     if (err && atomicCAS(&out[0], 0u, err) == 0u) { out[1] = i; out[2] = desc; out[3] = kind; }
+    {
+        bool has = od->Material.Transmission != 0.0f || od->TextureMapInfoArray[TEX_Transmission].Descriptor != ~0u || !isfinite(od->Material.Metallic);
+        for (int k = TEX_Metallic; k <= TEX_MetallicRoughness; k++) {
+            if (k == TEX_Roughness) continue;
+            const uint32_t d = od->TextureMapInfoArray[k].Descriptor;
+            if (d != ~0u && d < heapCount && heap[d].stride == kFmtRGBA32F) has = true;
+        }
+        if (has) out[5] = 1u;
+    }
     ShadeGeom sg; sg.vb = nullptr; sg.stride = 0; sg.nOff = ~0u; sg.tOff = ~0u; sg.uvOff[0] = sg.uvOff[1] = ~0u; sg._pad = 0;
     if (!err && md[0] != ~0u && md[1] != ~0u) {
         sg.vb = (const uint8_t*)heap[md[0]].ptr; sg.stride = od->VertexDesc.Stride;
@@ -688,6 +697,7 @@
         auto launch = [&](auto M) { k_gbuffer<S(), T(), M()><<<grid, 256, smem, c.stream>>>(sv, fv, c.camera, c.sceneData, flags, tx, c.scene.blob, c.counters.data()); };
         if (mode == 0) launch(std::integral_constant<int, 0>{}); else if (mode == 1) launch(std::integral_constant<int, 1>{}); else launch(std::integral_constant<int, 2>{});
     }, (c.debugFlags & PT_DEBUG_TRAVERSAL_STATS) != 0, c.heapHasTextures);
+    c.gbufferTransmission = c.hasTransmission;
     return hipGetLastError();
 }
 
@@ -760,6 +770,9 @@
     p.stats = (c.debugFlags & PT_DEBUG_TRAVERSAL_STATS) != 0;
     p.di = gs.IsDIEnabled != 0u;
     p.textured = c.heapHasTextures;
+    const bool generic = (c.debugFlags & (PT_DEBUG_GENERIC_SCENE | PT_DEBUG_TRAVERSAL_STATS | PT_DEBUG_BRUTE_FORCE | PT_DEBUG_TRAVERSAL_V1)) != 0;
+    p.alpha = generic || c.scene.hasNonOpaque || kSpecForceAlpha;
+    p.transmission = generic || c.hasTransmission || c.gbufferTransmission || kSpecForceTransmission;
 }
 
 constexpr uint32_t kStreamingChains = 3;
@@ -804,9 +817,10 @@
     }
     for (uint32_t r = 1; r <= p.rounds; r++) {
         timing_begin(c, c.evRound, c.nRound);
-        with_flags([&](auto T, auto L, auto F, auto D, auto S) {
-            k_round<T(), L(), F(), D(), S()><<<perSq * sqCount, 256, p.roundLds, s>>>(c.roundArgs.data() + r, sqBase, sqCount);
-        }, p.textured, p.lds, p.flat, p.di, p.sharc);
+        with_flags([&](auto T, auto L, auto F, auto D, auto S, auto A, auto X) {
+            constexpr bool generic = A() || X();
+            k_round<T(), L(), F(), D(), S(), kSpecSplit ? A() : generic, kSpecSplit ? X() : generic><<<perSq * sqCount, 256, p.roundLds, s>>>(c.roundArgs.data() + r, sqBase, sqCount);
+        }, p.textured, p.lds, p.flat, p.di, p.sharc, p.alpha, p.transmission);
         timing_end(c, c.evRound, c.nRound); c.nRound++;
     }
     return hipGetLastError();
@@ -896,7 +910,7 @@
     }
 
     const bool graphable = c.stream != nullptr && !c.timing && !c.disableGraphs &&
-                           (c.debugFlags & ~(PT_DEBUG_UNFUSED_ROUNDS | PT_DEBUG_TRAVERSAL_PHASED | PT_DEBUG_LOCKSTEP | PT_DEBUG_GATHER_LOCAL_ONLY | PT_DEBUG_GATHER_SELF_EXCHANGE | PT_DEBUG_SHARC_LOG_PATHS | PT_DEBUG_SHARC_SKIP_UPDATE)) == 0;
+                           (c.debugFlags & ~(PT_DEBUG_UNFUSED_ROUNDS | PT_DEBUG_TRAVERSAL_PHASED | PT_DEBUG_LOCKSTEP | PT_DEBUG_GATHER_LOCAL_ONLY | PT_DEBUG_GATHER_SELF_EXCHANGE | PT_DEBUG_SHARC_LOG_PATHS | PT_DEBUG_SHARC_SKIP_UPDATE | PT_DEBUG_GENERIC_SCENE)) == 0;
     auto capture = [&](hipStream_t s, GraphExec& exec, auto&& body) -> hipError_t {
         if (exec) { hipStreamSynchronize(c.stream); exec.reset(); }
         hipGraph_t graph = nullptr;
diff --git a/directx-physically-based-raytracer_amd/csrc/pt_math.hpp b/directx-physically-based-raytracer_amd/csrc/pt_math.hpp
--- a/directx-physically-based-raytracer_amd/csrc/pt_math.hpp
+++ b/directx-physically-based-raytracer_amd/csrc/pt_math.hpp
@@ -290,17 +290,24 @@
         return p;
     }
 
+    template <bool TRANSMISSION = true>
     PT_DEV void ComputeLobeWeights(const SurfaceVectors& sv, v3 V, uint32_t ext, float w[3]) const
     {
         if (ext & kExtLambertianOnly) { w[0] = 1.0f; w[1] = 0.0f; w[2] = 0.0f; return; }
         float NoV = fabsf(dot(sv.ShadingNormal, V));
-        float tw = Transmission * (1.0f - Metallic);
-        float rw = 1.0f - tw;
         float dw = EstimateDiffuseProbability(NoV);
         float sw = 1.0f - dw;
-        w[LOBE_DIFFUSE] = dw * rw;
-        w[LOBE_SPECULAR] = sw * rw;
-        w[LOBE_TRANSMISSION] = tw;
+        if constexpr (TRANSMISSION) {
+            float tw = Transmission * (1.0f - Metallic);
+            float rw = 1.0f - tw;
+            w[LOBE_DIFFUSE] = dw * rw;
+            w[LOBE_SPECULAR] = sw * rw;
+            w[LOBE_TRANSMISSION] = tw;
+        } else {
+            w[LOBE_DIFFUSE] = dw;
+            w[LOBE_SPECULAR] = sw;
+            w[LOBE_TRANSMISSION] = 0.0f;
+        }
     }
 
     PT_DEV static v3 reflect(v3 i, v3 n) { float d = dot(n, i); return madd(n, -(2.0f * d), i); }
@@ -313,13 +320,16 @@
         return madd(n, -s, i * eta);
     }
 
+    template <bool TRANSMISSION = true>
     PT_DEV bool Sample(const SurfaceVectors& sv, v3 V, const float w[3], const float rnd[4], v3& L, int& lobe) const
     {
         lobe = 0;
-        {
+        if constexpr (TRANSMISSION) {
             float weight = w[2];
             if (rnd[0] < weight) lobe = 2;
             else { weight += w[1]; if (rnd[0] < weight) lobe = 1; }
+        } else {
+            if (rnd[0] < w[1]) lobe = 1;
         }
         if (lobe == LOBE_DIFFUSE) {
             L = rotate_vector_inv(sv.ShadingBasis, ml_cosine_get_ray(rnd[1], rnd[2]));
@@ -327,7 +337,7 @@
         }
         v3 Vlocal = rotate_vector(sv.ShadingBasis, V);
         v3 H = rotate_vector_inv(sv.ShadingBasis, ml_vndf_get_ray(rnd[1], rnd[2], Roughness, Vlocal));
-        if (lobe == LOBE_SPECULAR) {
+        if (!TRANSMISSION || lobe == LOBE_SPECULAR) {
             L = reflect(-V, H);
             return dot(sv.FrontGeometricNormal, L) > 0.0f;
         }
@@ -341,10 +351,11 @@
         return true;
     }
 
+    template <bool TRANSMISSION = true>
     PT_DEV v3 ComputeHalfVector(const SurfaceVectors& sv, v3 L, v3 V, bool isTransmissive) const
     {
         v3 N = sv.FrontGeometricNormal, H;
-        if (isTransmissive && dot(N, L) < 0.0f) {
+        if (TRANSMISSION && isTransmissive && dot(N, L) < 0.0f) {
             H = normalize(L * IORo + V * IORi);
             if (dot(N, H) < 0.0f) H = -H;
         } else {
@@ -369,20 +380,21 @@
         }
     }
 
+    template <bool TRANSMISSION = true>
     PT_DEV void EvaluateLobe(const SurfaceVectors& sv, v3 L, v3 V, const float w[3], int lobe, uint32_t ext,
                              float& pdf, v3& f) const
     {
-        const float tw = w[LOBE_TRANSMISSION];
-        const v3 H = ComputeHalfVector(sv, L, V, tw > 0.0f);
+        const float tw = TRANSMISSION ? w[LOBE_TRANSMISSION] : 0.0f;
+        const v3 H = ComputeHalfVector<TRANSMISSION>(sv, L, V, tw > 0.0f);
         const v3 N = sv.ShadingNormal;
         const float lw = w[lobe];
         const float NoL = fabsf(dot(N, L));
-        if (lobe == LOBE_TRANSMISSION) {
+        if (TRANSMISSION && lobe == LOBE_TRANSMISSION) {
             pdf = NoL * lw;
             f = (BaseColor * NoL) * tw;
             return;
         }
-        const float rw = 1.0f - tw;
+        const float rw = TRANSMISSION ? 1.0f - tw : 1.0f;
         pdf = 0.0f; f = V3(0.0f, 0.0f, 0.0f);
         if (!(dot(sv.FrontGeometricNormal, L) > 0.0f)) return;
         const float NoV = fabsf(dot(N, V)), VoH = fabsf(dot(V, H));
diff --git a/directx-physically-based-raytracer_amd/csrc/pt_shade.hpp b/directx-physically-based-raytracer_amd/csrc/pt_shade.hpp
--- a/directx-physically-based-raytracer_amd/csrc/pt_shade.hpp
+++ b/directx-physically-based-raytracer_amd/csrc/pt_shade.hpp
@@ -278,20 +278,20 @@
     return true;
 }
 
-template <bool SHARC = false>
+template <bool SHARC = false, bool TRANSMISSION = true>
 PT_DEV bool scatter(const PtGraphicsSettings& gs, PathRegs& p, const SurfaceHit& h, const BSDFSample& bs, v3 emission, v3 rayDir, v3& newO, v3& newD, int& lobe,
                     float* previousRoughness = nullptr)
 {
     p.srad = madd(p.thr, emission, p.srad);
     const SurfaceVectors svec = surface_vectors(h.IsFrontFace, h.GeometricNormal, h.ShadingNormal);
     const v3 V = -rayDir;
-    float w[3]; bs.ComputeLobeWeights(svec, V, gs.ExtFlags, w);
+    float w[3]; bs.ComputeLobeWeights<TRANSMISSION>(svec, V, gs.ExtFlags, w);
     float rnd[4];
     rnd[0] = rng_float(p.rng); rnd[1] = rng_float(p.rng); rnd[2] = rng_float(p.rng); rnd[3] = rng_float(p.rng);
     v3 L;
-    if (!bs.Sample(svec, V, w, rnd, L, lobe)) return false;
+    if (!bs.Sample<TRANSMISSION>(svec, V, w, rnd, L, lobe)) return false;
     float pdf; v3 f;
-    bs.EvaluateLobe(svec, L, V, w, lobe, gs.ExtFlags, pdf, f);
+    bs.EvaluateLobe<TRANSMISSION>(svec, L, V, w, lobe, gs.ExtFlags, pdf, f);
     if (pdf == 0.0f || (f.x == 0.0f && f.y == 0.0f && f.z == 0.0f)) return false;
     { const float ipdf = 1.0f / pdf; p.thr = p.thr * V3(f.x * ipdf, f.y * ipdf, f.z * ipdf); }
     if (gs.IsRussianRouletteEnabled && p.bounce > 3) {
@@ -363,7 +363,7 @@
     PT_DEV HitGeometry load(uint32_t inst, uint32_t slot) const { return load_hit_geometry<LDS>(blob, bv, inst, slot); }
 };
 
-template <bool TEXTURED, bool DI = false, bool SHARC = false, typename GEOMETRY>
+template <bool TEXTURED, bool DI = false, bool SHARC = false, bool TRANSMISSION = true, typename GEOMETRY>
 PT_DEV void shade_traced(const SceneView& sv, const GEOMETRY& geometry, const PtSceneData& sd, const PtGraphicsSettings& gs, const PtTextures& tx, float2* aux,
                          PathRegs& p, uint4 hr, float hitT, v3 rayDir, bool& toTraced, bool& toFresh, v3& newO, v3& newD, RoundProf* prof = nullptr,
                          const SharcView* sharc = nullptr, float* previousRoughness = nullptr)
@@ -388,14 +388,14 @@
             bs.Initialize(V3(m.BaseColor), m.Metallic, m.Roughness, m.IOR, m.Transmission, h.IsFrontFace);
             v3 emission = material_emission(m);
             if constexpr (DI) if (p.bounce == 1u && direct_valid(tx, p.pixel)) emission = V3(0, 0, 0);
-            goes = scatter<SHARC>(gs, p, h, bs, emission, rayDir, newO, newD, lobe, previousRoughness);
+            goes = scatter<SHARC, TRANSMISSION>(gs, p, h, bs, emission, rayDir, newO, newD, lobe, previousRoughness);
         }
     }
     if (goes) toTraced = true;
     else toFresh = end_sample<DI, SHARC>(gs, tx, aux, p);
 }
 
-template <bool DI = false, bool SHARC = false>
+template <bool DI = false, bool SHARC = false, bool TRANSMISSION = true>
 PT_DEV void shade_fresh_record(const FrameView& fv, const PtCamera& cam, const PtGraphicsSettings& gs, const PtTextures& tx, float2* aux, uint4 r0, uint4 r1, uint4 r2,
                                PathRegs& p, bool& toTraced, bool& toFresh, v3& newO, v3& newD, float* previousRoughness = nullptr)
 {
@@ -427,20 +427,20 @@
         *previousRoughness = 0.0f;
         if constexpr (DI) { v3 dd, ds; load_direct(tx, p.pixel, dd, ds); p.srad = p.srad + (dd + ds); }
     }
-    if (scatter<SHARC>(gs, p, h, bs, emission, rayDir, newO, newD, lobe, previousRoughness)) {
+    if (scatter<SHARC, TRANSMISSION>(gs, p, h, bs, emission, rayDir, newO, newD, lobe, previousRoughness)) {
         toTraced = true;
         if (aux && first) aux[p.pixel].y = lobe == LOBE_DIFFUSE ? 1.0f : 0.0f;
     } else toFresh = end_sample<DI, SHARC>(gs, tx, aux, p);
 }
 
-template <bool DI = false, bool SHARC = false>
+template <bool DI = false, bool SHARC = false, bool TRANSMISSION = true>
 PT_DEV void shade_fresh(const FrameView& fv, const PtCamera& cam, const PtGraphicsSettings& gs, const PtTextures& tx, float2* aux, const uint4* __restrict__ primary,
                         PathRegs& p, bool& toTraced, bool& toFresh, v3& newO, v3& newD, RoundProf* prof = nullptr, float* previousRoughness = nullptr)
 {
     const uint32_t pixel = p.pixel;
     const uint4 r0 = primary[3 * (size_t)pixel], r1 = primary[3 * (size_t)pixel + 1], r2 = primary[3 * (size_t)pixel + 2];
     PT_PROF_WAIT(); PT_PROF_MARK(prof, 13);
-    shade_fresh_record<DI, SHARC>(fv, cam, gs, tx, aux, r0, r1, r2, p, toTraced, toFresh, newO, newD, previousRoughness);
+    shade_fresh_record<DI, SHARC, TRANSMISSION>(fv, cam, gs, tx, aux, r0, r1, r2, p, toTraced, toFresh, newO, newD, previousRoughness);
 }
 
 template <bool SHARC = false>
diff --git a/directx-physically-based-raytracer_amd/csrc/pt_trace.hpp b/directx-physically-based-raytracer_amd/csrc/pt_trace.hpp
--- a/directx-physically-based-raytracer_amd/csrc/pt_trace.hpp
+++ b/directx-physically-based-raytracer_amd/csrc/pt_trace.hpp
@@ -212,11 +212,12 @@
     return is_opaque(od, ac.heap, ac.srgbLut, tc, ac.shadeTex ? ac.shadeTex + (size_t)(ac.instances[inst].instanceID + geom) * kTextureSlots : nullptr);
 }
 
+template <bool ALPHA = true>
 PT_DEV void commit_candidate(const AlphaContext& ac, uint32_t flags, Hit& h, float tmin, float t, float u, float v,
                              uint32_t inst, uint32_t geom, uint32_t prim, uint32_t slot)
 {
     if (!is_better(h, tmin, t, inst, geom, prim)) return;
-    if (!(flags & PT_GEOMETRY_FLAG_OPAQUE) && !candidate_is_opaque(ac, inst, geom, prim, u, v)) return;
+    if constexpr (ALPHA) if (!(flags & PT_GEOMETRY_FLAG_OPAQUE) && !candidate_is_opaque(ac, inst, geom, prim, u, v)) return;
     h.t = t; h.u = u; h.v = v; h.inst = inst; h.geom = geom; h.prim = prim; h.slot = slot;
 }
 
diff --git a/directx-physically-based-raytracer_amd/csrc/pt_trace2.hpp b/directx-physically-based-raytracer_amd/csrc/pt_trace2.hpp
--- a/directx-physically-based-raytracer_amd/csrc/pt_trace2.hpp
+++ b/directx-physically-based-raytracer_amd/csrc/pt_trace2.hpp
@@ -65,7 +65,7 @@
     T = make_uint2(__float_as_uint(n1.y), hits & 0x00FFFFFFu);
 }
 
-template <bool STATS, bool LDS, bool CULL, typename STACK>
+template <bool STATS, bool LDS, bool CULL, bool ALPHA = true, typename STACK>
 PT_DEV f4v trace_item(const BlobReader<LDS>& blob, const BlobView& bv, const AlphaContext& ac, const f4v* rays, uint32_t src, uint32_t x,
                       STACK& stack, TraceStats* stats)
 {
@@ -107,7 +107,7 @@
                 if (STATS) stats->tris++;
                 float t, u, v;
                 if (tri_test(rs, ro, V3(pa.x, pa.y, pa.z), V3(pb.x, pb.y, pb.z), V3(pc.x, pc.y, pc.z), t, u, v))
-                    commit_candidate(ac, __float_as_uint(pc.w), hi, itmin, t, u, v, x, __float_as_uint(pa.w), __float_as_uint(pb.w), i);
+                    commit_candidate<ALPHA>(ac, __float_as_uint(pc.w), hi, itmin, t, u, v, x, __float_as_uint(pa.w), __float_as_uint(pb.w), i);
             }
             if (G.y <= 0x00FFFFFFu) {
                 if (stack.sp == floor) break;
@@ -129,7 +129,7 @@
 constexpr uint32_t kPhasedItems = 128;
 constexpr uint32_t kPhasedWaveLds = 64u * 32u + kPhasedItems * 16u + kPhasedItems * 4u;
 
-template <bool STATS, bool LDS, int STACK_DEPTH>
+template <bool STATS, bool LDS, int STACK_DEPTH, bool ALPHA = true>
 PT_DEV Hit trace_closest_v2(const BlobReader<LDS>& blob, const BlobView& bv, const AlphaContext& ac, v3 o, v3 d, float tmin, float tmax,
                             PT_LDS_AS void* ldsStack, uint32_t* ldsCand, unsigned char* ldsWave, TraceStats* stats)
 {
@@ -178,7 +178,7 @@
             __builtin_amdgcn_wave_barrier();
             for (uint32_t j = lane; j < total; j += 64u) {
                 const uint32_t it = items[j];
-                results[j] = trace_item<STATS, LDS, true>(blob, bv, ac, rays, it & 0xFFu, it >> 8, stack, stats);
+                results[j] = trace_item<STATS, LDS, true, ALPHA>(blob, bv, ac, rays, it & 0xFFu, it >> 8, stack, stats);
             }
             __builtin_amdgcn_wave_barrier();
             uint32_t off = 0;
@@ -203,7 +203,7 @@
 constexpr uint32_t kFlatWaveLds = 64u * 32u + kFlatItems * 16u + kFlatItems * 4u;
 constexpr uint32_t kFlatLdsFixed = (uint32_t)kStackLdsFlat * 256u * 8u + 4u * kFlatWaveLds;
 
-template <bool STATS, bool LDS>
+template <bool STATS, bool LDS, bool ALPHA = true>
 PT_DEV Hit trace_closest_flat(const BlobReader<LDS>& blob, const BlobView& bv, const AlphaContext& ac, v3 o, v3 d, float tmin, float tmax,
                               PT_LDS_AS void* ldsStack, unsigned char* ldsWave, TraceStats* stats, RoundProf* prof = nullptr)
 {
@@ -279,8 +279,8 @@
         for (uint32_t j = lane; j < total; j += 64u) {
             const uint32_t it = items[j];
             stack.sp = 0;
-            results[j] = firstBatch ? trace_item<STATS, LDS, false>(blob, bv, ac, rays, it & 0xFFu, it >> 8, stack, stats)
-                                    : trace_item<STATS, LDS, true>(blob, bv, ac, rays, it & 0xFFu, it >> 8, stack, stats);
+            results[j] = firstBatch ? trace_item<STATS, LDS, false, ALPHA>(blob, bv, ac, rays, it & 0xFFu, it >> 8, stack, stats)
+                                    : trace_item<STATS, LDS, true, ALPHA>(blob, bv, ac, rays, it & 0xFFu, it >> 8, stack, stats);
         }
         __builtin_amdgcn_wave_barrier();
         PT_PROF_MARK(prof, 3);
diff --git a/include/ptamd.h b/include/ptamd.h
--- a/include/ptamd.h
+++ b/include/ptamd.h
@@ -428,6 +428,7 @@
 #define PT_DEBUG_GATHER_SELF_EXCHANGE 0x80u
 #define PT_DEBUG_SHARC_LOG_PATHS 0x100u
 #define PT_DEBUG_SHARC_SKIP_UPDATE 0x200u
+#define PT_DEBUG_GENERIC_SCENE  0x400u
 int  pt_set_debug_flags(PtContext* ctx, uint32_t flags);
 int  pt_debug_read_mismatch(PtContext* ctx, float* out16);
 
```

After: 12310 (median of 6 runs). 2.9% higher.
